# tk1363704/CAREL-VAE

Measured on AMD Instinct MI355X. Metric: clause-pairs/sec (training step), higher is better.
Workload: dtype bf16

## Files before the change

carel_vae_amd/csrc/carel_hip_internal.h:

```cpp
#pragma once
#include <hip/hip_runtime.h>
#include <stdarg.h>
#include <stdio.h>
#include "../../include/carel_hip.h"
#include "carel_common.h"

#ifdef CAREL_EXPERIMENTS
#define CAREL_TUNABLE(type, name, value) static type name = value
#else
#define CAREL_TUNABLE(type, name, value) static constexpr type name = value
#endif

namespace carel {

int set_error(int code, const char* fmt, ...);
int check_launch(const char* what);
int slab_reduce_multi(const void* slabs, void* out, int64_t n, const void* slabs2, void* out2, int64_t n2, int splits, const void* partials,
                      int nparts, void* dgamma, void* dbeta, void* dbias, hipStream_t stream);
#ifdef CAREL_EXPERIMENTS
int gemm_rowln_wanted(long rows);
int gemm_rowln_wanted_k(int K);
#else
inline int gemm_rowln_wanted(long) { return 0; }
inline int gemm_rowln_wanted_k(int) { return 0; }
#endif
void encoder_ln_resid_enable(int on);
void encoder_ln_slab_fusion_enable(int on);
void encoder_wgrad_group_enable(int on);
void adam_grid_cap(long cap);
void tail_overlap_enable(int on);
int gemm_pp_init_device(int device);
int gather_rows(const void* in_f32, const void* in_bf16, const void* idx, int n, void* out_f32, void* out_bf16, hipStream_t stream);
int scatter_rows(const void* in_f32, const void* in_bf16, const void* idx, int n, void* out_f32, void* out_bf16, hipStream_t stream);

int layernorm_bwd_rows(const void* dy, const void* h, const void* stats, const void* gamma, int64_t rows, uint32_t drop_seed, uint32_t drop_site,
                       uint32_t drop_idx_offset, float drop_p, const void* drop_row_map, void* dh_f32, void* dy_bf16, void* partials,
                       hipStream_t stream);
int layernorm_bwd_reduce(const void* partials, int64_t rows, void* dgamma, void* dbeta, void* dbias, hipStream_t stream);
int layernorm_bwd_blocks_max(int64_t rows);
int layernorm_bwd_rows_slabs(const void* slabs, int splits, const void* resid, const void* h, const void* stats, const void* gamma, int64_t rows,
                             uint32_t drop_seed, uint32_t drop_site, uint32_t drop_idx_offset, float drop_p, const void* drop_row_map, void* dh_f32,
                             void* dy_bf16, void* partials, hipStream_t stream);
int layernorm_fwd_slabs(const void* slabs, int splits, const void* bias, const void* resid, const void* resid_stats, const void* resid_gamma,
                        const void* resid_beta, uint32_t drop_seed, uint32_t drop_site, uint32_t drop_idx_offset, float drop_p, const void* drop_row_map,
                        void* h_out, const void* gamma, const void* beta, float eps, int64_t rows, void* x_f32, void* x_bf16, void* stats,
                        hipStream_t stream);

constexpr int GEMM_EX_FIXED_ROWS = 0x100;
constexpr int GEMM_EX_DEFER_EPILOGUE = 0x200;
int gemm_bf16_ex(const carel_gemm_args* a, int split_tile_factor, void* stream);
int gemm_bf16_split_plan(const carel_gemm_args* a, int split_tile_factor);
int gemm_wgrad_splits_max(int M, int N, long T);
int embed_ln_bwd_ex(const carel_embed_args* a, const void* dx0, void* dword, void* dpos, void* dtype_, void* dgamma, void* dbeta,
                    void* partials, void* row_scratch, hipStream_t stream, const void* sort_ws = nullptr);
int embed_sort_supported(const carel_embed_args* a);
size_t embed_sort_bytes();
int embed_ln_fwd_keys(const carel_embed_args* a, void* sort_ws, hipStream_t stream);
int embed_sort_rows(const carel_embed_args* a, void* sort_ws, hipStream_t stream);

struct WgradGroupProb { const void* dY; const void* X; void* dW; void* db; int M, N; };
struct WgradGroupLn { const void* partials; int nparts; void* dgamma; void* dbeta; void* dbias; };
size_t gemm_pp_wgrad_group_ws_bytes(const WgradGroupProb* pb, int n, long T);
int gemm_pp_wgrad_group_ok(const WgradGroupProb* pb, int n, long T);
int gemm_pp_wgrad_group(const WgradGroupProb* pb, int n, long T, void* ws, size_t ws_bytes, const WgradGroupLn* ln, int n_ln, hipStream_t stream);

inline Dropout make_dropout(uint32_t seed, uint32_t site, float p, uint32_t idx_offset) {
  Dropout d;
  d.key = mix32(seed + site * 0x9E3779B9u);
  d.idx_offset = idx_offset;
  if (p <= 0.f) { d.thresh = 0u; d.scale = 1.f; }
  else if (p >= 1.f) { d.thresh = 0xFFFFFFFFu; d.scale = 0.f; }
  else {
    d.thresh = (uint32_t)((double)p * 4294967296.0);
    d.scale = (float)(1.0 / (1.0 - (double)p));
    if (d.thresh == 0u) d.scale = 1.f;
  }
  return d;
}

struct AttnParams;
int attn_long_fwd(const AttnParams& q, hipStream_t stream);
int attn_long_bwd(const AttnParams& q, void* workspace, int64_t workspace_bytes, hipStream_t stream);

}
```

carel_vae_amd/csrc/encoder.hip:

```cpp
#include <cstdlib>
#include <mutex>
#include <vector>
#include "carel_hip_internal.h"

using namespace carel;

namespace {

constexpr int EH = 768, EI = 3072, ENH = 12;

size_t al(size_t x) { return (x + 255) & ~(size_t)255; }

struct LayerAct {
  char* xin_bf16; char* qkv; char* lse; char* ctx; char* h1; char* st1; char* x1_bf16; char* u; char* g; char* h2; char* st2;
};
struct ActLayout {
  size_t per_layer, total;
  size_t o_xin, o_qkv, o_lse, o_ctx, o_h1, o_st1, o_x1, o_u, o_g, o_h2, o_st2;
  size_t o_embst, o_xa, o_xb, o_cctx, o_cxres, o_layers;
};

ActLayout act_layout(long B, long S, int L, int inference) {
  const size_t T = (size_t)B * S;
  ActLayout a; size_t o = 0;
// ... 51 lines not shown
    const size_t n = (size_t)gemm_wgrad_splits_max(sh[0], sh[1], (long)T) * ((size_t)sh[0] * sh[1] + sh[0]) * 4;
    slab = n > slab ? n : slab;
  }
  {
    const WgradGroupProb pb[4] = {{nullptr, nullptr, nullptr, nullptr, EH, EI}, {nullptr, nullptr, nullptr, nullptr, EI, EH}, {nullptr, nullptr, nullptr, nullptr, 3 * EH, EH},
                                  {nullptr, nullptr, nullptr, nullptr, EH, EH}};
    const size_t n = gemm_pp_wgrad_group_ws_bytes(pb, 4, (long)T);
    slab = n > slab ? n : slab;
  }
  s.o_slabs = o; o += al(slab); s.slab_bytes = al(slab);
  s.o_ws = o; o += al(slab); s.ws_bytes = al(slab);
  size_t part = (size_t)layernorm_bwd_blocks_max((long)T) * 4 * EH * 4;
  const size_t cs = ((T + 255) / 256) * EI * 4;
  part = part > cs ? part : cs;
  for (int par = 0; par < 2; ++par) {
    s.o_part[par] = o; o += al(part);
    s.o_part3[par] = o; o += al(part);
  }
  s.o_part2 = o; o += al(part);
  s.o_sort = o; o += al(embed_sort_bytes());
  s.attn_bytes = (size_t)carel_attention_bwd_workspace_bytes((int32_t)B, (int32_t)S, 1);
  s.o_attn = o; o += al(s.attn_bytes);
  s.total = o;
  return s;
}

Scratch scratch_of(const ScratchLayout& l, char* b, int par = 0) {
  Scratch s; s.dy = b + l.o_dy; s.dyb = b + l.o_dyb[par]; s.dyb2 = b + l.o_dyb2[par]; s.du = b + l.o_du[par]; s.dctx = b + l.o_dctx; s.dqkv = b + l.o_dqkv[par];
  s.slabs = b + l.o_slabs; s.ws = b + l.o_ws; s.part = b + l.o_part[par]; s.part2 = b + l.o_part2; s.part3 = b + l.o_part3[par];
  return s;
}

long n_rows_of(const carel_encoder_args* a) {
  return (a->tok_row && a->n_tokens > 0) ? (long)a->n_tokens : (long)a->batch * a->seq_len;
}

int enc_check(const carel_encoder_args* a, const char* who) {
  if (!a) return set_error(CAREL_ERR_ARG, "%s: null args", who);
  if (a->hidden != EH || a->heads != ENH || a->intermediate != EI)
    return set_error(CAREL_ERR_SHAPE, "%s: only the BERT-base geometry (768/12/3072) is supported", who);
  if (a->batch < 1 || a->n_layers < 1) return set_error(CAREL_ERR_SHAPE, "%s: bad batch / n_layers", who);
  if (a->seq_len < 32 || a->seq_len > 512 || (a->seq_len & 31)) return set_error(CAREL_ERR_SHAPE, "%s: seq_len must be a multiple of 32 in [32, 512]", who);
  if (((long)a->batch * a->seq_len) % 128) return set_error(CAREL_ERR_SHAPE, "%s: batch*seq_len must be a multiple of 128 (pad the batch)", who);
  if (!a->input_ids || !a->layers || !a->act) return set_error(CAREL_ERR_ARG, "%s: null tensor", who);
  if (a->n_cls) {
    if (!a->cls_rows || !a->cls_orig_rows || a->n_cls % 128 || a->n_cls < a->batch || a->n_cls > ((a->batch + 127) / 128) * 128)
      return set_error(CAREL_ERR_ARG, "%s: n_cls must be batch rounded up to 128, with cls_rows and cls_orig_rows", who);
  }
  if (a->tok_row || a->cu_seqlens || a->n_tokens) {
    if (!a->tok_row || !a->cu_seqlens || a->n_tokens <= 0 || a->n_tokens % 128 || a->n_tokens > a->batch * a->seq_len)
      return set_error(CAREL_ERR_ARG, "%s: packing needs tok_row, cu_seqlens and n_tokens (multiple of 128, <= batch*seq_len)", who);
  }
  return CAREL_OK;
}

struct SideStream { static constexpr int NEV = 13; hipStream_t stream; hipStream_t aux; hipStream_t peer; hipEvent_t ev[NEV]; bool ok; };
SideStream* side_stream() {
  static SideStream per_dev[16];
  static bool made[16];
  int dev = 0;
  if (hipGetDevice(&dev) != hipSuccess || dev < 0 || dev >= 16) return nullptr;
  if (!made[dev]) {
    SideStream& s = per_dev[dev];
    int lo = 0, hi = 0;
    s.ok = hipDeviceGetStreamPriorityRange(&lo, &hi) == hipSuccess;
#ifdef CAREL_EXPERIMENTS
    if (const char* e = getenv("CAREL_SIDE_STREAM_PRIORITY")) { if (e[0] == 'n') lo = 0; else if (e[0] == 'h') lo = hi; }
#endif
    s.ok = s.ok &&
           hipStreamCreateWithPriority(&s.stream, hipStreamNonBlocking, lo) == hipSuccess &&
           hipStreamCreateWithPriority(&s.aux, hipStreamNonBlocking, lo) == hipSuccess &&
           hipStreamCreateWithFlags(&s.peer, hipStreamNonBlocking) == hipSuccess;
    for (int i = 0; i < SideStream::NEV && s.ok; ++i) s.ok = hipEventCreateWithFlags(&s.ev[i], hipEventDisableTiming) == hipSuccess;
    made[dev] = true;
  }
  return per_dev[dev].ok ? &per_dev[dev] : nullptr;
}

struct LnResid { const void* stats; const void* gamma; const void* beta; };
CAREL_TUNABLE(int, g_ln_slab_fusion, 1);
int ln_slab_fusion_enabled() { return g_ln_slab_fusion; }
CAREL_TUNABLE(int, g_wgrad_group, 1);
int wgrad_group_enabled() { return g_wgrad_group; }
CAREL_TUNABLE(int, g_ln_resid, 1);
int ln_resid_enabled() { return g_ln_resid; }
struct GemmCall { carel_gemm_args g; int flags; };
GemmCall gemm_fill(const void* A, const void* B, long lda, long ldb, int M, int N, int K, int form, int epi, int splits, void* out_bf16,
                   void* out2, void* out_f32, const void* bias, const void* resid, const void* aux, uint32_t seed, uint32_t site,
                   uint32_t off, float p, void* colsum_part = nullptr, const void* row_map = nullptr, void* ws = nullptr,
                   size_t ws_bytes = 0, int split_tile_factor = 1, const LnResid* lnres = nullptr) {
  GemmCall c;
  c.flags = split_tile_factor;
  carel_gemm_args& g = c.g;
  g.resid_ln_stats = lnres ? lnres->stats : nullptr; g.resid_ln_gamma = lnres ? lnres->gamma : nullptr; g.resid_ln_beta = lnres ? lnres->beta : nullptr;
  g.A = A; g.B = B; g.lda = lda; g.ldb = ldb; g.ldc = N; g.M = M; g.N = N; g.K = K; g.form = form; g.epilogue = epi; g.splits = splits;
  g.out_bf16 = out_bf16; g.out2_bf16 = out2; g.out_f32 = out_f32; g.bias = bias; g.resid_f32 = resid; g.aux_bf16 = aux;
  g.drop_seed = seed; g.drop_site = site; g.drop_idx_offset = off; g.drop_p = p; g.colsum_part = colsum_part; g.drop_row_map = row_map; g.colsum_a = nullptr;
  g.splitk_ws = ws; g.splitk_ws_bytes = (int64_t)ws_bytes;
  g.splitk_ws_zeroed = (ws != nullptr && (split_tile_factor & 0xff) == 1) ? 1 : 0;
  return c;
}
int gemm_run_ln(const GemmCall& c, bool fuse, void* stream, int* slabs) {
  *slabs = fuse ? gemm_bf16_split_plan(&c.g, c.flags) : 1;
  return gemm_bf16_ex(&c.g, c.flags | (*slabs > 1 ? GEMM_EX_DEFER_EPILOGUE : 0), stream);
}
int gemm_run(const GemmCall& c, void* stream) { return gemm_bf16_ex(&c.g, c.flags, stream); }

struct LnPartials { const void* partials; long rows; void* dgamma; void* dbeta; void* dbias; };
int wgrad_call(const void* dY, const void* X, long T, int M, int N, void* slabs, void* dW, void* stream, void* db = nullptr,
               const LnPartials* lnp = nullptr) {
  const int splits = wgrad_splits(T, M, N);
  carel_gemm_args g = gemm_fill(dY, X, M, N, M, N, (int)T, CAREL_GEMM_TN, CAREL_EPI_SLAB_F32, splits, nullptr, nullptr, slabs, nullptr, nullptr, nullptr, 0, 0, 0,
                                0.f).g;
  float* cs = db ? (float*)slabs + (size_t)splits * M * N : nullptr;
  g.colsum_a = cs;
  if (splits == 1) {
    g.out_f32 = dW;
    if (db) g.colsum_a = db;
    int rc = carel_gemm_bf16(&g, stream);
    if (!rc && lnp) rc = layernorm_bwd_reduce(lnp->partials, lnp->rows, lnp->dgamma, lnp->dbeta, lnp->dbias, (hipStream_t)stream);
    return rc;
  }
  int rc = carel_gemm_bf16(&g, stream);
  if (rc) return rc;
  return slab_reduce_multi(slabs, dW, (int64_t)M * N, cs, db, M, splits, lnp ? lnp->partials : nullptr,
                           lnp ? carel_layernorm_bwd_blocks(lnp->rows) : 0, lnp ? lnp->dgamma : nullptr, lnp ? lnp->dbeta : nullptr,
                           lnp ? lnp->dbias : nullptr, (hipStream_t)stream);
}

}

#ifdef CAREL_EXPERIMENTS
extern "C" int64_t carel_encoder_workspace_bytes(int32_t batch, int32_t seq_len, int32_t which) {
  const ScratchLayout sl = scratch_layout(batch, seq_len);
  return which == 0 ? (int64_t)sl.ws_bytes : which == 1 ? (int64_t)sl.slab_bytes : -1;
}
namespace carel { void encoder_ln_resid_enable(int on) { g_ln_resid = on ? 1 : 0; } void encoder_wgrad_group_enable(int on) { g_wgrad_group = on ? 1 : 0; }
                  void encoder_ln_slab_fusion_enable(int on) { g_ln_slab_fusion = on ? 1 : 0; } }
#endif

extern "C" void* carel_side_stream(int32_t which) {
  SideStream* sd = side_stream();
  if (!sd) { set_error(CAREL_ERR_HIP, "carel_side_stream: could not create the side streams"); return nullptr; }
  return which == 0 ? (void*)sd->stream : (void*)sd->aux;
}

extern "C" int64_t carel_encoder_act_bytes(int32_t batch, int32_t seq_len, int32_t n_layers, int32_t inference) {
  return (int64_t)act_layout(batch, seq_len, n_layers, inference).total;
}
extern "C" int64_t carel_encoder_scratch_bytes(int32_t batch, int32_t seq_len) {
  return (int64_t)scratch_layout(batch, seq_len).total;
}
extern "C" void* carel_encoder_x_last(const carel_encoder_args* a) {
  if (!a || !a->act) return nullptr;
  const ActLayout l = act_layout(a->batch, a->seq_len, a->n_layers, a->inference);
  return (char*)a->act + l.o_xa;
}

static carel_embed_args embed_args_of(const carel_encoder_args* a, const ActLayout& l, const LayerAct& first) {
  carel_embed_args e;
  e.input_ids = a->input_ids; e.token_type_ids = a->token_type_ids; e.word_emb = a->word_emb; e.pos_emb = a->pos_emb;
  e.type_emb = a->type_emb; e.ln_gamma = a->emb_ln_g; e.ln_beta = a->emb_ln_b; e.ln_eps = a->ln_eps;
  e.batch = a->batch; e.seq_len = a->seq_len; e.hidden = EH; e.vocab_size = a->vocab_size; e.max_pos = a->max_pos;
  e.type_vocab = a->type_vocab; e.roberta = a->roberta; e.pad_id = a->pad_id;
  e.drop_seed = a->drop_seed; e.drop_idx_offset = a->drop_row_offset * (uint32_t)(a->seq_len * EH); e.drop_p = a->hidden_dropout;
  e.x_f32 = (char*)a->act + l.o_xa; e.x_bf16 = first.xin_bf16; e.stats = (char*)a->act + l.o_embst;
  e.tok_row = a->tok_row; e.n_rows = a->tok_row ? a->n_tokens : 0;
  return e;
}

static int forward_layers(const carel_encoder_args* a, int l0, int l1, long b0, long nb, void* stream, char* ws, size_t ws_bytes, int chains = 1) {
  int rc;
  const long B = a->batch, S = a->seq_len;
  const bool whole = b0 == 0 && nb == B;
  const long T = whole ? n_rows_of(a) : nb * S;
  const long r0 = b0 * S;
  const ActLayout l = act_layout(B, S, a->n_layers, a->inference);
  char* base = (char*)a->act;
  char* xa = base + l.o_xa + (size_t)r0 * EH * 4;
  char* xb = base + l.o_xb + (size_t)r0 * EH * 4;
  const uint32_t hoff = (a->drop_row_offset + (uint32_t)b0) * (uint32_t)(S * EH), aoff = (a->drop_row_offset + (uint32_t)b0) * (uint32_t)(ENH * S * S);
  for (int i = l0; i < l1; ++i) {
    const carel_layer_params& w = a->layers[i];
    LayerAct la = layer_act(l, base, i, a->inference);
    la.xin_bf16 += (size_t)r0 * EH * 2; la.qkv += (size_t)r0 * 3 * EH * 2; la.lse += (size_t)b0 * ENH * S * 4; la.ctx += (size_t)r0 * EH * 2;
    la.h1 += (size_t)r0 * EH * 4; la.st1 += (size_t)r0 * 2 * 4; la.x1_bf16 += (size_t)r0 * EH * 2; la.u += (size_t)r0 * EI * 2;
    la.g += (size_t)r0 * EI * 2; la.h2 += (size_t)r0 * EH * 4; la.st2 += (size_t)r0 * 2 * 4;
    if ((rc = gemm_run(gemm_fill(la.xin_bf16, w.qkv_w, EH, EH, (int)T, 3 * EH, EH, CAREL_GEMM_NT, CAREL_EPI_BIAS_BF16, 1, la.qkv, nullptr, nullptr,
                                 w.qkv_b, nullptr, nullptr, 0, 0, 0, 0.f, nullptr, nullptr, ws, ws_bytes, chains), stream))) return rc;
    carel_attn_args at;
    at.qkv = la.qkv; at.attention_mask = a->attention_mask ? (const void*)((const long*)a->attention_mask + b0 * S) : nullptr;
    at.ctx = la.ctx; at.lse = la.lse; at.dctx = nullptr; at.dqkv = nullptr;
    at.batch = (int)nb; at.seq_len = (int)S; at.heads = ENH; at.head_dim = 64;
    at.drop_seed = a->drop_seed; at.drop_site = 1 + 3 * i; at.drop_idx_offset = aoff; at.drop_p = a->attn_dropout;
    at.cu_seqlens = whole ? a->cu_seqlens : nullptr;
    at.rel_bias_dist = a->rel_bias_dist; at.d_rel_bias_dist = nullptr;
    const bool cls_only = a->n_cls > 0 && i + 1 == a->n_layers;
    at.q_rows = cls_only ? 32 : 0;
    at.workspace = nullptr; at.workspace_bytes = 0;
    if ((rc = carel_attention_fwd(&at, stream))) return rc;
    if (cls_only && !whole) return set_error(CAREL_ERR_ARG, "carel_encoder_forward: internal: [CLS]-only layer on a partial batch");
    long R = T;
    const int fixed = cls_only ? GEMM_EX_FIXED_ROWS : 0;
    const void* Actx = la.ctx; const void* res1 = xa; const void* rmap = whole ? a->tok_row : nullptr;
    LnResid lr1, lr2;
    const LnResid* plr1 = nullptr;
    const bool lnres_on = ln_resid_enabled() && !gemm_rowln_wanted(T);
    if (lnres_on && i > 0 && !cls_only) {
      LayerAct lp = layer_act(l, base, i - 1, a->inference);
      lr1.stats = (const char*)lp.st2 + (size_t)r0 * 2 * 4; lr1.gamma = a->layers[i - 1].ln2_g; lr1.beta = a->layers[i - 1].ln2_b;
      res1 = (const char*)lp.h2 + (size_t)r0 * EH * 4; plr1 = &lr1;
    }
    if (cls_only) {
      R = a->n_cls;
      char* cctx = base + l.o_cctx; char* cxres = base + l.o_cxres;
      if ((rc = gather_rows(xa, la.ctx, a->cls_rows, (int)R, cxres, cctx, (hipStream_t)stream))) return rc;
      Actx = cctx; res1 = cxres; rmap = a->cls_orig_rows;
    }
    const bool lnres2 = lnres_on;
    lr2.stats = la.st1; lr2.gamma = w.ln1_g; lr2.beta = w.ln1_b;
// ... 126 lines not shown
    sd = side_stream();
    if (!sd) return set_error(CAREL_ERR_HIP, "carel_encoder_backward_layer: could not create the side stream / events");
  }
  void* wstream = sd ? (void*)sd->stream : stream;
  int nfork = 0;
  auto fork = [&]() -> int {
    if (!sd) return CAREL_OK;
    hipEvent_t ev = sd->ev[nfork++];
    if (hipEventRecord(ev, (hipStream_t)stream) != hipSuccess || hipStreamWaitEvent(sd->stream, ev, 0) != hipSuccess)
      return set_error(CAREL_ERR_HIP, "carel_encoder_backward_layer: event fork failed");
    return CAREL_OK;
  };
  auto group_done = [&](int i) -> int {
    if (!sd) return CAREL_OK;
    return hipEventRecord(sd->ev[4 + i], sd->stream) == hipSuccess ? CAREL_OK : set_error(CAREL_ERR_HIP, "carel_encoder_backward_layer: event record failed");
  };
  auto wait_group = [&](int i) -> int {
    if (!sd) return CAREL_OK;
    return hipStreamWaitEvent((hipStream_t)stream, sd->ev[4 + i], 0) == hipSuccess ? CAREL_OK : set_error(CAREL_ERR_HIP, "carel_encoder_backward_layer: event wait failed");
  };
  const bool cls_only = a->n_cls > 0 && layer + 1 == a->n_layers;
  const long R = cls_only ? (long)a->n_cls : T;
  const void* rmap = cls_only ? a->cls_orig_rows : a->tok_row;
  const void* ctx_rows = cls_only ? (const void*)((char*)a->act + l.o_cctx) : (const void*)la.ctx;
  carel_wgrad_group_args ga;
  ga.prob[0] = carel_wgrad_problem{s.dyb, la.g, g.ffn2_w, nullptr, EH, EI};
  ga.prob[1] = carel_wgrad_problem{s.du, la.x1_bf16, g.ffn1_w, g.ffn1_b, EI, EH};
  ga.prob[2] = carel_wgrad_problem{s.dqkv, la.xin_bf16, g.qkv_w, g.qkv_b, 3 * EH, EH};
  ga.prob[3] = carel_wgrad_problem{s.dyb2, la.ctx, g.out_w, nullptr, EH, EH};
  ga.n_prob = 4; ga.T = T; ga.workspace = s.slabs; ga.workspace_bytes = (int64_t)sl.slab_bytes;
  ga.ln[0] = carel_ln_partial_set{s.part, R, g.ln2_g, g.ln2_b, g.ffn2_b};
  ga.ln[1] = carel_ln_partial_set{s.part3, R, g.ln1_g, g.ln1_b, g.out_b};
  ga.n_ln = 2;
  bool grouped = false;
  if (wgrad_group_enabled() && !cls_only) {
    const int64_t need = carel_gemm_wgrad_group_ws_bytes(&ga);
    grouped = need >= 0 && need <= (int64_t)sl.slab_bytes;
  }
  GemmCall gqkv = gemm_fill(s.dqkv, w.qkv_w, 3 * EH, EH, (int)T, EH, 3 * EH, CAREL_GEMM_NN, CAREL_EPI_ADD_F32, 1, nullptr, nullptr, a->dx, nullptr, s.dy,
                            nullptr, 0, 0, 0, 0.f, nullptr, nullptr, s.ws, ws_bytes, 1);
  const int qkv_slabs = ln_slab_fusion_enabled() ? gemm_bf16_split_plan(&gqkv.g, gqkv.flags) : 1;
  const bool dx_in_slabs = qkv_slabs > 1 && layer + 1 < a->n_layers && !(a->n_cls > 0 && layer + 2 == a->n_layers);
  if ((rc = wait_group(0))) return rc;
  if (dx_in_slabs) {
    if ((rc = layernorm_bwd_rows_slabs(s.ws, qkv_slabs, s.dy, la.h2, la.st2, w.ln2_g, R, a->drop_seed, 3 + 3 * layer, hoff, a->hidden_dropout, rmap, s.dy,
                                       s.dyb, s.part, (hipStream_t)stream))) return rc;
  } else if ((rc = layernorm_bwd_rows(a->dx, la.h2, la.st2, w.ln2_g, R, a->drop_seed, 3 + 3 * layer, hoff, a->hidden_dropout, rmap, s.dy, s.dyb,
                               s.part, (hipStream_t)stream))) return rc;
  if (!grouped) {
    if ((rc = fork())) return rc;
    const LnPartials lp2{s.part, R, g.ln2_g, g.ln2_b, g.ffn2_b};
    if ((rc = wgrad_call(s.dyb, la.g, R, EH, EI, s.slabs, g.ffn2_w, wstream, nullptr, &lp2))) return rc;
    if ((rc = group_done(0))) return rc;
  }
  if ((rc = wait_group(1))) return rc;
  if ((rc = gemm_run(gemm_fill(s.dyb, w.ffn2_w, EH, EI, (int)R, EI, EH, CAREL_GEMM_NN, CAREL_EPI_MUL_BF16, 1, s.du, nullptr, nullptr, nullptr,
                               nullptr, la.u, 0, 0, 0, 0.f, nullptr), stream))) return rc;
  if (!grouped) {
    if ((rc = fork())) return rc;
    if ((rc = wgrad_call(s.du, la.x1_bf16, R, EI, EH, s.slabs, g.ffn1_w, wstream, g.ffn1_b))) return rc;
    if ((rc = group_done(1))) return rc;
  }
  int ffn1_slabs;
  if ((rc = gemm_run_ln(gemm_fill(s.du, w.ffn1_w, EI, EH, (int)R, EH, EI, CAREL_GEMM_NN, CAREL_EPI_ADD_F32, 1, nullptr, nullptr, a->dx, nullptr, s.dy, nullptr,
                                  0, 0, 0, 0.f, nullptr, nullptr, s.ws, ws_bytes, 1 | (cls_only ? GEMM_EX_FIXED_ROWS : 0)),
                        ln_slab_fusion_enabled() && !cls_only, stream, &ffn1_slabs))) return rc;
  if ((rc = wait_group(2))) return rc;
  if (ffn1_slabs > 1) {
    if ((rc = layernorm_bwd_rows_slabs(s.ws, ffn1_slabs, s.dy, la.h1, la.st1, w.ln1_g, R, a->drop_seed, 2 + 3 * layer, hoff, a->hidden_dropout, rmap, s.dy,
                                       s.dyb2, s.part3, (hipStream_t)stream))) return rc;
  } else if ((rc = layernorm_bwd_rows(a->dx, la.h1, la.st1, w.ln1_g, R, a->drop_seed, 2 + 3 * layer, hoff, a->hidden_dropout, rmap, s.dy, s.dyb2,
                               s.part3, (hipStream_t)stream))) return rc;
  void* dctx_rows = cls_only ? (void*)s.dqkv : (void*)s.dctx;
  if (!grouped) {
    if ((rc = fork())) return rc;
    const LnPartials lp1{s.part3, R, g.ln1_g, g.ln1_b, g.out_b};
    if ((rc = wgrad_call(s.dyb2, ctx_rows, R, EH, EH, s.slabs, g.out_w, wstream, nullptr, &lp1))) return rc;
    if ((rc = group_done(2))) return rc;
  }
  if (cls_only && (rc = wait_group(3))) return rc;
  if ((rc = gemm_run(gemm_fill(s.dyb2, w.out_w, EH, EH, (int)R, EH, EH, CAREL_GEMM_NN, CAREL_EPI_BIAS_BF16, 1, dctx_rows, nullptr, nullptr, nullptr,
                               nullptr, nullptr, 0, 0, 0, 0.f, nullptr, nullptr, s.ws, ws_bytes, 1 | (cls_only ? GEMM_EX_FIXED_ROWS : 0)), stream))) return rc;
  if (cls_only) {
    hipError_t he = hipMemsetAsync(s.dctx, 0, (size_t)T * EH * 2, (hipStream_t)stream);
    if (he == hipSuccess) he = hipMemsetAsync(a->dx, 0, (size_t)T * EH * 4, (hipStream_t)stream);
    if (he != hipSuccess) return set_error(CAREL_ERR_HIP, "carel_encoder_backward_layer: memset: %s", hipGetErrorString(he));
    if ((rc = scatter_rows(nullptr, s.dqkv, a->cls_rows, (int)R, nullptr, s.dctx, (hipStream_t)stream))) return rc;
    if ((rc = scatter_rows(s.dy, nullptr, a->cls_rows, (int)R, a->dx, nullptr, (hipStream_t)stream))) return rc;
  }
  const void* dh1_full = cls_only ? (const void*)a->dx : (const void*)s.dy;
  carel_attn_args at;
  at.qkv = la.qkv; at.attention_mask = a->attention_mask; at.ctx = la.ctx; at.lse = la.lse; at.dctx = s.dctx; at.dqkv = s.dqkv;
  at.batch = (int)B; at.seq_len = (int)S; at.heads = ENH; at.head_dim = 64;
  at.drop_seed = a->drop_seed; at.drop_site = 1 + 3 * layer; at.drop_idx_offset = aoff; at.drop_p = a->attn_dropout;
  at.cu_seqlens = a->cu_seqlens;
  at.rel_bias_dist = a->rel_bias_dist; at.d_rel_bias_dist = a->d_rel_bias_dist;
  at.q_rows = cls_only ? 32 : 0;
  at.workspace = (char*)a->scratch + sl.o_attn; at.workspace_bytes = (int64_t)sl.attn_bytes;
  if (a->tok_row && layer + 2 >= a->n_layers) {
    hipError_t he = hipMemsetAsync(s.dqkv + (size_t)(T - 128) * 3 * EH * 2, 0, (size_t)128 * 3 * EH * 2, (hipStream_t)stream);
    if (he != hipSuccess) return set_error(CAREL_ERR_HIP, "carel_encoder_backward_layer: memset: %s", hipGetErrorString(he));
  }
  if ((rc = wait_group(3))) return rc;
  if ((rc = carel_attention_bwd(&at, stream))) return rc;
  if ((rc = fork())) return rc;
  if (grouped) { if ((rc = carel_gemm_wgrad_group(&ga, wstream))) return rc; }
  else if ((rc = wgrad_call(s.dqkv, la.xin_bf16, T, 3 * EH, EH, s.slabs, g.qkv_w, wstream, g.qkv_b))) return rc;
  const bool defer_qkv = qkv_slabs > 1 && layer > 0 && !cls_only;
  gqkv.g.resid_f32 = dh1_full;
  if ((rc = gemm_bf16_ex(&gqkv.g, gqkv.flags | (defer_qkv ? GEMM_EX_DEFER_EPILOGUE : 0), stream))) return rc;
  if (!grouped && (rc = group_done(3))) return rc;
  if (sd) {
    if (hipEventRecord(sd->ev[10 + par], sd->stream) != hipSuccess || hipStreamWaitEvent((hipStream_t)stream, sd->ev[10 + (par ^ 1)], 0) != hipSuccess)
      return set_error(CAREL_ERR_HIP, "carel_encoder_backward_layer: event record / wait failed");
  }
  return CAREL_OK;
}

extern "C" int carel_encoder_backward_join(const carel_encoder_args* a, void* stream) {
  if (!a) return set_error(CAREL_ERR_ARG, "carel_encoder_backward_join: null args");
  if (!(a->overlap_wgrad & 1)) return CAREL_OK;
  SideStream* sd = side_stream();
  if (!sd) return set_error(CAREL_ERR_HIP, "carel_encoder_backward_join: no side stream");
  hipEvent_t ev = sd->ev[SideStream::NEV - 1];
  if (hipEventRecord(ev, sd->stream) != hipSuccess || hipStreamWaitEvent((hipStream_t)stream, ev, 0) != hipSuccess)
    return set_error(CAREL_ERR_HIP, "carel_encoder_backward_join: event join failed");
  return CAREL_OK;
}

extern "C" int carel_encoder_backward_embeddings(const carel_encoder_args* a, void* stream) {
  int rc = enc_check(a, "carel_encoder_backward_embeddings");
  if (rc) return rc;
  if ((rc = carel_encoder_backward_join(a, stream))) return rc;
  if (a->inference || !a->scratch || !a->dx || !a->d_word_emb || !a->d_pos_emb || !a->d_type_emb || !a->d_emb_ln_g || !a->d_emb_ln_b)
    return set_error(CAREL_ERR_ARG, "carel_encoder_backward_embeddings: null buffer or inference-mode forward");
  const long B = a->batch, S = a->seq_len;
  const ActLayout l = act_layout(B, S, a->n_layers, 0);
  const LayerAct la = layer_act(l, (char*)a->act, 0, 0);
  const Scratch s = scratch_of(scratch_layout(B, S), (char*)a->scratch);
  carel_embed_args e = embed_args_of(a, l, la);
  hipError_t he = hipMemsetAsync(a->d_word_emb, 0, (size_t)a->vocab_size * EH * 4, (hipStream_t)stream);
  if (he == hipSuccess) he = hipMemsetAsync(a->d_pos_emb, 0, (size_t)a->max_pos * EH * 4, (hipStream_t)stream);
  if (he != hipSuccess) return set_error(CAREL_ERR_HIP, "carel_encoder_backward_embeddings: memset: %s", hipGetErrorString(he));
  const ScratchLayout sl = scratch_layout(B, S);
  bool side = false;
  const bool keyed = embed_sort_supported(&e) && embed_keys_match(a, &e, &side);
  if (keyed && side && !(a->overlap_wgrad & 1)) {
    SideStream* sd = side_stream();
    if (!sd) return set_error(CAREL_ERR_HIP, "carel_encoder_backward_embeddings: no side stream");
    hipEvent_t ev = sd->ev[SideStream::NEV - 1];
    if (hipEventRecord(ev, sd->stream) != hipSuccess || hipStreamWaitEvent((hipStream_t)stream, ev, 0) != hipSuccess)
      return set_error(CAREL_ERR_HIP, "carel_encoder_backward_embeddings: event join failed");
  }
  const void* sort_ws = keyed ? (const char*)a->scratch + sl.o_sort : nullptr;
  return embed_ln_bwd_ex(&e, a->dx, a->d_word_emb, a->d_pos_emb, a->d_type_emb, a->d_emb_ln_g, a->d_emb_ln_b, s.part, s.dy, (hipStream_t)stream, sort_ws);
}

namespace {

__global__ __launch_bounds__(64) void attn_f32_kernel(const float* __restrict__ qkv, const long* __restrict__ mask, const float* __restrict__ rel,
                                                      float* __restrict__ ctx, int S) {
  const int lane = threadIdx.x;
  const int q = blockIdx.x % S, h = (blockIdx.x / S) % ENH, b = blockIdx.x / (S * ENH);
  __shared__ float qs[64], ps[128];
  const float* base = qkv + (long)b * S * (3 * EH);
  qs[lane] = base[(long)q * (3 * EH) + h * 64 + lane];
  __syncthreads();
  float sc[2], mx = -INFINITY;
#pragma unroll
  for (int i = 0; i < 2; ++i) {
    const int k = lane + i * 64;
// ... 91 lines not shown
```

carel_vae_amd/csrc/gemm.hip:

```cpp
#include "gemm_epilogue.h"
#include "reduce_device.h"

namespace carel {

template <int EPI>
__global__ __launch_bounds__(256) void slab_epilogue_kernel(GemmParams p, const float* __restrict__ slabs, int splits) {
  const long chunk = (long)blockIdx.x * 256 + threadIdx.x;
  const int cpr = p.N >> 3;
  if (chunk >= (long)p.M * cpr) return;
  const long row = chunk / cpr, col = (chunk - row * cpr) * 8;
  const long off = row * p.N + col, plane = (long)p.M * p.N;
  float v[8];
  {
    const float4 a = *(const float4*)(slabs + off), b = *(const float4*)(slabs + off + 4);
    v[0] = a.x; v[1] = a.y; v[2] = a.z; v[3] = a.w; v[4] = b.x; v[5] = b.y; v[6] = b.z; v[7] = b.w;
  }
  for (int z = 1; z < splits; ++z) {
    const float4 a = *(const float4*)(slabs + z * plane + off), b = *(const float4*)(slabs + z * plane + off + 4);
    v[0] += a.x; v[1] += a.y; v[2] += a.z; v[3] += a.w; v[4] += b.x; v[5] += b.y; v[6] += b.z; v[7] += b.w;
  }
  epi_store8<EPI>(p, v, row, col);
}

template <bool AT, bool BT, int EPI, int DBG = 0>
// ... 675 lines not shown
      if (hipEventSynchronize(g_prof.cal2[i + 1]) == hipSuccess && hipEventElapsedTime(&t, g_prof.cal2[i], g_prof.cal2[i + 1]) == hipSuccess) c2.push_back(t);
    }
    if (!c2.empty()) { std::sort(c2.begin(), c2.end()); g_prof.last_pair_us = c2[c2.size() / 2] * 1e3; }
  }
  for (size_t i = 0; i + 1 < g_prof.used; i += 2) {
    if (hipEventSynchronize(g_prof.ev[i + 1]) != hipSuccess) return set_error(CAREL_ERR_HIP, "carel_profile_gemm_read: event sync failed");
    float t = 0.f;
    if (hipEventElapsedTime(&t, g_prof.ev[i], g_prof.ev[i + 1]) != hipSuccess) return set_error(CAREL_ERR_HIP, "carel_profile_gemm_read: elapsed failed");
    ms += (t > overhead ? t - overhead : 0.0); fl += g_prof.flops[i / 2];
  }
  *total_ms = ms; *total_flops = fl; *launches = (int64_t)(g_prof.used / 2);
  g_prof.used = 0; g_prof.flops.clear();
  return CAREL_OK;
}

extern "C" int carel_profile_gemm_overheads(double* empty_kernel_bracket_us, double* event_pair_us) {
  if (!empty_kernel_bracket_us || !event_pair_us) return set_error(CAREL_ERR_ARG, "carel_profile_gemm_overheads: null output");
  *empty_kernel_bracket_us = g_prof.last_empty_us; *event_pair_us = g_prof.last_pair_us;
  return CAREL_OK;
}

static int gemm_shape_ok(int M, int N, int K, int splits, int form) {
  if (M <= 0 || N <= 0 || K <= 0 || splits <= 0) return 0;
  if (form == CAREL_GEMM_TN) {
    if (M % 256 == 0 && N % 96 == 0 && K % 64 == 0 && (K >> 6) / splits >= 4) return 1;
  }
  const bool pp = form != CAREL_GEMM_TN && N % 96 == 0 && K >= 256;
  if (!((M % 128 == 0 && N % 128 == 0) || (M % 256 == 0 && N % 192 == 0) || pp)) return 0;
  if (K % (64 * splits)) return 0;
  return 1;
}

#ifdef CAREL_EXPERIMENTS
CAREL_TUNABLE(int, g_rowln_mode, 0);
CAREL_TUNABLE(long, g_rowln_min_rows, 6144);
namespace carel {
int gemm_rowln_wanted(long rows) { return g_rowln_mode != 0 && rows >= g_rowln_min_rows; }
int gemm_rowln_wanted_k(int K) { return g_rowln_mode == 1 || K <= 768; }
}
extern "C" int carel_gemm_rowln(const carel_gemm_rowln_args* a, void* stream_) {
  hipStream_t stream = (hipStream_t)stream_;
  if (!a) return set_error(CAREL_ERR_ARG, "carel_gemm_rowln: null args");
  if (a->M < 1 || a->K < 128 || (a->K & 127)) return set_error(CAREL_ERR_SHAPE, "carel_gemm_rowln: M >= 1 and K a multiple of 128 (M=%d K=%d)", a->M, a->K);
  if (!a->A || !a->W || !a->resid_f32 || !a->gamma || !a->beta) return set_error(CAREL_ERR_ARG, "carel_gemm_rowln: null operand");
  if ((((uintptr_t)a->A | (uintptr_t)a->W | (uintptr_t)a->resid_f32 | (uintptr_t)a->gamma | (uintptr_t)a->beta | (uintptr_t)a->bias | (uintptr_t)a->h_f32 |
        (uintptr_t)a->x_f32 | (uintptr_t)a->x_bf16) & 15) || (a->lda & 7) || a->lda < a->K || (!a->w_packed && ((a->ldb & 7) || a->ldb < a->K)))
    return set_error(CAREL_ERR_ARG, "carel_gemm_rowln: operands must be 16-byte aligned, leading dimensions multiples of 8 and >= K");
  RowLnParams p;
  p.A = (const bf16_t*)a->A; p.lda = a->lda; p.W = (const bf16_t*)a->W; p.ldb = a->ldb; p.bias = (const float*)a->bias; p.resid = (const float*)a->resid_f32;
  p.gamma = (const float*)a->gamma; p.beta = (const float*)a->beta; p.eps = a->eps;
  p.h_out = (float*)a->h_f32; p.x_f32 = (float*)a->x_f32; p.x_bf16 = (bf16_t*)a->x_bf16; p.stats = (float*)a->stats; p.M = a->M; p.K = a->K;
  p.drop = make_dropout(a->drop_seed, a->drop_site, a->drop_p, a->drop_idx_offset); p.drop_row_map = (const int*)a->drop_row_map;
  ProfScope prof_scope(stream, 2.0 * (double)a->M * 768.0 * (double)a->K);
  return gemm_rowln_launch(p, a->w_packed != 0, stream);
}
extern "C" int carel_gemm_rowln_pack(const void* W, int64_t ldb, int32_t K, void* out, void* stream) {
  if (!W || !out || K < 128 || (K & 127) || ldb < K || (ldb & 7) || (((uintptr_t)W | (uintptr_t)out) & 15))
    return set_error(CAREL_ERR_ARG, "carel_gemm_rowln_pack: bad arguments (K multiple of 128, ldb >= K multiple of 8, 16-byte aligned pointers)");
  return gemm_rowln_pack(W, (long)ldb, K, out, (hipStream_t)stream);
}

extern "C" int carel_gemm_set_variant(int32_t v) {
  if (v >= 20 && v <= 23) { g_xcd_n = 1 << (v - 20); return CAREL_OK; }
  if (v == 24) { g_xcd_n = 0; return CAREL_OK; }
  if (v == 30 || v == 31) { g_big_auto = v - 30; return CAREL_OK; }
  if (v >= 50 && v <= 59) { g_pp_min_tiles = (v - 50) * 32; return CAREL_OK; }
  if (v >= 340 && v <= 342) { g_sm_mode = v - 340; return CAREL_OK; }
  if (v >= 330 && v <= 333) { g_resid_split = v - 330; return CAREL_OK; }
  if (v >= 40 && v <= 49) { g_pp_min_tiles_k768 = (v - 40) * 32; return CAREL_OK; }
  if (v >= 70 && v <= 73) { gemm_pp_force_npn(v - 70); return CAREL_OK; }
  if (v >= 100 && v <= 116) { gemm_pp_wgrad_force(v - 100); return CAREL_OK; }
  if (v == 130 || v == 131) { g_auto_split_min_k = v == 130 ? 1536 : 768; return CAREL_OK; }
  if (v == 140 || v == 141) { g_pp_split = v - 140; return CAREL_OK; }
  if (v == 160 || v == 161) { gemm_pp_gelu_lut(v - 160); return CAREL_OK; }
  if (v >= 190 && v <= 192) { g_rowln_mode = v - 190; return CAREL_OK; }
  if (v >= 193 && v <= 195) { gemm_rowln_dbg(v - 193); return CAREL_OK; }
  if (v == 270 || v == 271) { encoder_ln_slab_fusion_enable(v - 270); return CAREL_OK; }
  if (v >= 250 && v <= 252) { gemm_pp_group_mode(v - 250); return CAREL_OK; }
  if (v == 240 || v == 241) { encoder_wgrad_group_enable(v - 240); return CAREL_OK; }
  if (v == 230 || v == 231) { encoder_ln_resid_enable(v - 230); return CAREL_OK; }
  if (v >= 220 && v <= 225) { gemm_tri_enable(v - 220); return CAREL_OK; }
  if (v >= 280 && v <= 292) { adam_grid_cap(32L << (v - 280)); return CAREL_OK; }
  if (v == 210 || v == 211) { tail_overlap_enable(v - 210); return CAREL_OK; }
  if (v == 200 || v == 201) { gemm_pp_pair_enable(v - 200); return CAREL_OK; }
  if (v == 170 || v == 171) { gemm_pp_epi_prefetch(v - 170); return CAREL_OK; }
  if (v == 120 || v == 121) { gemm_pp_xcd_rect(v - 120); return CAREL_OK; }
  if (v == 90 || v == 91) { gemm_pp_wide_variant(v - 90); return CAREL_OK; }
  g_gemm_variant = v;
  return CAREL_OK;
}
#endif

static int gemm_prepare(const carel_gemm_args* a, int split_tile_factor, PlannedGemm* out) {
  if (!a) return set_error(CAREL_ERR_ARG, "carel_gemm_bf16: null args");
  const int splits = a->splits > 0 ? a->splits : 1;
  if (!gemm_shape_ok(a->M, a->N, a->K, splits, a->form))
    return set_error(CAREL_ERR_SHAPE, "carel_gemm_bf16: (M,N) must be multiples of (128,128) or (256,192) and K of 64*splits (M=%d N=%d K=%d splits=%d)",
                     a->M, a->N, a->K, splits);
  if (!a->A || !a->B) return set_error(CAREL_ERR_ARG, "carel_gemm_bf16: null operand");
  if (((uintptr_t)a->A | (uintptr_t)a->B) & 15 || (a->lda & 7) || (a->ldb & 7) || (a->ldc & 3))
    return set_error(CAREL_ERR_ARG, "carel_gemm_bf16: operands must be 16-byte aligned, ld multiples of 8");
  GemmParams p = {};
  p.A = (const bf16_t*)a->A; p.B = (const bf16_t*)a->B; p.lda = a->lda; p.ldb = a->ldb;
  p.M = a->M; p.N = a->N; p.K = a->K / splits;
  p.out0 = (bf16_t*)a->out_bf16; p.out1 = (bf16_t*)a->out2_bf16; p.outf = (float*)a->out_f32; p.ldc = a->ldc;
  p.bias = (const float*)a->bias; p.resid = (const float*)a->resid_f32; p.aux = (const bf16_t*)a->aux_bf16;
  p.resid_stats = (const float*)a->resid_ln_stats; p.resid_gamma = (const float*)a->resid_ln_gamma; p.resid_beta = (const float*)a->resid_ln_beta;
  if (p.resid_stats || p.resid_gamma || p.resid_beta) {
    if (a->epilogue != EPI_BIAS_DROP_RESID || !p.resid_stats || !p.resid_gamma || !p.resid_beta)
      return set_error(CAREL_ERR_ARG, "carel_gemm_bf16: resid_ln_stats / _gamma / _beta go together and with CAREL_EPI_BIAS_DROP_RESID only");
    if ((((uintptr_t)p.resid_stats) & 7) || (((uintptr_t)p.resid_gamma | (uintptr_t)p.resid_beta) & 15))
      return set_error(CAREL_ERR_ARG, "carel_gemm_bf16: resid_ln_* pointers must be 8 / 16-byte aligned");
  }
  p.drop = make_dropout(a->drop_seed, a->drop_site, a->drop_p, a->drop_idx_offset);
  p.tiles_m = a->M / 128; p.tiles_n = a->N / 128;
  p.split_tile_factor = split_tile_factor;
  p.xcd_n = (a->form == CAREL_GEMM_TN && g_xcd_n <= 1) ? 8 : g_xcd_n;
  p.splitk_ws = (float*)a->splitk_ws; p.splitk_ws_bytes = a->splitk_ws ? (size_t)a->splitk_ws_bytes : 0;
  p.pair_flags = nullptr; p.pair_seq = 0;
  if (a->splitk_ws && a->splitk_ws_zeroed && (size_t)a->splitk_ws_bytes > (size_t)(64 << 20) && ((uintptr_t)a->splitk_ws & 15) == 0 && (a->splitk_ws_bytes & 15) == 0) {
    p.splitk_ws_bytes -= PP_PAIR_FLAG_BYTES;
    p.pair_flags = (unsigned*)((char*)a->splitk_ws + p.splitk_ws_bytes);
  }
  if (a->ldc != a->N) p.splitk_ws = nullptr;
  if (a->colsum_part) p.splitk_ws = nullptr;
  p.colsum_part = (float*)a->colsum_part; p.drop_row_map = (const int*)a->drop_row_map; p.colsum_a = (float*)a->colsum_a;
  if (p.colsum_a && a->form != CAREL_GEMM_TN) return set_error(CAREL_ERR_ARG, "carel_gemm_bf16: colsum_a is a TN-form (wgrad) option");
  const int form = a->form, epi = a->epilogue;
  if (splits != 1 && epi != EPI_SLAB_F32) return set_error(CAREL_ERR_ARG, "carel_gemm_bf16: split-K only with the slab epilogue");
#define NEED(ptr, what) if (!(ptr)) return set_error(CAREL_ERR_ARG, "carel_gemm_bf16: epilogue needs " what)
  switch (epi) {
    case EPI_BIAS_BF16: NEED(p.out0, "out_bf16"); break;
    case EPI_BIAS_GELU: NEED(p.out1, "out2_bf16"); break;
    case EPI_BIAS_GELU_DG: NEED(p.out0, "out_bf16"); NEED(p.out1, "out2_bf16"); break;
    case EPI_BIAS_DROP_RESID: NEED(p.outf, "out_f32"); NEED(p.resid, "resid_f32"); break;
    case EPI_DGELU_BF16: case EPI_MUL_BF16: NEED(p.out0, "out_bf16"); NEED(p.aux, "aux_bf16"); break;
    case EPI_ADD_F32: NEED(p.outf, "out_f32"); break;
    case EPI_SLAB_F32: NEED(p.outf, "out_f32"); break;
    default: return set_error(CAREL_ERR_ARG, "carel_gemm_bf16: unknown epilogue %d", epi);
  }
#undef NEED
  const auto fn = launch_instance(form, epi);
  if (!fn) return set_error(CAREL_ERR_ARG, "carel_gemm_bf16: unsupported form/epilogue combination (%d,%d)", form, epi);
  *out = PlannedGemm{p, splits, gemm_plan(p, form, epi, splits, a->K), fn};
  if (form == CAREL_GEMM_TN && out->plan.family == PLAN_PP) out->p.K = a->K;
  if (out->plan.family == PLAN_NONE)
    return set_error(CAREL_ERR_SHAPE, "carel_gemm_bf16: no kernel of this form takes the shape (M=%d N=%d K=%d splits=%d)", a->M, a->N, a->K, splits);
  return CAREL_OK;
}

extern "C" int carel_gemm_bf16(const carel_gemm_args* a, void* stream_) { return carel::gemm_bf16_ex(a, 1, stream_); }

int carel::gemm_bf16_split_plan(const carel_gemm_args* a, int split_tile_factor) {
  PlannedGemm g;
  return gemm_prepare(a, split_tile_factor, &g) ? 1 : g.plan.slabs;
}

#ifdef CAREL_EXPERIMENTS
extern "C" int carel_gemm_split_plan(const carel_gemm_args* a, int32_t flags, int32_t* plan) {
  if (!plan) return set_error(CAREL_ERR_ARG, "carel_gemm_split_plan: null plan");
  if (flags & ~(0xff | GEMM_EX_FIXED_ROWS)) return set_error(CAREL_ERR_ARG, "carel_gemm_split_plan: flags are a chain count | CAREL_PLAN_FIXED_ROWS");
  PlannedGemm g;
  if (const int rc = gemm_prepare(a, flags ? flags : 1, &g)) return rc;
  plan[0] = g.plan.slabs; plan[1] = g.plan.family; plan[2] = g.plan.npn;
  return CAREL_OK;
}
// ... 92 lines not shown
```

carel_vae_amd/csrc/ln.hip:

```cpp
#include "carel_hip_internal.h"
#include "ln_device.h"
#include "reduce_device.h"

namespace carel {

__global__ __launch_bounds__(256) void ln_fwd_kernel(const float* __restrict__ h, const float* __restrict__ gamma,
                                                     const float* __restrict__ beta, float eps, long rows,
                                                     float* __restrict__ x_f32, bf16_t* __restrict__ x_bf16,
                                                     float* __restrict__ stats) {
  const int lane = threadIdx.x & 63;
  const long row = (long)blockIdx.x * 4 + (threadIdx.x >> 6);
  if (row >= rows) return;
  Row X = load_row(h + row * H, lane);
  const Row G = load_row(gamma, lane), Bt = load_row(beta, lane);
  float mean, rstd;
  ln_normalise(X, G, Bt, eps, mean, rstd);
  if (x_f32) store_row(x_f32 + row * H, lane, X);
  if (x_bf16) store_row_bf16(x_bf16 + row * H, lane, X);
  if (stats && lane == 0) { stats[row * 2] = mean; stats[row * 2 + 1] = rstd; }
}

struct LnFwdSlabs {
  const float* slabs; int splits; long plane;
  const float* bias; const float* resid; const float* resid_stats; const float* resid_gamma; const float* resid_beta;
// ... 364 lines not shown
  if (threadIdx.x < PR_COLS && c < n) out[c] = accumulate ? out[c] + t : t;
}

__global__ __launch_bounds__(256) void partial_reduce_seg_kernel(const float* __restrict__ partials, SegOuts outs, int seg,
                                                                 int n, int nparts) {
  __shared__ float lds[256];
  int c;
  const float t = partial_colsum16(partials, n, nparts, lds, c, (int)blockIdx.x);
  if (threadIdx.x < PR_COLS && c < n) {
    float* o = outs.p[c / seg];
    if (o) o[c % seg] = t;
  }
}

__global__ __launch_bounds__(256) void colsum_bf16_kernel(const bf16_t* __restrict__ x, long ld, long rows, int n,
                                                          float* __restrict__ partials) {
  __shared__ float lds[8][256 + 8];
  const int cg = threadIdx.x & 31, rl = threadIdx.x >> 5;
  const int col = blockIdx.x * 256 + cg * 8;
  const long r0 = (long)blockIdx.y * 256;
  float acc[8] = {0.f, 0.f, 0.f, 0.f, 0.f, 0.f, 0.f, 0.f};
  if (col < n) {
    for (long r = r0 + rl; r < r0 + 256 && r < rows; r += 8) {
      const uint4 v = *(const uint4*)(x + r * ld + col);
      acc[0] += bf2f((bf16_t)(v.x & 0xffff)); acc[1] += bf2f((bf16_t)(v.x >> 16));
      acc[2] += bf2f((bf16_t)(v.y & 0xffff)); acc[3] += bf2f((bf16_t)(v.y >> 16));
      acc[4] += bf2f((bf16_t)(v.z & 0xffff)); acc[5] += bf2f((bf16_t)(v.z >> 16));
      acc[6] += bf2f((bf16_t)(v.w & 0xffff)); acc[7] += bf2f((bf16_t)(v.w >> 16));
    }
  }
#pragma unroll
  for (int e = 0; e < 8; ++e) lds[rl][cg * 8 + e] = acc[e];
  __syncthreads();
  const int c = threadIdx.x;
  if (blockIdx.x * 256 + c < n) {
    float s = 0.f;
#pragma unroll
    for (int r = 0; r < 8; ++r) s += lds[r][c];
    partials[(long)blockIdx.y * n + blockIdx.x * 256 + c] = s;
  }
}

__global__ __launch_bounds__(256) void gather_rows_kernel(const float* __restrict__ in_f, const bf16_t* __restrict__ in_b,
                                                          const int* __restrict__ idx, int n, float* __restrict__ out_f,
                                                          bf16_t* __restrict__ out_b) {
  const int lane = threadIdx.x & 63;
  const int i = blockIdx.x * 4 + (threadIdx.x >> 6);
  if (i >= n) return;
  const long r = idx[i];
  if (in_f) {
    Row X;
    if (r >= 0) X = load_row(in_f + r * H, lane);
    else for (int v = 0; v < NV; ++v) X.v[v] = float4{0.f, 0.f, 0.f, 0.f};
    store_row(out_f + (long)i * H, lane, X);
  }
  if (in_b) {
#pragma unroll
    for (int v = 0; v < NV; ++v) {
      const int c = (v * 64 + lane) * 4;
      uint2 x = {0u, 0u};
      if (r >= 0) x = *(const uint2*)(in_b + r * H + c);
      *(uint2*)(out_b + (long)i * H + c) = x;
    }
  }
}
__global__ __launch_bounds__(256) void scatter_rows_kernel(const float* __restrict__ in_f, const bf16_t* __restrict__ in_b,
                                                           const int* __restrict__ idx, int n, float* __restrict__ out_f,
                                                           bf16_t* __restrict__ out_b) {
  const int lane = threadIdx.x & 63;
  const int i = blockIdx.x * 4 + (threadIdx.x >> 6);
  if (i >= n) return;
  const long r = idx[i];
  if (r < 0) return;
  if (in_f) store_row(out_f + r * H, lane, load_row(in_f + (long)i * H, lane));
  if (in_b) {
#pragma unroll
    for (int v = 0; v < NV; ++v) {
      const int c = (v * 64 + lane) * 4;
      *(uint2*)(out_b + r * H + c) = *(const uint2*)(in_b + (long)i * H + c);
    }
  }
}

int gather_rows(const void* in_f32, const void* in_bf16, const void* idx, int n, void* out_f32, void* out_bf16, hipStream_t stream) {
  hipLaunchKernelGGL(gather_rows_kernel, dim3((n + 3) / 4), dim3(256), 0, stream, (const float*)in_f32, (const bf16_t*)in_bf16,
                     (const int*)idx, n, (float*)out_f32, (bf16_t*)out_bf16);
  return check_launch("gather_rows_kernel");
}
int scatter_rows(const void* in_f32, const void* in_bf16, const void* idx, int n, void* out_f32, void* out_bf16, hipStream_t stream) {
  hipLaunchKernelGGL(scatter_rows_kernel, dim3((n + 3) / 4), dim3(256), 0, stream, (const float*)in_f32, (const bf16_t*)in_bf16,
                     (const int*)idx, n, (float*)out_f32, (bf16_t*)out_bf16);
  return check_launch("scatter_rows_kernel");
}

}

using namespace carel;

static EmbedArgs make_embed(const carel_embed_args* a) {
  EmbedArgs e;
  e.ids = (const long*)a->input_ids; e.tt = (const long*)a->token_type_ids;
  e.word = (const float*)a->word_emb; e.pos = (const float*)a->pos_emb; e.type = (const float*)a->type_emb;
  e.gamma = (const float*)a->ln_gamma; e.beta = (const float*)a->ln_beta;
  e.eps = a->ln_eps; e.S = a->seq_len; e.roberta = a->roberta; e.pad_id = a->pad_id;
  e.tok_row = (const int*)a->tok_row;
  e.rows = (a->tok_row && a->n_rows > 0) ? (long)a->n_rows : (long)a->batch * a->seq_len;
  e.vocab = a->vocab_size; e.max_pos = a->max_pos; e.type_vocab = a->type_vocab;
  e.drop = make_dropout(a->drop_seed, 0u, a->drop_p, a->drop_idx_offset);
  return e;
}

static int embed_check(const carel_embed_args* a, const char* who) {
  if (!a) return set_error(CAREL_ERR_ARG, "%s: null args", who);
  if (a->hidden != H) return set_error(CAREL_ERR_SHAPE, "%s: hidden must be %d (got %d)", who, H, a->hidden);
  if (!a->input_ids || !a->word_emb || !a->pos_emb || !a->type_emb || !a->ln_gamma || !a->ln_beta)
    return set_error(CAREL_ERR_ARG, "%s: null tensor", who);
  if (a->batch <= 0 || a->seq_len <= 0 || a->type_vocab < 1 || a->type_vocab > 2)
    return set_error(CAREL_ERR_SHAPE, "%s: bad batch/seq_len/type_vocab", who);
  const long pos_limit = a->roberta ? (long)a->max_pos - a->pad_id - 1 : (long)a->max_pos;
  if (a->seq_len > pos_limit)
    return set_error(CAREL_ERR_SHAPE, "%s: seq_len %d runs past the position table (max_pos %d%s: at most %ld positions)", who, a->seq_len,
                     a->max_pos, a->roberta ? ", ids from pad_id + 1" : "", pos_limit);
  return CAREL_OK;
}

extern "C" int carel_embed_ln_fwd(const carel_embed_args* a, void* stream_) {
  hipStream_t stream = (hipStream_t)stream_;
  int rc = embed_check(a, "carel_embed_ln_fwd");
  if (rc) return rc;
  if (!a->x_f32 || !a->x_bf16 || !a->stats) return set_error(CAREL_ERR_ARG, "carel_embed_ln_fwd: null output");
  EmbedArgs e = make_embed(a);
  hipLaunchKernelGGL(embed_fwd_kernel, dim3((unsigned)((e.rows + 3) / 4)), dim3(256), 0, stream, e, (float*)a->x_f32,
                     (bf16_t*)a->x_bf16, (float*)a->stats, (int2*)nullptr);
  return check_launch("embed_fwd_kernel");
}

namespace carel {
int embed_sort_supported(const carel_embed_args* a) {
  const long rows = (a->tok_row && a->n_rows > 0) ? (long)a->n_rows : (long)a->batch * a->seq_len;
  return rows >= 1 && rows <= EMB_SORT_MAX && a->vocab_size < (1 << (32 - EMB_ROW_BITS)) && a->max_pos < (1 << (32 - EMB_ROW_BITS));
}
size_t embed_sort_bytes() { return (size_t)EMB_SORT_MAX * 8 + 2 * (size_t)EMB_SORT_MAX * 4; }
int embed_ln_fwd_keys(const carel_embed_args* a, void* sort_ws, hipStream_t stream) {
  int rc = embed_check(a, "carel_embed_ln_fwd");
  if (rc) return rc;
  if (!a->x_f32 || !a->x_bf16 || !a->stats || !sort_ws) return set_error(CAREL_ERR_ARG, "carel_embed_ln_fwd: null output");
  EmbedArgs e = make_embed(a);
  hipLaunchKernelGGL(embed_fwd_kernel, dim3((unsigned)((e.rows + 3) / 4)), dim3(256), 0, stream, e, (float*)a->x_f32,
                     (bf16_t*)a->x_bf16, (float*)a->stats, (int2*)sort_ws);
  return check_launch("embed_fwd_kernel");
}
int embed_sort_rows(const carel_embed_args* a, void* sort_ws, hipStream_t stream) {
  const long rows = (a->tok_row && a->n_rows > 0) ? (long)a->n_rows : (long)a->batch * a->seq_len;
  hipLaunchKernelGGL(embed_sort_kernel, dim3(2), dim3(1024), 0, stream, (const int2*)sort_ws, (int)rows, (uint32_t*)((char*)sort_ws + (size_t)EMB_SORT_MAX * 8));
  return check_launch("embed_sort_kernel");
}
}

extern "C" int carel_embed_ln_bwd_blocks(int64_t rows) { return (int)((rows + LNB_ROWS - 1) / LNB_ROWS); }

namespace carel {
int embed_ln_bwd_ex(const carel_embed_args* a, const void* dx0, void* dword, void* dpos, void* dtype_, void* dgamma, void* dbeta,
                    void* partials, void* row_scratch, hipStream_t stream, const void* sort_ws) {
  int rc = embed_check(a, "carel_embed_ln_bwd");
  if (rc) return rc;
  if (!dx0 || !dword || !dpos || !dtype_ || !dgamma || !dbeta || !partials || !a->stats)
// ... 151 lines not shown
```

carel_vae_amd/csrc/rowvec_device.h:

```cpp
#pragma once
#include "carel_hip_internal.h"

namespace carel {

constexpr int TH = 768;
constexpr int TNV = TH / 256;

struct PtrSet4 { const float* w[4]; const float* b[4]; };

template <int ACT>
__global__ __launch_bounds__(256) void rowvec_linear_kernel(const float* __restrict__ in, long in_stride, const int* __restrict__ row_idx,
                                                            int B, int N, int seg, PtrSet4 ps, float* __restrict__ out, long out_stride) {
  const int lane = threadIdx.x & 63;
  const int n = blockIdx.x * 4 + (threadIdx.x >> 6);
  if (n >= N) return;
  const int bg = (B + gridDim.y - 1) / gridDim.y, b0 = blockIdx.y * bg, b1 = min(B, b0 + bg);
  const float* w = ps.w[n / seg] + (long)(n % seg) * TH;
  const float bias = ps.b[n / seg] ? ps.b[n / seg][n % seg] : 0.f;
  float4 wv[TNV];
#pragma unroll
  for (int i = 0; i < TNV; ++i) wv[i] = *(const float4*)(w + (i * 64 + lane) * 4);
  for (int b = b0; b < b1; b += 4) {
    float s[4];
#pragma unroll
    for (int u = 0; u < 4; ++u) {
      const int bb = min(b + u, b1 - 1);
      const float* x = row_idx ? in + (long)row_idx[bb] * TH : in + (long)bb * in_stride;
      float t = 0.f;
#pragma unroll
      for (int i = 0; i < TNV; ++i) {
        const float4 xv = *(const float4*)(x + (i * 64 + lane) * 4);
        t += (xv.x * wv[i].x + xv.y * wv[i].y) + (xv.z * wv[i].z + xv.w * wv[i].w);
      }
      s[u] = t;
    }
#pragma unroll
    for (int off = 32; off > 0; off >>= 1) {
#pragma unroll
      for (int u = 0; u < 4; ++u) s[u] += __shfl_xor(s[u], off, 64);
    }
#pragma unroll
    for (int u = 0; u < 4; ++u) {
      float v = s[u] + bias;
      if (ACT == 1) v = tanhf(v);
      if (lane == 0 && b + u < b1) out[(long)(b + u) * out_stride + n] = v;
    }
  }
}

struct OutSet4 { float* w[4]; float* b[4]; };
static __global__ __launch_bounds__(256) void rowvec_wgrad_kernel(const float* __restrict__ dY, long dy_stride, const float* __restrict__ X,
                                                           long x_stride, const int* __restrict__ row_idx, int B, int N, int seg, OutSet4 os) {
  const int lane = threadIdx.x & 63;
  const int n = blockIdx.x * 4 + (threadIdx.x >> 6);
  if (n >= N) return;
  float4 acc[TNV];
#pragma unroll
  for (int i = 0; i < TNV; ++i) acc[i] = float4{0.f, 0.f, 0.f, 0.f};
  float sb = 0.f;
  constexpr int U = 8;
  for (int b = 0; b < B; b += U) {
    float g[U]; float4 xv[U][TNV];
#pragma unroll
    for (int u = 0; u < U; ++u) {
      const int bb = min(b + u, B - 1);
      g[u] = (b + u < B) ? dY[(long)bb * dy_stride + n] : 0.f;
      const float* x = row_idx ? X + (long)row_idx[bb] * TH : X + (long)bb * x_stride;
#pragma unroll
      for (int i = 0; i < TNV; ++i) xv[u][i] = *(const float4*)(x + (i * 64 + lane) * 4);
    }
#pragma unroll
    for (int u = 0; u < U; ++u) {
      sb += g[u];
#pragma unroll
      for (int i = 0; i < TNV; ++i) {
        acc[i].x = fmaf(g[u], xv[u][i].x, acc[i].x); acc[i].y = fmaf(g[u], xv[u][i].y, acc[i].y);
        acc[i].z = fmaf(g[u], xv[u][i].z, acc[i].z); acc[i].w = fmaf(g[u], xv[u][i].w, acc[i].w);
      }
    }
  }
  float* w = os.w[n / seg] + (long)(n % seg) * TH;
#pragma unroll
  for (int i = 0; i < TNV; ++i) *(float4*)(w + (i * 64 + lane) * 4) = acc[i];
  if (lane == 0 && os.b[n / seg]) os.b[n / seg][n % seg] = sb;
}

constexpr int DG_CHUNK = 32;
template <int MODE>
__global__ __launch_bounds__(256) void rowvec_dgrad_kernel(const float* __restrict__ dY, long dy_stride, int B, int N, int seg,
                                                           PtrSet4 ps, const float* __restrict__ y, float* __restrict__ dpre,
                                                           float* __restrict__ part) {
  const int lane = threadIdx.x & 63;
  const int b = blockIdx.x * 4 + (threadIdx.x >> 6);
  if (b >= B) return;
  float4 acc[TNV];
#pragma unroll
  for (int i = 0; i < TNV; ++i) acc[i] = float4{0.f, 0.f, 0.f, 0.f};
  const int n0 = blockIdx.y * DG_CHUNK, n1 = min(N, n0 + DG_CHUNK);
  constexpr int U = 8;
  for (int nb = n0; nb < n1; nb += U) {
    float g[U]; float4 wv[U][TNV];
#pragma unroll
    for (int u = 0; u < U; ++u) {
      const int n = min(nb + u, n1 - 1);
      float gg = (nb + u < n1) ? dY[(long)b * dy_stride + n] : 0.f;
      if (MODE == 1) {
        const float yy = y[(long)b * N + n];
        gg *= (1.0f - yy * yy);
        if (lane == 0 && nb + u < n1) dpre[(long)b * N + n] = gg;
      }
      g[u] = gg;
      const float* w = ps.w[n / seg] + (long)(n % seg) * TH;
#pragma unroll
      for (int i = 0; i < TNV; ++i) wv[u][i] = *(const float4*)(w + (i * 64 + lane) * 4);
    }
#pragma unroll
    for (int u = 0; u < U; ++u) {
#pragma unroll
      for (int i = 0; i < TNV; ++i) {
        acc[i].x = fmaf(g[u], wv[u][i].x, acc[i].x); acc[i].y = fmaf(g[u], wv[u][i].y, acc[i].y);
        acc[i].z = fmaf(g[u], wv[u][i].z, acc[i].z); acc[i].w = fmaf(g[u], wv[u][i].w, acc[i].w);
      }
    }
  }
  float* o = part + ((long)blockIdx.y * B + b) * TH;
#pragma unroll
  for (int i = 0; i < TNV; ++i) *(float4*)(o + (i * 64 + lane) * 4) = acc[i];
}

static __global__ __launch_bounds__(256) void sum_parts_kernel(const float* __restrict__ part, float* __restrict__ out, long n, int nparts) {
  const long i = ((long)blockIdx.x * 256 + threadIdx.x) * 4;
  if (i >= n) return;
  float4 a = *(const float4*)(part + i);
  for (int p = 1; p < nparts; ++p) {
    const float4 b = *(const float4*)(part + (long)p * n + i);
    a.x += b.x; a.y += b.y; a.z += b.z; a.w += b.w;
  }
  *(float4*)(out + i) = a;
}

static __global__ void scale_inplace_kernel(float* __restrict__ x, long n, const float* __restrict__ scale) {
  const float s = scale[0];
  long i = (long)blockIdx.x * blockDim.x + threadIdx.x;
  const long stride = (long)gridDim.x * blockDim.x;
  for (; i < n; i += stride) x[i] *= s;
}
static __global__ __launch_bounds__(256) void scatter_cls_kernel(const float* __restrict__ dcls, int B, int S, const int* __restrict__ row_idx,
                                                          float* __restrict__ dx) {
  const int b = blockIdx.x;
  const long row = row_idx ? (long)row_idx[b] : (long)b * S;
  for (int k = threadIdx.x; k < TH; k += 256) dx[row * TH + k] = dcls[(long)b * TH + k];
}


}
```

carel_vae_amd/csrc/tail.hip:

```cpp
#include "carel_hip_internal.h"
#include "mmd_device.h"
#include "hsic_device.h"
#include "rowvec_device.h"

namespace carel {

struct TailCore {
  int B, D, EC;
  const float* lat;
  const float* eps_e; const float* eps_c;
  const float* emo_w; const float* emo_b;
  const float* cau_w; const float* cau_b;
  const float* pair_w; const float* pair_b;
  const long* emo_labels; const float* cau_labels; const float* pair_labels;
  float w_mmd, w_emo, w_cau, w_pair, kl_w, ls;
  int dis_mode;
  int emo_bce;
  Dropout d_emo, d_cau, d_pair;
  float alpha, mmd_eps;
  const float* label_sum_override; float n_override;
  int label_sum_ranks;
  const float* z_global; int n_global, row_offset; float mmd_grad_scale;
  int rank_stride;
  const float* mmd_part; int mmd_nblk; const float* dz_mmd;
// ... 9 lines not shown

struct MmdGlobalArgs {
  const float* zg; int n, B, D, rank_stride, row_offset;
  float alpha, eps, gscale;
  float* part;
  float* dz;
};
template <int CD>
__global__ __launch_bounds__(256) void mmd_global_kernel(MmdGlobalArgs a) {
  constexpr int CH = 256, ZS = CD + 1;
  __shared__ float zc[CH * ZS];
  __shared__ float nc[CH];
  __shared__ float red[64];
  const int t = threadIdx.x, grp = t & 7;
  const int n = a.n, n2 = 2 * n, D = a.D, D2 = 2 * D;
  auto zrow = [&](int r) -> const float* {
    const int side = r >= n, s = r - side * n;
    return a.zg + (long)(s / a.B) * a.rank_stride + (long)(s % a.B) * D2 + side * D;
  };
  const int i = blockIdx.x * 32 + (t >> 3);
  const bool live = i < n2;
  float zi[CD], g[CD];
  float ni = 0.f;
  {
    const float* zp = zrow(live ? i : 0);
#pragma unroll
    for (int k = 0; k < CD; ++k) { zi[k] = (k < D) ? zp[k] : 0.f; g[k] = 0.f; ni = fmaf(zi[k], zi[k], ni); }
  }
  const bool i1 = i < n;
  const int si = i - (i1 ? 0 : n);
  const bool local = live && si >= a.row_offset && si < a.row_offset + a.B;
  const float a00 = (float)(1.0 / ((double)n * (n - 1))), a01 = (float)(-1.0 / ((double)n * n));
  float s11 = 0.f, s22 = 0.f, s12 = 0.f;
  for (int c0 = 0; c0 < n2; c0 += CH) {
    const int cn = min(CH, n2 - c0);
    __syncthreads();
    for (int e = t; e < cn * CD; e += 256) {
      const int r = e / CD, k = e - r * CD;
      zc[r * ZS + k] = (k < D) ? zrow(c0 + r)[k] : 0.f;
    }
    __syncthreads();
    for (int r = t; r < cn; r += 256) {
      float s = 0.f;
#pragma unroll
      for (int k = 0; k < CD; ++k) s = fmaf(zc[r * ZS + k], zc[r * ZS + k], s);
      nc[r] = s;
    }
    __syncthreads();
    if (live) {
      for (int jj = grp; jj < cn; jj += 8) {
        const int j = c0 + jj;
        if (j == i) continue;
        float zj[CD], dot = 0.f;
#pragma unroll
        for (int k = 0; k < CD; ++k) { zj[k] = zc[jj * ZS + k]; dot = fmaf(zi[k], zj[k], dot); }
        const float d2 = ni + nc[jj] - 2.0f * dot;
        const float e = expf(-a.alpha * (a.eps + fabsf(d2)));
        const bool j1 = j < n;
        if (i1 && j1) s11 += e; else if (!i1 && !j1) s22 += e; else if (i1 && !j1) s12 += e;
        if (local) {
          const float dcs = (d2 > 0.f) ? a.alpha * e : ((d2 < 0.f) ? -a.alpha * e : 0.f);
          const float coef = -4.0f * ((i1 == j1) ? a00 : a01) * dcs * a.gscale;
#pragma unroll
          for (int k = 0; k < CD; ++k) g[k] = fmaf(coef, zi[k] - zj[k], g[k]);
        }
      }
    }
  }
#pragma unroll
  for (int k = 0; k < CD; ++k) {
    float v = g[k];
    v += __shfl_xor(v, 1, 64); v += __shfl_xor(v, 2, 64); v += __shfl_xor(v, 4, 64);
    if (local && grp == 0 && k < D) a.dz[(long)(si - a.row_offset) * D2 + (i1 ? 0 : D) + k] = v;
  }
  __syncthreads();
  s11 = block_sum(s11, red);
  s22 = block_sum(s22, red + 16);
  s12 = block_sum(s12, red + 32);
  if (t == 0) { a.part[blockIdx.x * 4] = s11; a.part[blockIdx.x * 4 + 1] = s22; a.part[blockIdx.x * 4 + 2] = s12; }
}

static long long* g_tail_prof = nullptr;
CAREL_TUNABLE(int, g_tail_overlap, 1);
#ifdef CAREL_EXPERIMENTS
void tail_overlap_enable(int on) { g_tail_overlap = on ? 1 : 0; }
#endif
struct TailEvents { hipEvent_t fork, join; bool ok; };
static TailEvents* tail_events() {
  static TailEvents per_dev[16];
  static bool made[16];
  int dev = 0;
  if (hipGetDevice(&dev) != hipSuccess || dev < 0 || dev >= 16) return nullptr;
  if (!made[dev]) {
    TailEvents& t = per_dev[dev];
    t.ok = hipEventCreateWithFlags(&t.fork, hipEventDisableTiming) == hipSuccess && hipEventCreateWithFlags(&t.join, hipEventDisableTiming) == hipSuccess;
    made[dev] = true;
  }
  return per_dev[dev].ok ? &per_dev[dev] : nullptr;
}

__global__ __launch_bounds__(1024) void tail_core_kernel(TailCore a) {
  extern __shared__ __attribute__((aligned(16))) char smem_raw[];
  float* red = (float*)smem_raw;
  float* sc = red + 64;
  const int B = a.B, D = a.D, D2 = 2 * a.D, D4 = 4 * a.D;
  float* zl = sc + 64;
  float* dzl = zl + B * D2;
  float* elog = dzl + B * D2;
  float* gx = elog + B * 8;
  float* mlt = gx + B * 2;
  float* lg = mlt + B * D4;
  float* hw = lg + B * 16;
  const int n_emo = a.EC * D;
  const int o_eb = n_emo, o_cw = o_eb + a.EC, o_cb = o_cw + D, o_pw = o_cb + 1, o_pb = o_pw + D2, n_hw = o_pb + 1;
  const int nm = a.z_global ? a.n_global : B;
  float* nrm = hw + ((n_hw + 3) & ~3);
  float* Z = nrm + ((2 * nm + 3) & ~3);
  const int zs = D | 1;
  const int t = threadIdx.x;
  TAIL_STAMP(0);

  for (int e = t; e < B * D2; e += blockDim.x) {
    const int b = e / D2, k = e - b * D2;
    const float* row = a.lat + (long)b * 4 * D;
    const float z = (k < D) ? row[k] + a.eps_e[k] * expf(row[D + k]) : row[2 * D + (k - D)] + a.eps_c[k - D] * expf(row[3 * D + (k - D)]);
    zl[e] = z; dzl[e] = 0.f;
    if (a.z) a.z[e] = z;
  }
  for (int e = t; e < B * D4; e += blockDim.x) {
    const int b = e / D4, k = e - b * D4;
    mlt[e] = k < D ? dropout_mult(a.d_emo, b * D + k) : (k < D2 ? dropout_mult(a.d_cau, b * D + (k - D)) : dropout_mult(a.d_pair, b * D2 + (k - D2)));
  }
  for (int e = t; e < n_hw; e += blockDim.x)
    hw[e] = e < o_eb ? a.emo_w[e] : e < o_cw ? a.emo_b[e - o_eb] : e < o_cb ? a.cau_w[e - o_cw] : e < o_pw ? a.cau_b[0]
          : e < o_pb ? a.pair_w[e - o_pw] : a.pair_b[0];
  __syncthreads();
  for (int e = t; e < (a.mmd_part ? 0 : 2 * nm * D); e += blockDim.x) {
    const int i = e / D, k = e - i * D;
    const int s = i < nm ? i : i - nm, off = i < nm ? 0 : D;
    Z[i * zs + k] = a.z_global ? a.z_global[(long)(s / B) * a.rank_stride + (long)(s % B) * D2 + off + k] : zl[s * D2 + off + k];
  }
  __syncthreads();
  TAIL_STAMP(1);
  float mmd = 0.f;
  float dis_term = 0.f;
  if (a.dis_mode == 0 && a.mmd_part) {
    if (t == 0) {
      double s11 = 0.0, s22 = 0.0, s12 = 0.0;
      for (int q = 0; q < a.mmd_nblk; ++q) { s11 += a.mmd_part[q * 4]; s22 += a.mmd_part[q * 4 + 1]; s12 += a.mmd_part[q * 4 + 2]; }
      const double b00 = 1.0 / ((double)nm * (nm - 1)), b01 = -1.0 / ((double)nm * nm);
      sc[0] = (float)(2.0 * b01 * s12 + b00 * s11 + b00 * s22);
    }
    __syncthreads();
    mmd = sc[0];
    dis_term = -a.w_mmd * mmd;
    for (int e = t; e < B * D2; e += blockDim.x) dzl[e] += a.dz_mmd[e];
    TAIL_STAMP(2);
  } else if (a.dis_mode == 0) {
    MmdCfg mc; mc.n1 = nm; mc.n2 = nm; mc.d = D; mc.zs = zs; mc.n_alphas = 1; mc.alphas[0] = a.alpha; mc.eps = a.mmd_eps;
    if (!a.z_global && D == 24) {
      mmd = mmd_forward_backward_block<24>(mc, Z, nrm, red, -a.w_mmd * a.mmd_grad_scale, dzl, D2);
      dis_term = -a.w_mmd * mmd;
      TAIL_STAMP(2);
    } else {
      mmd = mmd_forward_block(mc, Z, nrm, red, nullptr);
      dis_term = -a.w_mmd * mmd;
      TAIL_STAMP(2);
      const int rows = 2 * B;
// ... 96 lines not shown
    const float sg = 1.0f / (1.0f + expf(-xb));
    gx[b * 2 + 1] = dead ? 0.f : ((1.f - tb) - lw * (1.f - sg)) * (a.w_pair / B);
  }
  __syncthreads();
  TAIL_STAMP(4);
  float kle = 0.f, klc = 0.f;
  for (int e = t; e < B * D; e += blockDim.x) {
    const int b = e / D, k = e - b * D;
    const float* row = a.lat + (long)b * 4 * D;
    const float mue = row[k], lve = row[D + k], muc = row[2 * D + k], lvc = row[3 * D + k];
    kle += -0.5f * (1.f + lve - expf(lve) - mue * mue);
    klc += -0.5f * (1.f + lvc - expf(lvc) - muc * muc);
    float* dl = a.dlat_direct + (long)b * 4 * D;
    dl[k] = a.kl_w * mue / B; dl[D + k] = a.kl_w * (-0.5f) * (1.f - expf(lve)) / B;
    dl[2 * D + k] = a.kl_w * muc / B; dl[3 * D + k] = a.kl_w * (-0.5f) * (1.f - expf(lvc)) / B;
  }
  kle = block_sum(kle, red) / B * a.kl_w;
  klc = block_sum(klc, red) / B * a.kl_w;
  TAIL_STAMP(5);
  for (int e = t; e < B * D2; e += blockDim.x) {
    const int b = e / D2, k = e - b * D2;
    float g = hw[o_pw + k] * gx[b * 2 + 1] * mlt[b * D4 + D2 + k];
    if (k < D) {
      float s = 0.f;
      for (int c = 0; c < a.EC; ++c) s = fmaf(hw[c * D + k], elog[b * 8 + c], s);
      g += s * mlt[b * D4 + k];
    } else {
      g += hw[o_cw + (k - D)] * gx[b * 2] * mlt[b * D4 + k];
    }
    dzl[e] += g;
  }
  TAIL_STAMP(6);
  for (int e = t; e < n_hw; e += blockDim.x) {
    float s = 0.f;
    if (e < o_eb) {
      const int c = e / D, k = e - c * D;
      for (int b = 0; b < B; ++b) s = fmaf(elog[b * 8 + c], zl[b * D2 + k] * mlt[b * D4 + k], s);
      a.d_emo_w[e] = s;
    } else if (e < o_cw) {
      const int c = e - o_eb;
      for (int b = 0; b < B; ++b) s += elog[b * 8 + c];
      a.d_emo_b[c] = s;
    } else if (e < o_cb) {
      const int k = e - o_cw;
      for (int b = 0; b < B; ++b) s = fmaf(gx[b * 2], zl[b * D2 + D + k] * mlt[b * D4 + D + k], s);
      a.d_cau_w[k] = s;
    } else if (e == o_cb) {
      for (int b = 0; b < B; ++b) s += gx[b * 2];
      a.d_cau_b[0] = s;
    } else if (e < o_pb) {
      const int k = e - o_pw;
      for (int b = 0; b < B; ++b) s = fmaf(gx[b * 2 + 1], zl[b * D2 + k] * mlt[b * D4 + D2 + k], s);
      a.d_pair_w[k] = s;
    } else {
      for (int b = 0; b < B; ++b) s += gx[b * 2 + 1];
      a.d_pair_b[0] = s;
    }
  }
  __syncthreads();
  TAIL_STAMP(7);
  for (int e = t; e < B * D2; e += blockDim.x) a.dz[e] = dzl[e];
  if (t == 0) {
    a.terms[1] = mmd; a.terms[2] = l_emo; a.terms[3] = l_cau; a.terms[4] = l_pair; a.terms[5] = kle; a.terms[6] = klc;
    a.terms[0] = dis_term + a.w_emo * l_emo + a.w_cau * l_cau + a.w_pair * l_pair + kle + klc;
    a.pair_dead[0] = dead ? 1.f : 0.f;
  }
}

constexpr int DEC_J = 128;
constexpr int DEC_MAXD2 = 64;
constexpr int DEC_MAXG = 4;

struct DecArgs {
  int B, D2, V;
  const float* z;
  const float* w; const float* b;
  const float* bow;
  float ls;
  float* part;
  float* rowstat;
  float* dz_part;
  float* dw; float* db;
  float gscale;
};

template <int CD2>
__device__ __forceinline__ float dec_logit(const float* wr, const float* zrow, int D2rt, float bias) {
  const int D2 = CD2 ? CD2 : D2rt;
  float s = bias;
  if (CD2 && (CD2 & 3) == 0) {
#pragma unroll
    for (int k = 0; k < D2; k += 4) {
      const float4 zv = *(const float4*)(zrow + k);
      s = fmaf(wr[k], zv.x, s); s = fmaf(wr[k + 1], zv.y, s); s = fmaf(wr[k + 2], zv.z, s); s = fmaf(wr[k + 3], zv.w, s);
    }
  } else {
#pragma unroll
    for (int k = 0; k < D2; ++k) s = fmaf(wr[k], zrow[k], s);
  }
  return s;
}

template <int PASS, int CD2>
__global__ __launch_bounds__(DEC_J * DEC_MAXG) void decoder_kernel(DecArgs a) {
  const int D2 = CD2 ? CD2 : a.D2;
  const int ws = D2 + 1;
  extern __shared__ __attribute__((aligned(16))) char smem_raw[];
  float* zl = (float*)smem_raw;
  float* red = zl + a.B * D2;
  float* wl = red + 16;
  float* tile = wl + DEC_J * ws;
  float* tile2 = tile + a.B * DEC_J;
  const int t = threadIdx.x, nthr = blockDim.x, G = nthr / DEC_J;
  const int tj = t & (DEC_J - 1), g = t / DEC_J;
  const int j0 = blockIdx.x * DEC_J, j = j0 + tj;
  const bool live = j < a.V;
  const int Bg = (a.B + G - 1) / G, b0 = g * Bg, b1 = min(a.B, b0 + Bg);
  for (int e = t; e < a.B * D2; e += nthr) zl[e] = a.z[e];
  {
    const int nrow = min(DEC_J, a.V - j0);
    for (int e = t; e < nrow * D2; e += nthr) { const int r = e / D2, k = e - r * D2; wl[r * ws + k] = a.w[(long)j0 * D2 + e]; }
  }
  __syncthreads();
  float wr[CD2 ? CD2 : DEC_MAXD2];
  _Pragma("unroll") for (int k = 0; k < D2; ++k) wr[k] = live ? wl[tj * ws + k] : 0.f;
  const float bias = live ? a.b[j] : 0.f;
  const int lane = t & 63, wv = t >> 6, nwv = nthr >> 6;
  if (PASS == 1) {
    for (int b = b0; b < b1; ++b) tile[b * DEC_J + tj] = live ? dec_logit<CD2>(wr, zl + b * D2, D2, bias) : -INFINITY;
    __syncthreads();
    for (int b = wv; b < a.B; b += nwv) {
      const float x0 = tile[b * DEC_J + lane], x1 = tile[b * DEC_J + 64 + lane];
      const float m = wave_max(fmaxf(x0, x1));
      const float s2 = wave_sum(expf(x0 - m) + expf(x1 - m));
      if (lane == 0) { a.part[((long)blockIdx.x * a.B + b) * 2] = m; a.part[((long)blockIdx.x * a.B + b) * 2 + 1] = s2; }
    }
  } else if (PASS == 2) {
    for (int bb = b0; bb < b1; bb += 4) {
      float bw[4];
      _Pragma("unroll") for (int u = 0; u < 4; ++u) bw[u] = (live && bb + u < b1) ? a.bow[(long)(bb + u) * a.V + j] : 0.f;
      _Pragma("unroll") for (int u = 0; u < 4; ++u) {
        const int b = bb + u;
        if (b < b1) {
          float le = 0.f, dt = 0.f;
          if (live) {
            const float lp = dec_logit<CD2>(wr, zl + b * D2, D2, bias) - a.rowstat[b * 4] - a.rowstat[b * 4 + 1];
            const float p = expf(lp);
            const float tg = bw[u] * (1.f - a.ls) + a.ls / a.V;
            le = -(tg * fmaxf(lp, -100.f) + (1.f - tg) * fmaxf(log1pf(-p), -100.f));
            dt = p * ((p - tg) / fmaxf((1.f - p) * p, 1e-12f));
          }
          tile[b * DEC_J + tj] = le; tile2[b * DEC_J + tj] = dt;
        }
      }
    }
    __syncthreads();
    for (int b = wv; b < a.B; b += nwv) {
      const float le = wave_sum(tile[b * DEC_J + lane] + tile[b * DEC_J + 64 + lane]);
      const float dt = wave_sum(tile2[b * DEC_J + lane] + tile2[b * DEC_J + 64 + lane]);
      if (lane == 0) { a.part[((long)blockIdx.x * a.B + b) * 2] = le; a.part[((long)blockIdx.x * a.B + b) * 2 + 1] = dt; }
    }
  } else {
    float dwr[CD2 ? CD2 : DEC_MAXD2];
    _Pragma("unroll") for (int k = 0; k < D2; ++k) dwr[k] = 0.f;
    float dbj = 0.f;
    for (int bb = b0; bb < b1; bb += 4) {
      float bw[4];
      _Pragma("unroll") for (int u = 0; u < 4; ++u) bw[u] = (live && bb + u < b1) ? a.bow[(long)(bb + u) * a.V + j] : 0.f;
      _Pragma("unroll") for (int u = 0; u < 4; ++u) {
        const int b = bb + u;
        if (b < b1) {
          float gg = 0.f;
          if (live) {
            const float lp = dec_logit<CD2>(wr, zl + b * D2, D2, bias) - a.rowstat[b * 4] - a.rowstat[b * 4 + 1];
            const float p = expf(lp);
            const float tg = bw[u] * (1.f - a.ls) + a.ls / a.V;
            const float gp = (p - tg) / fmaxf((1.f - p) * p, 1e-12f);
            gg = p * (gp - a.rowstat[b * 4 + 2]) * a.gscale;
            _Pragma("unroll") for (int k = 0; k < D2; ++k) dwr[k] = fmaf(gg, zl[b * D2 + k], dwr[k]);
            dbj += gg;
          }
          tile[b * DEC_J + tj] = gg;
        }
      }
    }
    float* dwp = tile2;
    float* dbp = dwp + (G - 1) * DEC_J * ws;
    if (g > 0) {
      _Pragma("unroll") for (int k = 0; k < D2; ++k) dwp[((g - 1) * DEC_J + tj) * ws + k] = dwr[k];
      dbp[(g - 1) * DEC_J + tj] = dbj;
    }
    __syncthreads();
    if (g == 0 && live) {
      for (int q = 0; q < G - 1; ++q) {
        _Pragma("unroll") for (int k = 0; k < D2; ++k) dwr[k] += dwp[(q * DEC_J + tj) * ws + k];
        dbj += dbp[q * DEC_J + tj];
      }
      _Pragma("unroll") for (int k = 0; k < D2; ++k) a.dw[(long)j * D2 + k] = dwr[k];
      a.db[j] = dbj;
    }
    for (int e = t; e < a.B * D2; e += nthr) {
      const int b = e / D2, k = e - b * D2;
      const int nrow = min(DEC_J, a.V - j0);
      float s = 0.f;
      for (int jj = 0; jj < nrow; ++jj) s = fmaf(tile[b * DEC_J + jj], wl[jj * ws + k], s);
      a.dz_part[(long)blockIdx.x * a.B * D2 + e] = s;
    }
  }
}

__global__ __launch_bounds__(256) void decoder_combine_kernel(const float* __restrict__ part, int chunks, int B, int pass,
                                                              float* __restrict__ rowstat) {
  const int lane = threadIdx.x & 63;
  const int b = blockIdx.x * 4 + (threadIdx.x >> 6);
  if (b >= B) return;
  if (pass == 1) {
    float m = -INFINITY;
    for (int c = lane; c < chunks; c += 64) m = fmaxf(m, part[((long)c * B + b) * 2]);
    m = wave_max(m);
    float s = 0.f;
    for (int c = lane; c < chunks; c += 64) s += part[((long)c * B + b) * 2 + 1] * expf(part[((long)c * B + b) * 2] - m);
    s = wave_sum(s);
    if (lane == 0) { rowstat[b * 4] = m; rowstat[b * 4 + 1] = logf(s); }
  } else {
    float le = 0.f, dt = 0.f;
    for (int c = lane; c < chunks; c += 64) { le += part[((long)c * B + b) * 2]; dt += part[((long)c * B + b) * 2 + 1]; }
    le = wave_sum(le); dt = wave_sum(dt);
    if (lane == 0) { rowstat[b * 4 + 2] = dt; rowstat[b * 4 + 3] = le; }
  }
}
__global__ __launch_bounds__(256) void decoder_total_kernel(const float* __restrict__ rowstat, int B, float inv_bv, float* __restrict__ terms) {
  __shared__ float red[16];
  float tot = 0.f;
  for (int b = threadIdx.x; b < B; b += 256) tot += rowstat[b * 4 + 3];
  tot = block_sum(tot, red);
  if (threadIdx.x == 0) { terms[7] = tot * inv_bv; terms[8] = terms[0] + tot * inv_bv; }
}

__global__ __launch_bounds__(256) void reduce_parts16_kernel(const float* __restrict__ parts, float* __restrict__ out, int n, int nparts) {
  __shared__ float lds[256];
  const int cl = threadIdx.x & 15, rl = threadIdx.x >> 4;
  const int c = blockIdx.x * 16 + cl;
  float s = 0.f;
  if (c < n) for (int p = rl; p < nparts; p += 16) s += parts[(long)p * n + c];
  lds[threadIdx.x] = s;
  __syncthreads();
  if (rl == 0 && c < n) {
    float t = 0.f;
#pragma unroll
    for (int r = 0; r < 16; ++r) t += lds[r * 16 + cl];
    out[c] = t;
  }
}

__global__ __launch_bounds__(256) void tail_dlat_kernel(const float* __restrict__ dz_core, const float* __restrict__ dz_part, int chunks,
                                                        const float* __restrict__ dlat_direct, const float* __restrict__ lat,
                                                        const float* __restrict__ eps_e, const float* __restrict__ eps_c, int B, int D,
                                                        float gout, float* __restrict__ dlat) {
  const int e = blockIdx.x * 256 + threadIdx.x;
  if (e >= B * 2 * D) return;
  const int b = e / (2 * D), k = e - b * 2 * D;
  float g = dz_core[e];
  for (int c = 0; c < chunks; ++c) g += dz_part[(long)c * B * 2 * D + e];
  const int side = k >= D, kk = k - side * D;
  const float* row = lat + (long)b * 4 * D;
  const float ep = side ? eps_c[kk] : eps_e[kk];
  const float lv = row[(2 * side + 1) * D + kk];
  dlat[(long)b * 4 * D + 2 * side * D + kk] = (dlat_direct[(long)b * 4 * D + 2 * side * D + kk] + g) * gout;
  dlat[(long)b * 4 * D + (2 * side + 1) * D + kk] = (dlat_direct[(long)b * 4 * D + (2 * side + 1) * D + kk] + g * ep * expf(lv)) * gout;
}

__global__ __launch_bounds__(256) void sample_z_kernel(const float* __restrict__ lat, const float* __restrict__ eps_e,
                                                       const float* __restrict__ eps_c, int B, int D, float* __restrict__ z) {
  const int e = blockIdx.x * 256 + threadIdx.x;
  if (e >= B * 2 * D) return;
  const int b = e / (2 * D), k = e - b * 2 * D;
  const float* row = lat + (long)b * 4 * D;
  z[e] = (k < D) ? row[k] + eps_e[k] * expf(row[D + k]) : row[2 * D + (k - D)] + eps_c[k - D] * expf(row[3 * D + (k - D)]);
}

__global__ __launch_bounds__(256) void pair_prob_kernel(const float* __restrict__ lat, const float* __restrict__ eps_e,
                                                        const float* __restrict__ eps_c, const float* __restrict__ w,
                                                        const float* __restrict__ bias, int B, int D, float* __restrict__ prob) {
  const int b = blockIdx.x * 256 + threadIdx.x;
  if (b >= B) return;
  const float* row = lat + (long)b * 4 * D;
  float s = bias[0];
  for (int k = 0; k < D; ++k) {
    s = fmaf(w[k], row[k] + eps_e[k] * expf(row[D + k]), s);
    s = fmaf(w[D + k], row[2 * D + k] + eps_c[k] * expf(row[3 * D + k]), s);
  }
  prob[b] = 1.0f / (1.0f + expf(-s));
}

constexpr int TT_R = 64;
constexpr int TT_THREADS = 256;
constexpr int TT_MAX_B = 1024;
constexpr int TT_MAX_SLABS = TT_MAX_B / TT_R;
constexpr int TT_MAX_NHW = 8 * 32 + 8 + 32 + 1 + 64 + 1;

struct TailTiled {
  TailCore c;
  float* lg;
  float* spart;
  float* hpart;
};

template <int PHASE>
__global__ __launch_bounds__(TT_THREADS) void tail_heads_kernel(TailTiled q) {
  const TailCore& a = q.c;
  extern __shared__ __attribute__((aligned(16))) char smem_raw[];
  float* red = (float*)smem_raw;
  const int B = a.B, D = a.D, D2 = 2 * a.D, D4 = 4 * a.D;
  float* zl = red + 64;
  float* mlt = zl + TT_R * D2;
  float* lg = mlt + TT_R * D4;
  float* elog = lg + TT_R * 16;
  float* gx = elog + TT_R * 8;
  float* hw = gx + TT_R * 2;
  const int n_emo = a.EC * D;
  const int o_eb = n_emo, o_cw = o_eb + a.EC, o_cb = o_cw + D, o_pw = o_cb + 1, o_pb = o_pw + D2, n_hw = o_pb + 1;
  const int t = threadIdx.x;
  const int r0 = blockIdx.x * TT_R, nr = min(TT_R, B - r0);
  const int nslab = gridDim.x;

  for (int e = t; e < nr * D2; e += TT_THREADS) zl[e] = a.z[(long)r0 * D2 + e];
  for (int e = t; e < nr * D4; e += TT_THREADS) {
    const int b = r0 + e / D4, k = e % D4;
    mlt[e] = k < D ? dropout_mult(a.d_emo, b * D + k) : (k < D2 ? dropout_mult(a.d_cau, b * D + (k - D)) : dropout_mult(a.d_pair, b * D2 + (k - D2)));
  }
  for (int e = t; e < n_hw; e += TT_THREADS)
    hw[e] = e < o_eb ? a.emo_w[e] : e < o_cw ? a.emo_b[e - o_eb] : e < o_cb ? a.cau_w[e - o_cw] : e < o_pw ? a.cau_b[0]
          : e < o_pb ? a.pair_w[e - o_pw] : a.pair_b[0];
  if (PHASE == 2) for (int e = t; e < nr * 16; e += TT_THREADS) lg[e] = q.lg[(long)r0 * 16 + e];
  __syncthreads();
  if (PHASE == 1) {
    for (int e = t; e < nr * 16; e += TT_THREADS) {
      const int b = e >> 4, h = e & 15;
      float s = 0.f;
      if (h < a.EC) {
        s = hw[o_eb + h];
        for (int k = 0; k < D; ++k) s = fmaf(hw[h * D + k], zl[b * D2 + k] * mlt[b * D4 + k], s);
      } else if (h == a.EC) {
        s = hw[o_cb];
        for (int k = 0; k < D; ++k) s = fmaf(hw[o_cw + k], zl[b * D2 + D + k] * mlt[b * D4 + D + k], s);
      } else if (h == a.EC + 1) {
        s = hw[o_pb];
        for (int k = 0; k < D2; ++k) s = fmaf(hw[o_pw + k], zl[b * D2 + k] * mlt[b * D4 + D2 + k], s);
      }
      lg[e] = s;
      q.lg[(long)r0 * 16 + e] = s;
    }
  }
  float ysum = 0.f;
  for (int b = t; b < B; b += TT_THREADS) ysum += a.pair_labels[b];
  ysum = block_sum(ysum, red);
  const float ntot = a.label_sum_override ? a.n_override : (float)B;
  float ytot = ysum;
  if (a.label_sum_override) {
    ytot = a.label_sum_override[0];
    for (int r = 1; r < a.label_sum_ranks; ++r) ytot += a.label_sum_override[(long)r * a.rank_stride];
// ... 196 lines not shown
              le = -(tg * fmaxf(lp, -100.f) + (1.f - tg) * fmaxf(log1pf(-p), -100.f));
              dt = p * ((p - tg) / fmaxf((1.f - p) * p, 1e-12f));
            }
            tile[lb * DEC_J + tj] = le; tile2[lb * DEC_J + tj] = dt;
          }
        }
      }
      __syncthreads();
      for (int lb = wv; lb < nb; lb += nwv) {
        const float le = wave_sum(tile[lb * DEC_J + lane] + tile[lb * DEC_J + 64 + lane]);
        const float dt = wave_sum(tile2[lb * DEC_J + lane] + tile2[lb * DEC_J + 64 + lane]);
        if (lane == 0) { a.part[((long)blockIdx.x * a.B + t0 + lb) * 2] = le; a.part[((long)blockIdx.x * a.B + t0 + lb) * 2 + 1] = dt; }
      }
    }
  } else {
    float dwr[CD2 ? CD2 : DEC_MAXD2];
    _Pragma("unroll") for (int k = 0; k < D2; ++k) dwr[k] = 0.f;
    float dbj = 0.f;
    for (int t0 = 0; t0 < a.B; t0 += TB) {
      const int nb = min(TB, a.B - t0);
      const int lb1 = min(nb, lb0 + Rg);
      __syncthreads();
      for (int e = t; e < nb * D2; e += NTHR) zl[e] = a.z[(long)t0 * D2 + e];
      __syncthreads();
      for (int bb = lb0; bb < lb1; bb += 4) {
        float bw[4];
        _Pragma("unroll") for (int u = 0; u < 4; ++u) bw[u] = (live && bb + u < lb1) ? a.bow[(long)(t0 + bb + u) * a.V + j] : 0.f;
        _Pragma("unroll") for (int u = 0; u < 4; ++u) {
          const int lb = bb + u;
          if (lb < lb1) {
            float gg = 0.f;
            if (live) {
              const float lp = dec_logit<CD2>(wr, zl + lb * D2, D2, bias) - a.rowstat[(t0 + lb) * 4] - a.rowstat[(t0 + lb) * 4 + 1];
              const float p = expf(lp);
              const float tg = bw[u] * (1.f - a.ls) + a.ls / a.V;
              const float gp = (p - tg) / fmaxf((1.f - p) * p, 1e-12f);
              gg = p * (gp - a.rowstat[(t0 + lb) * 4 + 2]) * a.gscale;
              _Pragma("unroll") for (int k = 0; k < D2; ++k) dwr[k] = fmaf(gg, zl[lb * D2 + k], dwr[k]);
              dbj += gg;
            }
            tile[lb * DEC_J + tj] = gg;
          }
        }
      }
      __syncthreads();
      for (int e = t; e < nb * D2; e += NTHR) {
        const int lb = e / D2, k = e - lb * D2;
        float s = 0.f;
        for (int jj = 0; jj < nrow; ++jj) s = fmaf(tile[lb * DEC_J + jj], wl[jj * ws + k], s);
        a.dz_part[((long)blockIdx.x * a.B + t0) * D2 + e] = s;
      }
    }
    for (int p = 1; p < G; ++p) {
      __syncthreads();
      if (g == p) {
        _Pragma("unroll") for (int k = 0; k < D2; ++k) wl[tj * ws + k] = dwr[k];
        tile[tj] = dbj;
      }
      __syncthreads();
      if (g == 0) {
        _Pragma("unroll") for (int k = 0; k < D2; ++k) dwr[k] += wl[tj * ws + k];
        dbj += tile[tj];
      }
    }
    if (g == 0 && live) {
      _Pragma("unroll") for (int k = 0; k < D2; ++k) a.dw[(long)j * D2 + k] = dwr[k];
      a.db[j] = dbj;
    }
  }
}

}

using namespace carel;

static size_t align_up(size_t x) { return (x + 63) & ~(size_t)63; }
constexpr int MMD_MAX_BLOCKS = 1024;
constexpr size_t TAIL_LDS_MAX = 160 * 1024;

struct TailWork {
  float* dz_core; float* dlat_direct; float* dlat; float* dpooled; float* dpre; float* part; float* rowstat; float* dz_part;
  float* dcls; float* dgpart; float* pair_dead; float* mmd_part; float* dz_mmd;
  float* tt_lg; float* tt_spart; float* tt_hpart;
  size_t total;
};
static TailWork carve(float* base, int B, int D, int V) {
  TailWork w; size_t o = 0;
  const int chunks = (V + DEC_J - 1) / DEC_J;
  auto take = [&](size_t n) { float* p = base ? base + o : nullptr; o += align_up(n); return p; };
  w.dz_core = take((size_t)B * 2 * D); w.dlat_direct = take((size_t)B * 4 * D); w.dlat = take((size_t)B * 4 * D);
  w.dpooled = take((size_t)B * TH); w.dpre = take((size_t)B * TH); w.part = take((size_t)chunks * B * 2);
  w.rowstat = take((size_t)B * 4); w.dz_part = take((size_t)chunks * B * 2 * D); w.dcls = take((size_t)B * TH);
  w.dgpart = take((size_t)((TH + DG_CHUNK - 1) / DG_CHUNK) * B * TH);
  w.pair_dead = take(16);
  w.mmd_part = take(4 * MMD_MAX_BLOCKS); w.dz_mmd = take((size_t)B * 2 * D);
  w.tt_lg = take((size_t)B * 16); w.tt_spart = take((size_t)TT_MAX_SLABS * 8); w.tt_hpart = take((size_t)TT_MAX_SLABS * TT_MAX_NHW);
  w.total = o;
  return w;
}

extern "C" int64_t carel_tail_workspace_floats(int32_t batch, int32_t ec_dim, int32_t bow_dim) {
  return (int64_t)carve(nullptr, batch, ec_dim, bow_dim).total;
}

static int tail_check(const carel_tail_args* a, const char* who) {
  if (!a) return set_error(CAREL_ERR_ARG, "%s: null args", who);
  if (a->hidden != TH) return set_error(CAREL_ERR_SHAPE, "%s: hidden must be %d", who, TH);
  if (a->batch < 1 || a->seq_len < 1) return set_error(CAREL_ERR_SHAPE, "%s: bad batch/seq_len", who);
  if (a->ec_dim < 1 || a->ec_dim > 32 || a->e_classes < 1 || a->e_classes > 8)
    return set_error(CAREL_ERR_SHAPE, "%s: ec_dim must be <= 32 and e_num_class <= 8", who);
  if (!a->x_last_f32 || !a->pooler_w || !a->pooler_b || !a->pooled || !a->lat)
    return set_error(CAREL_ERR_ARG, "%s: null tensor", who);
  for (int i = 0; i < 4; ++i) if (!a->head_w[i] || !a->head_b[i]) return set_error(CAREL_ERR_ARG, "%s: null latent head", who);
  return CAREL_OK;
}

extern "C" int carel_tail_latents(const carel_tail_args* a, void* stream_) {
  hipStream_t stream = (hipStream_t)stream_;
  int rc = tail_check(a, "carel_tail_latents");
  if (rc) return rc;
  auto sample_groups = [&](int ncols) { int g = (4096 + ncols - 1) / ncols;       const int mx = (a->batch + 3) / 4; g = g > mx ? mx : g; return g < 1 ? 1 : g; };
  const int N = 4 * a->ec_dim;
  if (a->head_in_f32) {
    const int N2 = 2 * a->ec_dim;
    for (int side = 0; side < 2; ++side) {
      PtrSet4 hp; for (int i = 0; i < 4; ++i) { hp.w[i] = nullptr; hp.b[i] = nullptr; }
      for (int i = 0; i < 2; ++i) { hp.w[i] = (const float*)a->head_w[2 * side + i]; hp.b[i] = (const float*)a->head_b[2 * side + i]; }
      hipLaunchKernelGGL(rowvec_linear_kernel<0>, dim3((N2 + 3) / 4, sample_groups(N2)), dim3(256), 0, stream,
                         (const float*)a->head_in_f32 + (long)side * a->batch * TH, (long)TH, (const int*)nullptr, a->batch, N2, a->ec_dim, hp,
                         (float*)a->lat + side * N2, (long)N);
    }
  } else {
    PtrSet4 pp; for (int i = 0; i < 4; ++i) { pp.w[i] = nullptr; pp.b[i] = nullptr; }
    pp.w[0] = (const float*)a->pooler_w; pp.b[0] = (const float*)a->pooler_b;
    hipLaunchKernelGGL(rowvec_linear_kernel<1>, dim3(TH / 4, sample_groups(TH)), dim3(256), 0, stream, (const float*)a->x_last_f32,
                       (long)a->seq_len * TH, (const int*)a->cls_rows, a->batch, TH, TH, pp, (float*)a->pooled, (long)TH);
    PtrSet4 hp; for (int i = 0; i < 4; ++i) { hp.w[i] = (const float*)a->head_w[i]; hp.b[i] = (const float*)a->head_b[i]; }
    hipLaunchKernelGGL(rowvec_linear_kernel<0>, dim3((N + 3) / 4, sample_groups(N)), dim3(256), 0, stream, (const float*)a->pooled, (long)TH,
                       (const int*)nullptr, a->batch, N, a->ec_dim, hp, (float*)a->lat, (long)N);
  }
  if (a->eps_e && a->eps_c && a->z)
    hipLaunchKernelGGL(sample_z_kernel, dim3((a->batch * 2 * a->ec_dim + 255) / 256), dim3(256), 0, stream, (const float*)a->lat,
                       (const float*)a->eps_e, (const float*)a->eps_c, a->batch, a->ec_dim, (float*)a->z);
  return check_launch("tail latents");
}

extern "C" int carel_pair_probs(const void* lat, const void* eps_e, const void* eps_c, const void* pair_w, const void* pair_b,
                                int32_t batch, int32_t ec_dim, void* prob, void* stream_) {
  hipStream_t stream = (hipStream_t)stream_;
  if (!lat || !eps_e || !eps_c || !pair_w || !pair_b || !prob || batch < 1) return set_error(CAREL_ERR_ARG, "carel_pair_probs: bad arguments");
  hipLaunchKernelGGL(pair_prob_kernel, dim3((batch + 255) / 256), dim3(256), 0, stream, (const float*)lat, (const float*)eps_e,
                     (const float*)eps_c, (const float*)pair_w, (const float*)pair_b, batch, ec_dim, (float*)prob);
  return check_launch("pair_prob_kernel");
}

static size_t tail_core_lds_bytes(int B, int D, int EC, int nm) {
  const int n_hw = EC * D + EC + D + 1 + 2 * D + 1;
  return sizeof(float) * (64 + 64 + (size_t)2 * B * 2 * D + (size_t)B * 8 + (size_t)B * 2 + (size_t)B * 4 * D + (size_t)B * 16 +
                          ((n_hw + 3) & ~3) + ((2 * nm + 3) & ~3) + (size_t)2 * nm * (D | 1) + 2 * (size_t)B);
}
struct DecPlan { int G; size_t lds1, lds2, lds3, ldsmax; };
static DecPlan tail_decoder_plan(int B, int D) {
  DecPlan p;
  const size_t lds0 = sizeof(float) * ((size_t)B * 2 * D + 16 + (size_t)DEC_J * (2 * D + 1) + (size_t)B * DEC_J);
  int G = DEC_MAXG;
  auto lds3_of = [&](int g) { return lds0 + sizeof(float) * (size_t)(g - 1) * DEC_J * (2 * D + 2); };
  while (G > 1 && (lds3_of(G) > TAIL_LDS_MAX || (B + G - 1) / G < 4)) G >>= 1;
  p.G = G; p.lds1 = lds0; p.lds2 = lds0 + sizeof(float) * (size_t)B * DEC_J; p.lds3 = lds3_of(G);
  p.ldsmax = p.lds2 > p.lds3 ? p.lds2 : p.lds3;
  return p;
}

extern "C" int32_t carel_tail_batch_limit(int32_t ec_dim, int32_t e_classes) {
  if (ec_dim < 1 || ec_dim > 32 || e_classes < 1 || e_classes > 8 || 2 * ec_dim > DEC_MAXD2) return 0;
  int B = 1;
  while (tail_core_lds_bytes(B + 1, ec_dim, e_classes, B + 1) <= TAIL_LDS_MAX && tail_decoder_plan(B + 1, ec_dim).ldsmax <= TAIL_LDS_MAX) ++B;
  return B >= 2 ? B : 0;
}

static int tail_losses_prepare(const carel_tail_args* a, const char* who, TailCore& c, TailWork& w) {
  int rc = tail_check(a, who);
  if (rc) return rc;
  const int B = a->batch, D = a->ec_dim, V = a->bow_dim;
  if (V < 1) return set_error(CAREL_ERR_SHAPE, "%s: bow_dim must be positive", who);
  if (2 * D > DEC_MAXD2) return set_error(CAREL_ERR_SHAPE, "%s: 2*ec_dim must be <= %d", who, DEC_MAXD2);
  if (B < 2 && !a->z_global) return set_error(CAREL_ERR_SHAPE, "%s: batch must be >= 2 (MMD divides by n(n-1))", who);
  if (!a->emo_w || !a->emo_b || !a->cau_w || !a->cau_b || !a->pair_w || !a->pair_b || !a->dec_w || !a->dec_b ||
      !a->emo_labels || !a->cau_labels || !a->pair_labels || !a->bow || !a->eps_e || !a->eps_c || !a->z || !a->terms ||
      !a->work || !a->d_emo_w || !a->d_emo_b || !a->d_cau_w || !a->d_cau_b || !a->d_pair_w || !a->d_pair_b || !a->d_dec_w ||
      !a->d_dec_b)
    return set_error(CAREL_ERR_ARG, "%s: null tensor", who);
  w = carve((float*)a->work, B, D, V);
  c.B = B; c.D = D; c.EC = a->e_classes; c.lat = (const float*)a->lat; c.eps_e = (const float*)a->eps_e; c.eps_c = (const float*)a->eps_c;
  c.emo_w = (const float*)a->emo_w; c.emo_b = (const float*)a->emo_b; c.cau_w = (const float*)a->cau_w; c.cau_b = (const float*)a->cau_b;
  c.pair_w = (const float*)a->pair_w; c.pair_b = (const float*)a->pair_b;
  c.emo_labels = (const long*)a->emo_labels; c.cau_labels = (const float*)a->cau_labels; c.pair_labels = (const float*)a->pair_labels;
  c.w_mmd = a->w_mmd; c.w_emo = a->w_emo; c.w_cau = a->w_cau; c.w_pair = a->w_pair; c.kl_w = a->kl_weight; c.ls = a->label_smoothing;
  c.dis_mode = a->dis_mode; c.emo_bce = a->emo_bce;
  if (c.dis_mode < 0 || c.dis_mode > 2) return set_error(CAREL_ERR_ARG, "%s: dis_mode must be 0 (MMD), 1 (HSIC) or 2 (none)", who);
  if (c.emo_bce && a->e_classes != 1) return set_error(CAREL_ERR_ARG, "%s: the BCE emotion head has exactly one logit", who);
  if (c.dis_mode == 1 && a->z_global) return set_error(CAREL_ERR_ARG, "%s: HSIC has no global-batch mode", who);
  c.d_emo = make_dropout(a->drop_seed, 100u, a->drop_p, a->drop_row_offset * (uint32_t)D);
  c.d_cau = make_dropout(a->drop_seed, 101u, a->drop_p, a->drop_row_offset * (uint32_t)D);
  c.d_pair = make_dropout(a->drop_seed, 102u, a->drop_p, a->drop_row_offset * (uint32_t)(2 * D));
  c.alpha = a->mmd_alpha; c.mmd_eps = a->mmd_eps;
  c.label_sum_override = (const float*)a->global_label_sum; c.n_override = (float)a->global_n;
  c.label_sum_ranks = a->global_label_ranks > 1 ? a->global_label_ranks : 1;
  if (c.label_sum_ranks > 1 && a->global_rank_stride <= 0)
    return set_error(CAREL_ERR_ARG, "%s: global_label_ranks > 1 needs global_rank_stride", who);
  c.z_global = (const float*)a->z_global; c.n_global = a->global_n; c.row_offset = a->global_row_offset;
  c.rank_stride = a->global_rank_stride > 0 ? a->global_rank_stride : B * 2 * D;
  if (c.z_global && a->global_rank_stride > 0 && (a->global_rank_stride < B * 2 * D || c.n_global % B))
    return set_error(CAREL_ERR_ARG, "%s: global_rank_stride needs global_n to be a multiple of batch and stride >= batch*2*ec_dim", who);
  c.mmd_grad_scale = a->mmd_grad_scale > 0.f ? a->mmd_grad_scale : 1.f;
  if (c.z_global && (c.n_global < 2 || c.row_offset < 0 || c.row_offset + B > c.n_global))
    return set_error(CAREL_ERR_ARG, "%s: inconsistent global batch description", who);
  c.z = (float*)a->z; c.terms = (float*)a->terms; c.dz = w.dz_core; c.dlat_direct = w.dlat_direct;
  c.d_emo_w = (float*)a->d_emo_w; c.d_emo_b = (float*)a->d_emo_b; c.d_cau_w = (float*)a->d_cau_w; c.d_cau_b = (float*)a->d_cau_b;
  c.d_pair_w = (float*)a->d_pair_w; c.d_pair_b = (float*)a->d_pair_b; c.pair_dead = w.pair_dead;
  c.mmd_part = nullptr; c.mmd_nblk = 0; c.dz_mmd = nullptr; c.prof = nullptr;
  return CAREL_OK;
}

extern "C" int carel_tail_losses(const carel_tail_args* a, void* stream_) {
  hipStream_t stream = (hipStream_t)stream_;
  TailCore c; TailWork w;
  int rc = tail_losses_prepare(a, "carel_tail_losses", c, w);
  if (rc) return rc;
  const int B = a->batch, D = a->ec_dim, V = a->bow_dim;
  const int nm = (c.z_global && c.dis_mode != 0) ? c.n_global : B;
  const size_t lds = tail_core_lds_bytes(B, D, a->e_classes, nm);
  if (lds > TAIL_LDS_MAX) return set_error(CAREL_ERR_SHAPE, "carel_tail_losses: batch too large for the single-workgroup tail (%zu B LDS)", lds);
  if (lds > 64 * 1024) {
    hipError_t e = hipFuncSetAttribute((const void*)tail_core_kernel, hipFuncAttributeMaxDynamicSharedMemorySize, (int)lds);
    if (e != hipSuccess) return set_error(CAREL_ERR_HIP, "carel_tail_losses: hipFuncSetAttribute: %s", hipGetErrorString(e));
  }
  const int chunks = (V + DEC_J - 1) / DEC_J;
  const DecPlan dp = tail_decoder_plan(B, D);
  const int G = dp.G;
  const size_t lds1 = dp.lds1, lds2 = dp.lds2, lds3 = dp.lds3, ldsmax = dp.ldsmax;
  if (ldsmax > TAIL_LDS_MAX) return set_error(CAREL_ERR_SHAPE, "carel_tail_losses: batch too large for the decoder kernel (%zu B LDS)", ldsmax);
  if (ldsmax > 64 * 1024) {
    hipError_t e = hipSuccess;
    const void* fns[6] = {(const void*)decoder_kernel<1, 48>, (const void*)decoder_kernel<2, 48>, (const void*)decoder_kernel<3, 48>,
                          (const void*)decoder_kernel<1, 0>, (const void*)decoder_kernel<2, 0>, (const void*)decoder_kernel<3, 0>};
    for (int i = 0; i < 6 && e == hipSuccess; ++i) e = hipFuncSetAttribute(fns[i], hipFuncAttributeMaxDynamicSharedMemorySize, (int)ldsmax);
    if (e != hipSuccess) return set_error(CAREL_ERR_HIP, "carel_tail_losses: hipFuncSetAttribute: %s", hipGetErrorString(e));
  }
  c.mmd_part = nullptr; c.mmd_nblk = 0; c.dz_mmd = nullptr;
  if (c.z_global && c.dis_mode == 0 && (2 * c.n_global + 31) / 32 > MMD_MAX_BLOCKS)
    return set_error(CAREL_ERR_SHAPE, "carel_tail_losses: global batch too large for the MMD partial buffer");
  hipStream_t core_stream = stream;
  TailEvents* tev = nullptr;
  auto join_on_error = [&](int code) -> int {
    if (tev && core_stream != stream) {
      (void)hipEventRecord(tev->join, core_stream);
      (void)hipStreamWaitEvent(stream, tev->join, 0);
    }
    return code;
  };
  if (g_tail_overlap && !a->serial && !g_tail_prof) {
    hipStream_t side = (hipStream_t)carel_side_stream(0);
    tev = side ? tail_events() : nullptr;
    if (tev) {
      hipLaunchKernelGGL(sample_z_kernel, dim3((B * 2 * D + 255) / 256), dim3(256), 0, stream, c.lat, c.eps_e, c.eps_c, B, D, c.z);
      if (hipEventRecord(tev->fork, stream) != hipSuccess || hipStreamWaitEvent(side, tev->fork, 0) != hipSuccess)
        return set_error(CAREL_ERR_HIP, "carel_tail_losses: event fork failed");
      core_stream = side;
      c.z = nullptr;
    }
  }
  if (c.z_global && c.dis_mode == 0) {
    MmdGlobalArgs g;
    g.zg = c.z_global; g.n = c.n_global; g.B = B; g.D = D; g.rank_stride = c.rank_stride; g.row_offset = c.row_offset;
    g.alpha = c.alpha; g.eps = c.mmd_eps; g.gscale = -c.w_mmd * c.mmd_grad_scale; g.part = w.mmd_part; g.dz = w.dz_mmd;
    const int nblk = (2 * c.n_global + 31) / 32;
    if (D == 24) hipLaunchKernelGGL(mmd_global_kernel<24>, dim3(nblk), dim3(256), 0, core_stream, g);
    else hipLaunchKernelGGL(mmd_global_kernel<32>, dim3(nblk), dim3(256), 0, core_stream, g);
    if ((rc = check_launch("mmd_global_kernel"))) return join_on_error(rc);
    c.mmd_part = w.mmd_part; c.mmd_nblk = nblk; c.dz_mmd = w.dz_mmd;
  }
  c.prof = g_tail_prof;
  hipLaunchKernelGGL(tail_core_kernel, dim3(1), dim3(1024), lds, core_stream, c);
  if ((rc = check_launch("tail_core_kernel"))) return join_on_error(rc);
  if (tev && hipEventRecord(tev->join, core_stream) != hipSuccess) return join_on_error(set_error(CAREL_ERR_HIP, "carel_tail_losses: event record failed"));

  DecArgs d;
  d.B = B; d.D2 = 2 * D; d.V = V; d.z = (const float*)a->z; d.w = (const float*)a->dec_w; d.b = (const float*)a->dec_b;
  d.bow = (const float*)a->bow; d.ls = a->label_smoothing; d.part = w.part; d.rowstat = w.rowstat; d.dz_part = w.dz_part;
  d.dw = (float*)a->d_dec_w; d.db = (float*)a->d_dec_b; d.gscale = 1.0f / ((float)B * (float)V);
#define DEC_LAUNCH(PASS, LDS)                                                                              \
  do {                                                                                                  \
    if (2 * D == 48) hipLaunchKernelGGL((decoder_kernel<PASS, 48>), dim3(chunks), dim3(DEC_J * G), LDS, stream, d); \
    else hipLaunchKernelGGL((decoder_kernel<PASS, 0>), dim3(chunks), dim3(DEC_J * G), LDS, stream, d);      \
  } while (0)
  DEC_LAUNCH(1, lds1);
  hipLaunchKernelGGL(decoder_combine_kernel, dim3((B + 3) / 4), dim3(256), 0, stream, (const float*)w.part, chunks, B, 1, w.rowstat);
  DEC_LAUNCH(2, lds2);
  hipLaunchKernelGGL(decoder_combine_kernel, dim3((B + 3) / 4), dim3(256), 0, stream, (const float*)w.part, chunks, B, 2, w.rowstat);
  DEC_LAUNCH(3, lds3);
#undef DEC_LAUNCH
  if ((rc = check_launch("decoder kernels"))) return join_on_error(rc);
  hipLaunchKernelGGL(reduce_parts16_kernel, dim3((B * 2 * D + 15) / 16), dim3(256), 0, stream, (const float*)w.dz_part, w.dz_part, B * 2 * D, chunks);
  if (tev && hipStreamWaitEvent(stream, tev->join, 0) != hipSuccess) return join_on_error(set_error(CAREL_ERR_HIP, "carel_tail_losses: event join failed"));
  hipLaunchKernelGGL(decoder_total_kernel, dim3(1), dim3(256), 0, stream, (const float*)w.rowstat, B, d.gscale, (float*)a->terms);
  hipLaunchKernelGGL(tail_dlat_kernel, dim3((B * 2 * D + 255) / 256), dim3(256), 0, stream, (const float*)w.dz_core, (const float*)w.dz_part,
                     1, (const float*)w.dlat_direct, (const float*)a->lat, (const float*)a->eps_e, (const float*)a->eps_c, B, D, 1.0f, w.dlat);
  return check_launch("tail_dlat_kernel");
}

extern "C" int carel_tail_losses_tiled(const carel_tail_args* a, void* stream_) {
  hipStream_t stream = (hipStream_t)stream_;
  const char* who = "carel_tail_losses_tiled";
  if (!a) return set_error(CAREL_ERR_ARG, "%s: null args", who);
  if (a->batch > TT_MAX_B) return set_error(CAREL_ERR_SHAPE, "%s: batch must be <= %d; got %d", who, TT_MAX_B, a->batch);
  TailTiled q; TailWork w;
  TailCore& c = q.c;
  int rc = tail_losses_prepare(a, who, c, w);
  if (rc) return rc;
  const int B = a->batch, D = a->ec_dim, V = a->bow_dim;
  if (c.dis_mode == 1)
    return set_error(CAREL_ERR_SHAPE, "%s: HSIC (dis_mode 1) keeps the single-workgroup limit of carel_tail_losses: batch <= %d at ec_dim %d, "
                     "e_classes %d; got %d", who, (int)carel_tail_batch_limit(D, a->e_classes), D, a->e_classes, B);
  const int nm = c.z_global ? c.n_global : B;
  const int nblk = (2 * nm + 31) / 32;
  if (c.dis_mode == 0 && nblk > MMD_MAX_BLOCKS) return set_error(CAREL_ERR_SHAPE, "%s: global batch too large for the MMD partial buffer", who);
  const int nslab = (B + TT_R - 1) / TT_R;
  const int n_hw = a->e_classes * D + a->e_classes + D + 1 + 2 * D + 1;
  const size_t lds_h = sizeof(float) * (64 + (size_t)TT_R * (2 * D + 4 * D + 16 + 8 + 2) + ((n_hw + 3) & ~3));
  const int D2 = 2 * D, chunks = (V + DEC_J - 1) / DEC_J;
  auto dec_lds = [&](int tb, int tiles) { return sizeof(float) * ((size_t)tb * D2 + ((DEC_J * (D2 + 1) + 3) & ~3) + (size_t)tiles * tb * DEC_J); };
  const int TB = dec_lds(32, 2) <= 64 * 1024 ? 32 : 16;
  if (lds_h > 64 * 1024 || dec_lds(TB, 2) > 64 * 1024 || nslab > TT_MAX_SLABS || n_hw > TT_MAX_NHW)
    return set_error(CAREL_ERR_SHAPE, "%s: internal tile plan does not fit (ec_dim %d, e_classes %d)", who, D, a->e_classes);
  const int ntile = (B + TB - 1) / TB;
  q.lg = w.tt_lg; q.spart = w.tt_spart; q.hpart = w.tt_hpart;

  hipLaunchKernelGGL(sample_z_kernel, dim3((B * 2 * D + 255) / 256), dim3(256), 0, stream, c.lat, c.eps_e, c.eps_c, B, D, c.z);
  if (c.dis_mode == 0) {
    MmdGlobalArgs g;
    g.zg = c.z_global ? c.z_global : (const float*)c.z; g.n = nm; g.B = B; g.D = D;
    g.rank_stride = c.z_global ? c.rank_stride : B * 2 * D; g.row_offset = c.z_global ? c.row_offset : 0;
    g.alpha = c.alpha; g.eps = c.mmd_eps; g.gscale = -c.w_mmd * c.mmd_grad_scale; g.part = w.mmd_part; g.dz = w.dz_mmd;
    if (D == 24) hipLaunchKernelGGL(mmd_global_kernel<24>, dim3(nblk), dim3(256), 0, stream, g);
    else hipLaunchKernelGGL(mmd_global_kernel<32>, dim3(nblk), dim3(256), 0, stream, g);
    if ((rc = check_launch("mmd_global_kernel"))) return rc;
    c.mmd_part = w.mmd_part; c.mmd_nblk = nblk; c.dz_mmd = w.dz_mmd;
  }
  hipLaunchKernelGGL(tail_heads_kernel<1>, dim3(nslab), dim3(TT_THREADS), lds_h, stream, q);
  hipLaunchKernelGGL(tail_heads_kernel<2>, dim3(nslab), dim3(TT_THREADS), lds_h, stream, q);
  hipLaunchKernelGGL(tail_head_grads_kernel, dim3(1), dim3(TT_THREADS), 0, stream, q, nslab);
  if ((rc = check_launch("tail_heads_kernel"))) return rc;

  DecArgs d;
  d.B = B; d.D2 = D2; d.V = V; d.z = (const float*)a->z; d.w = (const float*)a->dec_w; d.b = (const float*)a->dec_b;
  d.bow = (const float*)a->bow; d.ls = a->label_smoothing; d.part = w.part; d.rowstat = w.rowstat; d.dz_part = w.dz_part;
  d.dw = (float*)a->d_dec_w; d.db = (float*)a->d_dec_b; d.gscale = 1.0f / ((float)B * (float)V);
#define DEC_TILED_LAUNCH(PASS, GRID, LDS)                                                                                         \
  do {                                                                                                                         \
    if (D2 == 48) hipLaunchKernelGGL((decoder_tiled_kernel<PASS, 48>), GRID, dim3(DEC_J * DEC_MAXG), LDS, stream, d, TB);          \
    else hipLaunchKernelGGL((decoder_tiled_kernel<PASS, 0>), GRID, dim3(DEC_J * DEC_MAXG), LDS, stream, d, TB);                    \
  } while (0)
  DEC_TILED_LAUNCH(1, dim3(chunks, ntile), dec_lds(TB, 1));
  hipLaunchKernelGGL(decoder_combine_kernel, dim3((B + 3) / 4), dim3(256), 0, stream, (const float*)w.part, chunks, B, 1, w.rowstat);
  DEC_TILED_LAUNCH(2, dim3(chunks, ntile), dec_lds(TB, 2));
  hipLaunchKernelGGL(decoder_combine_kernel, dim3((B + 3) / 4), dim3(256), 0, stream, (const float*)w.part, chunks, B, 2, w.rowstat);
  DEC_TILED_LAUNCH(3, dim3(chunks), dec_lds(TB, 1));
#undef DEC_TILED_LAUNCH
  if ((rc = check_launch("decoder kernels (tiled)"))) return rc;
  hipLaunchKernelGGL(reduce_parts16_kernel, dim3((B * 2 * D + 15) / 16), dim3(256), 0, stream, (const float*)w.dz_part, w.dz_part, B * 2 * D, chunks);
  hipLaunchKernelGGL(decoder_total_kernel, dim3(1), dim3(256), 0, stream, (const float*)w.rowstat, B, d.gscale, (float*)a->terms);
  hipLaunchKernelGGL(tail_dlat_kernel, dim3((B * 2 * D + 255) / 256), dim3(256), 0, stream, (const float*)w.dz_core, (const float*)w.dz_part,
                     1, (const float*)w.dlat_direct, (const float*)a->lat, (const float*)a->eps_e, (const float*)a->eps_c, B, D, 1.0f, w.dlat);
  return check_launch("tail_dlat_kernel");
}

extern "C" int carel_scale_f32(void* x, int64_t n, const void* scale_dev, void* stream_) {
  hipStream_t stream = (hipStream_t)stream_;
  if (!x || !scale_dev || n <= 0) return set_error(CAREL_ERR_ARG, "carel_scale_f32: bad arguments");
  long blocks = (n + 255) / 256; if (blocks > 2048) blocks = 2048;
  hipLaunchKernelGGL(scale_inplace_kernel, dim3((unsigned)blocks), dim3(256), 0, stream, (float*)x, (long)n, (const float*)scale_dev);
  return check_launch("scale_inplace_kernel");
}

__global__ void bow_scatter_kernel(const int* __restrict__ rows, const int* __restrict__ cols, const float* __restrict__ vals, int nnz,
                                   float* __restrict__ out, int B, int V) {
  const int i = blockIdx.x * blockDim.x + threadIdx.x;
  if (i >= nnz) return;
  const int r = rows[i], c = cols[i];
  if (r >= 0 && r < B && c >= 0 && c < V) out[(long)r * V + c] = vals[i];
}
extern "C" int carel_bow_expand(const void* trip, int32_t nnz, void* out, int32_t B, int32_t V, void* stream_) {
  hipStream_t stream = (hipStream_t)stream_;
  if (!out || B < 1 || V < 1 || nnz < 0 || (nnz > 0 && !trip)) return set_error(CAREL_ERR_ARG, "carel_bow_expand: bad arguments");
  hipError_t e = hipMemsetAsync(out, 0, (size_t)B * V * 4, stream);
  if (e != hipSuccess) return set_error(CAREL_ERR_HIP, "carel_bow_expand: memset: %s", hipGetErrorString(e));
  if (nnz == 0) return CAREL_OK;
  const int* rows = (const int*)trip;
  hipLaunchKernelGGL(bow_scatter_kernel, dim3((nnz + 255) / 256), dim3(256), 0, stream, rows, rows + nnz, (const float*)(rows + 2 * (long)nnz), nnz,
                     (float*)out, B, V);
  return check_launch("bow_scatter_kernel");
}

extern "C" int64_t carel_tail_pair_dead_offset(int32_t batch, int32_t ec_dim, int32_t bow_dim) {
  TailWork w = carve((float*)nullptr + 1, batch, ec_dim, bow_dim);
  return (int64_t)(w.pair_dead - ((float*)nullptr + 1));
}

extern "C" int carel_tail_profile(void* dev_i64_x16) { g_tail_prof = (long long*)dev_i64_x16; return CAREL_OK; }

extern "C" int carel_tail_backward(const carel_tail_args* a, const void* grad_out_dev, void* stream_) {
  return carel_tail_backward_dz(a, grad_out_dev, nullptr, stream_);
}

__global__ __launch_bounds__(256) void tail_add_dz_kernel(const float* __restrict__ dz, const float* __restrict__ lat,
                                                          const float* __restrict__ eps_e, const float* __restrict__ eps_c, int B, int D,
                                                          float* __restrict__ dlat) {
  const int e = blockIdx.x * 256 + threadIdx.x;
  if (e >= B * 2 * D) return;
  const int b = e / (2 * D), k = e - b * 2 * D, side = k >= D, kk = k - side * D;
  const float g = dz[e];
  const float ep = side ? eps_c[kk] : eps_e[kk];
  const float lv = lat[(long)b * 4 * D + (2 * side + 1) * D + kk];
  dlat[(long)b * 4 * D + 2 * side * D + kk] += g;
  dlat[(long)b * 4 * D + (2 * side + 1) * D + kk] += g * ep * expf(lv);
}

extern "C" int carel_tail_backward_dz(const carel_tail_args* a, const void* grad_out_dev, const void* dz_extra, void* stream_) {
  hipStream_t stream = (hipStream_t)stream_;
  int rc = tail_check(a, "carel_tail_backward");
  if (rc) return rc;
  if (!a->work || !a->dx_last_f32 || !a->d_pooler_w || !a->d_pooler_b) return set_error(CAREL_ERR_ARG, "carel_tail_backward: null tensor");
  const int B = a->batch, D = a->ec_dim, N = 4 * D;
  TailWork w = carve((float*)a->work, B, D, a->bow_dim);
  if (grad_out_dev) {
    hipLaunchKernelGGL(scale_inplace_kernel, dim3((B * N + 255) / 256), dim3(256), 0, stream, w.dlat, (long)B * N, (const float*)grad_out_dev);
  }
  if (dz_extra) {
    if (!a->lat || !a->eps_e || !a->eps_c) return set_error(CAREL_ERR_ARG, "carel_tail_backward_dz: lat / eps needed");
    hipLaunchKernelGGL(tail_add_dz_kernel, dim3((B * 2 * D + 255) / 256), dim3(256), 0, stream, (const float*)dz_extra, (const float*)a->lat,
                       (const float*)a->eps_e, (const float*)a->eps_c, B, D, w.dlat);
  }
  const int hc = (N + DG_CHUNK - 1) / DG_CHUNK, pc = (TH + DG_CHUNK - 1) / DG_CHUNK;
  const long bt = (long)B * TH;
  if (a->head_in_f32) {
    if (!a->d_head_in_f32) return set_error(CAREL_ERR_ARG, "carel_tail_backward: head_in_f32 needs d_head_in_f32");
    const int N2 = 2 * D, hc2 = (N2 + DG_CHUNK - 1) / DG_CHUNK;
    for (int side = 0; side < 2; ++side) {
      PtrSet4 hp; OutSet4 ho;
      for (int i = 0; i < 4; ++i) { hp.w[i] = nullptr; hp.b[i] = nullptr; ho.w[i] = nullptr; ho.b[i] = nullptr; }
      for (int i = 0; i < 2; ++i) { hp.w[i] = (const float*)a->head_w[2 * side + i]; ho.w[i] = (float*)a->d_head_w[2 * side + i]; ho.b[i] = (float*)a->d_head_b[2 * side + i]; }
      const float* hin = (const float*)a->head_in_f32 + side * bt;
      if (ho.w[0] && ho.w[1])
        hipLaunchKernelGGL(rowvec_wgrad_kernel, dim3((N2 + 3) / 4), dim3(256), 0, stream, (const float*)w.dlat + side * N2, (long)N, hin,
                           (long)TH, (const int*)nullptr, B, N2, D, ho);
      hipLaunchKernelGGL(rowvec_dgrad_kernel<0>, dim3((B + 3) / 4, hc2), dim3(256), 0, stream, (const float*)w.dlat + side * N2, (long)N, B, N2, D, hp,
                         (const float*)nullptr, (float*)nullptr, w.dgpart);
      hipLaunchKernelGGL(sum_parts_kernel, dim3((unsigned)((bt / 4 + 255) / 256)), dim3(256), 0, stream, (const float*)w.dgpart,
                         (float*)a->d_head_in_f32 + side * bt, bt, hc2);
    }
    (void)hipMemsetAsync(a->d_pooler_w, 0, (size_t)TH * TH * sizeof(float), stream);
    (void)hipMemsetAsync(a->d_pooler_b, 0, (size_t)TH * sizeof(float), stream);
    return check_launch("tail backward (adapter heads)");
  }
  PtrSet4 hp; OutSet4 ho;
  for (int i = 0; i < 4; ++i) { hp.w[i] = (const float*)a->head_w[i]; hp.b[i] = nullptr; ho.w[i] = (float*)a->d_head_w[i]; ho.b[i] = (float*)a->d_head_b[i]; }
  if (ho.w[0] && ho.w[1] && ho.w[2] && ho.w[3])
    hipLaunchKernelGGL(rowvec_wgrad_kernel, dim3((N + 3) / 4), dim3(256), 0, stream, (const float*)w.dlat, (long)N, (const float*)a->pooled,
                       (long)TH, (const int*)nullptr, B, N, D, ho);
  hipLaunchKernelGGL(rowvec_dgrad_kernel<0>, dim3((B + 3) / 4, hc), dim3(256), 0, stream, (const float*)w.dlat, (long)N, B, N, D, hp,
                     (const float*)nullptr, (float*)nullptr, w.dgpart);
  hipLaunchKernelGGL(sum_parts_kernel, dim3((unsigned)((bt / 4 + 255) / 256)), dim3(256), 0, stream, (const float*)w.dgpart, w.dpooled, bt, hc);
  PtrSet4 pp; OutSet4 po;
  for (int i = 0; i < 4; ++i) { pp.w[i] = nullptr; pp.b[i] = nullptr; po.w[i] = nullptr; po.b[i] = nullptr; }
  pp.w[0] = (const float*)a->pooler_w; po.w[0] = (float*)a->d_pooler_w; po.b[0] = (float*)a->d_pooler_b;
  hipLaunchKernelGGL(rowvec_dgrad_kernel<1>, dim3((B + 3) / 4, pc), dim3(256), 0, stream, (const float*)w.dpooled, (long)TH, B, TH, TH, pp,
                     (const float*)a->pooled, w.dpre, w.dgpart);
  hipLaunchKernelGGL(sum_parts_kernel, dim3((unsigned)((bt / 4 + 255) / 256)), dim3(256), 0, stream, (const float*)w.dgpart, w.dcls, bt, pc);
  hipLaunchKernelGGL(rowvec_wgrad_kernel, dim3(TH / 4), dim3(256), 0, stream, (const float*)w.dpre, (long)TH, (const float*)a->x_last_f32,
                     (long)a->seq_len * TH, (const int*)a->cls_rows, B, TH, TH, po);
  const size_t dx_rows = a->n_rows > 0 ? (size_t)a->n_rows : (size_t)B * a->seq_len;
  (void)hipMemsetAsync(a->dx_last_f32, 0, dx_rows * TH * sizeof(float), stream);
  hipLaunchKernelGGL(scatter_cls_kernel, dim3(B), dim3(256), 0, stream, (const float*)w.dcls, B, a->seq_len, (const int*)a->cls_rows,
                     (float*)a->dx_last_f32);
  return check_launch("tail backward");
}
```

carel_vae_amd/drl_classifier.py:

```python
import ctypes as C
import math
import os
from types import SimpleNamespace

import numpy as np
import torch
import torch.nn as nn

from . import _lib as L
from . import ops

H, I_FF, NH = 768, 3072, 12

DEFAULT_OPT = dict(language="zh", max_len=128, e_num_class=6, c_num_class=1, pair_num_class=1, ec_dim=24, bert_dim=768,
                   kl_ann_iterations=20000, epochs=20, batch_size=64, ec_kl_lambda=0.03, label_smoothing=0.1,
                   mmd_loss_weight=30.0, emo_mul_loss_weight=10.0, cau_mul_loss_weight=10.0, pair_mul_loss_weight=30.0,
                   dropout=0.5, epsilon=1e-8, vae_lr=1e-5, aprx_lr=0.003, pair_bow_dim=23771, self_iteration=50, self_epochs=10,
                   self_strategy="random", best_model_path="ECPE_model/best_cause_pair_model", model_id="carel")


def make_opt(**kw):
    d = dict(DEFAULT_OPT)
    d.update(kw)
    return SimpleNamespace(**d)
# ... 849 lines not shown

    def _grad_view(self, k):
        p = self._named[k]
        o = self._offs[k]
        return self._flat_grad[o:o + p.numel()].view(p.shape)

    def _adapter_weights(self):
        out = []
        for side in ("emotion", "cause"):
            m = getattr(self, side + "_adapter")
            if self.adapter == "raw":
                w, b = m.in_proj_weight.data, m.in_proj_bias.data
                out.append(dict(q_w=w[:H], q_b=b[:H], k_w=w[H:2 * H], v_w=w[2 * H:], v_b=b[2 * H:], o_w=m.out_proj.weight.data,
                                o_b=m.out_proj.bias.data))
            else:
                out.append(dict(q_w=m.q_proj.weight.data, q_b=m.q_proj.bias.data, k_w=m.k_proj.weight.data))
        return out

    def _adapter_grads(self):
        out = []
        for side in ("emotion", "cause"):
            g = lambda n: self._grad_view("%s_adapter.%s" % (side, n))
            if self.adapter == "raw":
                w, b = g("in_proj_weight"), g("in_proj_bias")
                out.append(dict(d_q_w=w[:H], d_q_b=b[:H], d_k_w=w[H:2 * H], d_k_b=b[H:2 * H], d_v_w=w[2 * H:], d_v_b=b[2 * H:],
                                d_o_w=g("out_proj.weight"), d_o_b=g("out_proj.bias")))
            else:
                out.append(dict(d_q_w=g("q_proj.weight"), d_q_b=g("q_proj.bias"), d_k_w=g("k_proj.weight"), d_k_b=g("k_proj.bias")))
        return out

    def _adapter_forward(self, c, x_last_ptr):
        dev = self._flat.device
        G = self.head_number if self.adapter == "raw" else 1
        key = ("adapter", c.B, c.S)
        buf = self._ws.get(key)
        if buf is None:
            buf = self._ws[key] = ops.AdapterBuffers(c.B, c.S, G, dev)
        qs = [getattr(self, n).to(dev, torch.float32).reshape(-1).contiguous() for n in ("emotion_q", "cause_q")]
        if qs[0].numel() != H or qs[1].numel() != H:
            raise L.CarelError("emotion_q / cause_q must hold 768 values")
        u = self._ws.get("adapter_u")
        if u is None:
            u = self._ws["adapter_u"] = torch.empty((2, G, H), device=dev, dtype=torch.float32)
        a = ops.adapter_args(self.adapter, G, qs, self._adapter_weights(), u, buf, c.Bp, x=SimpleNamespace(data_ptr=lambda: x_last_ptr))
        ops.adapter_build_u(a)
        ops.adapter_forward(a)
        return a, buf

    def _run_forward(self, c, training):
        if self._adam_hook is not None:
            self._adam_hook._join()
        self._refresh_shadow()
        train_drop = self.training
        lib = L.load()
        st = L.current_stream()
        if self.debug_fp32:
            if training:
                raise L.CarelError("debug_fp32 is a forward-only measurement mode: call forward_terms() / forward() under torch.no_grad()")
            train_drop = False
            c.pack, c.cls, ws = None, None, None
            ea, x_f32 = self._run_encoder_fp32(c)
            x_last_ptr = x_f32.data_ptr()
        else:
            ws = self._workspace(c.Bp, c.S, inference=not training)
            c.cls = self._cls_info(c.B, c.Bp, c.S, c.pack, self._flat.device)
            ea = self._encoder_args(c.ids, c.att, c.tt, ws, c.Bp, c.S, not training, train_drop, c.seed, c.row_offset, c.pack, c.cls)
            L.check(lib.carel_encoder_forward(C.byref(ea), st), "carel_encoder_forward")
            x_last_ptr = lib.carel_encoder_x_last(C.byref(ea))
        W, G = self._tail_weights()
        xl = SimpleNamespace(data_ptr=lambda: x_last_ptr)
        c.ad = None
        head_in = d_head_in = None
        if self.adapter != "false":
            c.ad, abuf = self._adapter_forward(c, x_last_ptr)
            head_in, d_head_in = abuf.out, abuf.d_out
        klw = ops.kl_anneal_weight(c.iteration, self.opt)
        drop = (self.opt.dropout if train_drop else 0.0, c.seed, c.row_offset)
        if c.cls is not None:
            cls_rows, n_rows = c.cls.compact, c.cls.n_cls
        else:
            cls_rows, n_rows = (None, c.Bp * c.S) if c.pack is None else (c.pack.cu, c.pack.n_tokens)
        ta = ops.tail_args(c.buf, xl, W, c.labels, c.eps_e, c.eps_c, self.opt, klw, grads=G, drop=drop, cls_rows=cls_rows, n_rows=n_rows,
                           head_in=head_in, d_head_in=d_head_in)
        ops.tail_latents(ta)
        if self._dp is not None:
            self._dp.fill_global(ta, c)
        ta.serial = 0 if self.overlap_wgrad else 1
        ops.tail_losses(ta)
        if self._gan:
            c.gan_terms = self._gan_disc(c, drop)
        c.ea, c.ta, c.ws = ea, ta, ws
        c.keep = (W, G, xl)

    def _gan_disc(self, c, drop):
        key = ("gan_terms", c.B, c.S)
        terms = self._ws.get(key)
        if terms is None:
            terms = self._ws[key] = torch.zeros(8, device=self._flat.device, dtype=torch.float32)

        def img(i, k):
            o = self._offs[k] - self._disc_lo
            return self._disc_img[i][o:o + self._named[k].numel()]
        w = [self._named[g + ".weight"].data for g in GAN_DISCS]
        b = [self._named[g + ".bias"].data for g in GAN_DISCS]
        ops.gan_disc(c.buf.z, c.labels["emo_f"], c.labels["cau"], w, b, self.opt, terms,
                     [img(0, g + ".weight") for g in GAN_DISCS], [img(0, g + ".bias") for g in GAN_DISCS],
                     [img(1, g + ".weight") for g in GAN_DISCS], [img(1, g + ".bias") for g in GAN_DISCS],
                     drop=drop, vae_loss_in=c.buf.terms[8:9])
        return terms

    def _group_has_grad(self, g):
        if g == "vae":
            return self._named["encoder.embeddings.word_embeddings.weight"].grad is not None
        return all(self._named[g + t].grad is not None for t in (".weight", ".bias"))

    def _run_backward_gan(self, c, grads):
        f32 = torch.float32
        if self._grad_views is None:
            self._grad_views = {k: self._grad_view(k) for k in self._order}

        def share(group, image, g_dev):
            lo, hi = self._group_ranges[group]
            ops.axpy_(self._flat_grad[lo:hi], self._disc_img[image][lo - self._disc_lo:hi - self._disc_lo], g_dev, self._group_has_grad(group))
            for t in (".weight", ".bias"):
                self._named[group + t].grad = self._grad_views[group + t]

        for i, group in enumerate(GAN_DISCS):
            if grads[i] is not None:
                share(group, 0, grads[i].to(f32).reshape(1).contiguous())
        if grads[2] is not None:
            go = grads[2].to(f32).reshape(1).contiguous()
            w = float(self.opt.ecce_adv_loss_weight)
            ge = go if w == 1.0 else go * w
            for group in GAN_DISCS:
                share(group, 1, ge)
            self._run_backward(c, go, None)

    def _run_backward(self, c, grad_out, grad_z=None):
        lib = L.load()
        st = L.current_stream()
        named = self._named
        first = named[self._order[0]]
        accumulate = first.grad is not None
        prev = self._flat_grad.clone() if accumulate else None
        if accumulate and self._gan:
            prev[self._disc_lo:self._disc_hi].zero_()
        go = grad_out.to(torch.float32).reshape(1).contiguous()
        ea = c.ea
        ea.dx = c.buf.dx_last.data_ptr()
        ops.tail_backward(c.ta, go, None if grad_z is None else grad_z.to(torch.float32).contiguous())
        if c.ad is not None:
            c.ad.dx_f32 = ea.dx
            ops.adapter_backward(c.ad)
            if self._adapter_train_names:
                ops.adapter_backward_weights(c.ad, ops.adapter_wgrad_args(self._ws[("adapter", c.B, c.S)], self._adapter_grads()))
        lo = self._offs["decoder.weight"]
        ops.scale_(self._flat_grad[lo:self._pair_hi], go)
        if self._dp is not None:
            self._dp.tail_done()
        self._backward_encoder(ea, accumulate)
        if c.ad is not None:
            e = "encoder.embeddings."
            self._grad_view(e + "word_embeddings.weight")[self.cfg.pad_id].zero_()
            if self.cfg.roberta:
                self._grad_view(e + "position_embeddings.weight")[self.cfg.pad_id].zero_()
        if self._dp is not None:
            self._dp.backward_done(None if accumulate else self._adam_hook)
# ... 282 lines not shown
```

Before: 8394.

## Merge tail decoder passes and backward kernels, replace memset+scatter with expand_rows

Fuses the decoder's z sampling and per-pass combine reductions into the decoder kernels. It also folds the final reduce, total and dlat steps into a single close kernel. In the tail backward, the grad scaling and partial-sum reductions are folded into the rowvec kernels, and the memset plus scatter of dx is replaced by a kernel that writes every row once. The encoder's CLS-only backward likewise swaps two memsets and two scatters for one expand_rows kernel. The aim is fewer launches and fewer full-buffer passes, at the cost of redundant per-block combine work and more complex kernels.

```diff
diff --git a/carel_vae_amd/csrc/carel_hip_internal.h b/carel_vae_amd/csrc/carel_hip_internal.h
--- a/carel_vae_amd/csrc/carel_hip_internal.h
+++ b/carel_vae_amd/csrc/carel_hip_internal.h
@@ -29,9 +29,12 @@
 void encoder_wgrad_group_enable(int on);
 void adam_grid_cap(long cap);
 void tail_overlap_enable(int on);
+void tail_merged_enable(int on);
+void encoder_cls_expand_enable(int on);
 int gemm_pp_init_device(int device);
 int gather_rows(const void* in_f32, const void* in_bf16, const void* idx, int n, void* out_f32, void* out_bf16, hipStream_t stream);
 int scatter_rows(const void* in_f32, const void* in_bf16, const void* idx, int n, void* out_f32, void* out_bf16, hipStream_t stream);
+int expand_rows(const void* in_f32, const void* in_bf16, const void* idx, int n, int64_t rows, void* out_f32, void* out_bf16, hipStream_t stream);
 
 int layernorm_bwd_rows(const void* dy, const void* h, const void* stats, const void* gamma, int64_t rows, uint32_t drop_seed, uint32_t drop_site,
                        uint32_t drop_idx_offset, float drop_p, const void* drop_row_map, void* dh_f32, void* dy_bf16, void* partials,
diff --git a/carel_vae_amd/csrc/encoder.hip b/carel_vae_amd/csrc/encoder.hip
--- a/carel_vae_amd/csrc/encoder.hip
+++ b/carel_vae_amd/csrc/encoder.hip
@@ -157,6 +157,7 @@
 int ln_slab_fusion_enabled() { return g_ln_slab_fusion; }
 CAREL_TUNABLE(int, g_wgrad_group, 1);
 int wgrad_group_enabled() { return g_wgrad_group; }
+CAREL_TUNABLE(int, g_cls_expand, 1);
 CAREL_TUNABLE(int, g_ln_resid, 1);
 int ln_resid_enabled() { return g_ln_resid; }
 struct GemmCall { carel_gemm_args g; int flags; };
@@ -210,7 +211,7 @@
   const ScratchLayout sl = scratch_layout(batch, seq_len);
   return which == 0 ? (int64_t)sl.ws_bytes : which == 1 ? (int64_t)sl.slab_bytes : -1;
 }
-namespace carel { void encoder_ln_resid_enable(int on) { g_ln_resid = on ? 1 : 0; } void encoder_wgrad_group_enable(int on) { g_wgrad_group = on ? 1 : 0; }
+namespace carel { void encoder_cls_expand_enable(int on) { g_cls_expand = on ? 1 : 0; } void encoder_ln_resid_enable(int on) { g_ln_resid = on ? 1 : 0; } void encoder_wgrad_group_enable(int on) { g_wgrad_group = on ? 1 : 0; }
                   void encoder_ln_slab_fusion_enable(int on) { g_ln_slab_fusion = on ? 1 : 0; } }
 #endif
 
@@ -503,11 +504,15 @@
   if ((rc = gemm_run(gemm_fill(s.dyb2, w.out_w, EH, EH, (int)R, EH, EH, CAREL_GEMM_NN, CAREL_EPI_BIAS_BF16, 1, dctx_rows, nullptr, nullptr, nullptr,
                                nullptr, nullptr, 0, 0, 0, 0.f, nullptr, nullptr, s.ws, ws_bytes, 1 | (cls_only ? GEMM_EX_FIXED_ROWS : 0)), stream))) return rc;
   if (cls_only) {
-    hipError_t he = hipMemsetAsync(s.dctx, 0, (size_t)T * EH * 2, (hipStream_t)stream);
-    if (he == hipSuccess) he = hipMemsetAsync(a->dx, 0, (size_t)T * EH * 4, (hipStream_t)stream);
-    if (he != hipSuccess) return set_error(CAREL_ERR_HIP, "carel_encoder_backward_layer: memset: %s", hipGetErrorString(he));
-    if ((rc = scatter_rows(nullptr, s.dqkv, a->cls_rows, (int)R, nullptr, s.dctx, (hipStream_t)stream))) return rc;
-    if ((rc = scatter_rows(s.dy, nullptr, a->cls_rows, (int)R, a->dx, nullptr, (hipStream_t)stream))) return rc;
+    if (g_cls_expand) {
+      if ((rc = expand_rows(s.dy, s.dqkv, a->cls_rows, (int)R, T, a->dx, s.dctx, (hipStream_t)stream))) return rc;
+    } else {
+      hipError_t he = hipMemsetAsync(s.dctx, 0, (size_t)T * EH * 2, (hipStream_t)stream);
+      if (he == hipSuccess) he = hipMemsetAsync(a->dx, 0, (size_t)T * EH * 4, (hipStream_t)stream);
+      if (he != hipSuccess) return set_error(CAREL_ERR_HIP, "carel_encoder_backward_layer: memset: %s", hipGetErrorString(he));
+      if ((rc = scatter_rows(nullptr, s.dqkv, a->cls_rows, (int)R, nullptr, s.dctx, (hipStream_t)stream))) return rc;
+      if ((rc = scatter_rows(s.dy, nullptr, a->cls_rows, (int)R, a->dx, nullptr, (hipStream_t)stream))) return rc;
+    }
   }
   const void* dh1_full = cls_only ? (const void*)a->dx : (const void*)s.dy;
   carel_attn_args at;
diff --git a/carel_vae_amd/csrc/gemm.hip b/carel_vae_amd/csrc/gemm.hip
--- a/carel_vae_amd/csrc/gemm.hip
+++ b/carel_vae_amd/csrc/gemm.hip
@@ -781,6 +781,7 @@
   if (v >= 220 && v <= 225) { gemm_tri_enable(v - 220); return CAREL_OK; }
   if (v >= 280 && v <= 292) { adam_grid_cap(32L << (v - 280)); return CAREL_OK; }
   if (v == 210 || v == 211) { tail_overlap_enable(v - 210); return CAREL_OK; }
+  if (v == 350 || v == 351) { tail_merged_enable(v - 350); encoder_cls_expand_enable(v - 350); return CAREL_OK; }
   if (v == 200 || v == 201) { gemm_pp_pair_enable(v - 200); return CAREL_OK; }
   if (v == 170 || v == 171) { gemm_pp_epi_prefetch(v - 170); return CAREL_OK; }
   if (v == 120 || v == 121) { gemm_pp_xcd_rect(v - 120); return CAREL_OK; }
diff --git a/carel_vae_amd/csrc/ln.hip b/carel_vae_amd/csrc/ln.hip
--- a/carel_vae_amd/csrc/ln.hip
+++ b/carel_vae_amd/csrc/ln.hip
@@ -470,6 +470,48 @@
   }
 }
 
+constexpr int XR_ROWS = 16;
+__global__ __launch_bounds__(256) void expand_rows_kernel(const float* __restrict__ in_f, const bf16_t* __restrict__ in_b,
+                                                          const int* __restrict__ idx, int n, long rows, float* __restrict__ out_f,
+                                                          bf16_t* __restrict__ out_b) {
+  __shared__ int owner[XR_ROWS];
+  const int lane = threadIdx.x & 63, wv = threadIdx.x >> 6;
+  const long r0 = (long)blockIdx.x * XR_ROWS;
+  if (threadIdx.x < XR_ROWS) owner[threadIdx.x] = -1;
+  __syncthreads();
+  for (int i = threadIdx.x; i < n; i += 256) {
+    const long r = idx[i];
+    if (r >= r0 && r < r0 + XR_ROWS) owner[r - r0] = i;
+  }
+  __syncthreads();
+  for (int q = wv; q < XR_ROWS; q += 4) {
+    const long r = r0 + q;
+    if (r >= rows) break;
+    const int i = owner[q];
+    if (out_f) {
+      Row X;
+      if (i >= 0) X = load_row(in_f + (long)i * H, lane);
+      else for (int v = 0; v < NV; ++v) X.v[v] = float4{0.f, 0.f, 0.f, 0.f};
+      store_row(out_f + r * H, lane, X);
+    }
+    if (out_b) {
+#pragma unroll
+      for (int v = 0; v < NV; ++v) {
+        const int c = (v * 64 + lane) * 4;
+        uint2 x = {0u, 0u};
+        if (i >= 0) x = *(const uint2*)(in_b + (long)i * H + c);
+        *(uint2*)(out_b + r * H + c) = x;
+      }
+    }
+  }
+}
+int expand_rows(const void* in_f32, const void* in_bf16, const void* idx, int n, int64_t rows, void* out_f32, void* out_bf16, hipStream_t stream) {
+  if (rows < 1) return CAREL_OK;
+  hipLaunchKernelGGL(expand_rows_kernel, dim3((unsigned)((rows + XR_ROWS - 1) / XR_ROWS)), dim3(256), 0, stream, (const float*)in_f32,
+                     (const bf16_t*)in_bf16, (const int*)idx, n, (long)rows, in_f32 ? (float*)out_f32 : nullptr, in_bf16 ? (bf16_t*)out_bf16 : nullptr);
+  return check_launch("expand_rows_kernel");
+}
+
 int gather_rows(const void* in_f32, const void* in_bf16, const void* idx, int n, void* out_f32, void* out_bf16, hipStream_t stream) {
   hipLaunchKernelGGL(gather_rows_kernel, dim3((n + 3) / 4), dim3(256), 0, stream, (const float*)in_f32, (const bf16_t*)in_bf16,
                      (const int*)idx, n, (float*)out_f32, (bf16_t*)out_bf16);
diff --git a/carel_vae_amd/csrc/rowvec_device.h b/carel_vae_amd/csrc/rowvec_device.h
--- a/carel_vae_amd/csrc/rowvec_device.h
+++ b/carel_vae_amd/csrc/rowvec_device.h
@@ -50,7 +50,8 @@
 
 struct OutSet4 { float* w[4]; float* b[4]; };
 static __global__ __launch_bounds__(256) void rowvec_wgrad_kernel(const float* __restrict__ dY, long dy_stride, const float* __restrict__ X,
-                                                           long x_stride, const int* __restrict__ row_idx, int B, int N, int seg, OutSet4 os) {
+                                                           long x_stride, const int* __restrict__ row_idx, int B, int N, int seg, OutSet4 os,
+                                                           const float* __restrict__ dy_scale = nullptr) {
   const int lane = threadIdx.x & 63;
   const int n = blockIdx.x * 4 + (threadIdx.x >> 6);
   if (n >= N) return;
@@ -58,6 +59,7 @@
 #pragma unroll
   for (int i = 0; i < TNV; ++i) acc[i] = float4{0.f, 0.f, 0.f, 0.f};
   float sb = 0.f;
+  const float dys = dy_scale ? dy_scale[0] : 1.f;
   constexpr int U = 8;
   for (int b = 0; b < B; b += U) {
     float g[U]; float4 xv[U][TNV];
@@ -65,6 +67,7 @@
     for (int u = 0; u < U; ++u) {
       const int bb = min(b + u, B - 1);
       g[u] = (b + u < B) ? dY[(long)bb * dy_stride + n] : 0.f;
+      if (dy_scale) g[u] = __fmul_rn(g[u], dys);
       const float* x = row_idx ? X + (long)row_idx[bb] * TH : X + (long)bb * x_stride;
 #pragma unroll
       for (int i = 0; i < TNV; ++i) xv[u][i] = *(const float4*)(x + (i * 64 + lane) * 4);
@@ -89,7 +92,8 @@
 template <int MODE>
 __global__ __launch_bounds__(256) void rowvec_dgrad_kernel(const float* __restrict__ dY, long dy_stride, int B, int N, int seg,
                                                            PtrSet4 ps, const float* __restrict__ y, float* __restrict__ dpre,
-                                                           float* __restrict__ part) {
+                                                           float* __restrict__ part, int dy_parts = 1, long dy_part_stride = 0,
+                                                           const float* __restrict__ dy_scale = nullptr) {
   const int lane = threadIdx.x & 63;
   const int b = blockIdx.x * 4 + (threadIdx.x >> 6);
   if (b >= B) return;
@@ -97,19 +101,27 @@
 #pragma unroll
   for (int i = 0; i < TNV; ++i) acc[i] = float4{0.f, 0.f, 0.f, 0.f};
   const int n0 = blockIdx.y * DG_CHUNK, n1 = min(N, n0 + DG_CHUNK);
+  const float dys = dy_scale ? dy_scale[0] : 1.f;
+  float gl = 0.f;
+  if (n0 + lane < n1) {
+    const int n = n0 + lane;
+    gl = dY[(long)b * dy_stride + n];
+    for (int p = 1; p < dy_parts; ++p) gl += dY[p * dy_part_stride + (long)b * dy_stride + n];
+    if (dy_scale) gl = __fmul_rn(gl, dys);
+    if (MODE == 1) {
+      const float yy = y[(long)b * N + n];
+      gl *= (1.0f - yy * yy);
+      dpre[(long)b * N + n] = gl;
+    }
+  }
   constexpr int U = 8;
   for (int nb = n0; nb < n1; nb += U) {
     float g[U]; float4 wv[U][TNV];
 #pragma unroll
     for (int u = 0; u < U; ++u) {
       const int n = min(nb + u, n1 - 1);
-      float gg = (nb + u < n1) ? dY[(long)b * dy_stride + n] : 0.f;
-      if (MODE == 1) {
-        const float yy = y[(long)b * N + n];
-        gg *= (1.0f - yy * yy);
-        if (lane == 0 && nb + u < n1) dpre[(long)b * N + n] = gg;
-      }
-      g[u] = gg;
+      const float gs = __shfl(gl, n - n0, 64);
+      g[u] = (nb + u < n1) ? gs : 0.f;
       const float* w = ps.w[n / seg] + (long)(n % seg) * TH;
 #pragma unroll
       for (int i = 0; i < TNV; ++i) wv[u][i] = *(const float4*)(w + (i * 64 + lane) * 4);
@@ -152,5 +164,37 @@
   for (int k = threadIdx.x; k < TH; k += 256) dx[row * TH + k] = dcls[(long)b * TH + k];
 }
 
-
-}
+static __global__ __launch_bounds__(256) void tail_dx_kernel(const float* __restrict__ part, long n, int nparts, int B, int S,
+                                                             const int* __restrict__ row_idx, long rows, float* __restrict__ dx) {
+  __shared__ int owner;
+  const long r = blockIdx.x;
+  if (threadIdx.x == 0) owner = -1;
+  __syncthreads();
+  for (int b = threadIdx.x; b < B; b += 256) {
+    const long row = row_idx ? (long)row_idx[b] : (long)b * S;
+    if (row == r) owner = b;
+  }
+  __syncthreads();
+  const int b = owner;
+  if (threadIdx.x >= TH / 4) return;
+  float4 a = float4{0.f, 0.f, 0.f, 0.f};
+  if (b >= 0) {
+    const float* src = part + (long)b * TH + threadIdx.x * 4;
+    a = *(const float4*)src;
+    int p = 1;
+    for (; p + 8 <= nparts; p += 8) {
+      float4 c[8];
+#pragma unroll
+      for (int u = 0; u < 8; ++u) c[u] = *(const float4*)(src + (long)(p + u) * n);
+#pragma unroll
+      for (int u = 0; u < 8; ++u) { a.x += c[u].x; a.y += c[u].y; a.z += c[u].z; a.w += c[u].w; }
+    }
+    for (; p < nparts; ++p) {
+      const float4 c = *(const float4*)(src + (long)p * n);
+      a.x += c.x; a.y += c.y; a.z += c.z; a.w += c.w;
+    }
+  }
+  *(float4*)(dx + r * TH + threadIdx.x * 4) = a;
+}
+
+}
diff --git a/carel_vae_amd/csrc/tail.hip b/carel_vae_amd/csrc/tail.hip
--- a/carel_vae_amd/csrc/tail.hip
+++ b/carel_vae_amd/csrc/tail.hip
@@ -115,8 +115,10 @@
 
 static long long* g_tail_prof = nullptr;
 CAREL_TUNABLE(int, g_tail_overlap, 1);
+CAREL_TUNABLE(int, g_tail_merged, 1);
 #ifdef CAREL_EXPERIMENTS
 void tail_overlap_enable(int on) { g_tail_overlap = on ? 1 : 0; }
+void tail_merged_enable(int on) { g_tail_merged = on ? 1 : 0; }
 #endif
 struct TailEvents { hipEvent_t fork, join; bool ok; };
 static TailEvents* tail_events() {
@@ -379,7 +381,67 @@
   float* dz_part;
   float* dw; float* db;
   float gscale;
+  const float* lat; const float* eps_e; const float* eps_c;
+  float* z_out;
+  float* part2;
+  int chunks;
 };
+
+__device__ __forceinline__ float tail_sample_z(const float* __restrict__ lat, const float* __restrict__ eps_e, const float* __restrict__ eps_c,
+                                               int D, int b, int k) {
+  const float* row = lat + (long)b * 4 * D;
+  return (k < D) ? row[k] + eps_e[k] * expf(row[D + k]) : row[2 * D + (k - D)] + eps_c[k - D] * expf(row[3 * D + (k - D)]);
+}
+
+template <int WHICH>
+__device__ __forceinline__ void dec_combine_rows(const float* __restrict__ part, int chunks, int B, float* rs, int rss, float* __restrict__ out) {
+  constexpr int R = 8;
+  const int lane = threadIdx.x & 63, wv = threadIdx.x >> 6, nwv = blockDim.x >> 6;
+  const float2* __restrict__ p2 = (const float2*)part;
+  for (int r0 = wv * R; r0 < B; r0 += nwv * R) {
+    float x[R], y[R];
+    if (WHICH == 1) {
+      _Pragma("unroll") for (int u = 0; u < R; ++u) x[u] = -INFINITY;
+      for (int c = lane; c < chunks; c += 64) {
+        _Pragma("unroll") for (int u = 0; u < R; ++u) { const int b = min(r0 + u, B - 1); x[u] = fmaxf(x[u], p2[(long)b * chunks + c].x); }
+      }
+      _Pragma("unroll") for (int u = 0; u < R; ++u) { x[u] = wave_max(x[u]); y[u] = 0.f; }
+      for (int c = lane; c < chunks; c += 64) {
+        float2 v[R];
+        _Pragma("unroll") for (int u = 0; u < R; ++u) { const int b = min(r0 + u, B - 1); v[u] = p2[(long)b * chunks + c]; }
+        _Pragma("unroll") for (int u = 0; u < R; ++u) y[u] += v[u].y * expf(v[u].x - x[u]);
+      }
+      _Pragma("unroll") for (int u = 0; u < R; ++u) y[u] = wave_sum(y[u]);
+      if (lane == 0) {
+        _Pragma("unroll") for (int u = 0; u < R; ++u) {
+          const int b = r0 + u;
+          if (b < B) {
+            const float ll = logf(y[u]);
+            rs[b * rss] = x[u]; rs[b * rss + 1] = ll;
+            if (out) { out[b * 4] = x[u]; out[b * 4 + 1] = ll; }
+          }
+        }
+      }
+    } else {
+      _Pragma("unroll") for (int u = 0; u < R; ++u) { x[u] = 0.f; y[u] = 0.f; }
+      for (int c = lane; c < chunks; c += 64) {
+        float2 v[R];
+        _Pragma("unroll") for (int u = 0; u < R; ++u) { const int b = min(r0 + u, B - 1); v[u] = p2[(long)b * chunks + c]; }
+        _Pragma("unroll") for (int u = 0; u < R; ++u) { x[u] += v[u].x; y[u] += v[u].y; }
+      }
+      _Pragma("unroll") for (int u = 0; u < R; ++u) { x[u] = wave_sum(x[u]); y[u] = wave_sum(y[u]); }
+      if (lane == 0) {
+        _Pragma("unroll") for (int u = 0; u < R; ++u) {
+          const int b = r0 + u;
+          if (b < B) {
+            rs[b * rss + 2] = y[u]; rs[b * rss + 3] = x[u];
+            if (out) { out[b * 4 + 2] = y[u]; out[b * 4 + 3] = x[u]; }
+          }
+        }
+      }
+    }
+  }
+}
 
 template <int CD2>
 __device__ __forceinline__ float dec_logit(const float* wr, const float* zrow, int D2rt, float bias) {
@@ -398,7 +460,7 @@
   return s;
 }
 
-template <int PASS, int CD2>
+template <int PASS, int CD2, bool MG>
 __global__ __launch_bounds__(DEC_J * DEC_MAXG) void decoder_kernel(DecArgs a) {
   const int D2 = CD2 ? CD2 : a.D2;
   const int ws = D2 + 1;
@@ -413,7 +475,17 @@
   const int j0 = blockIdx.x * DEC_J, j = j0 + tj;
   const bool live = j < a.V;
   const int Bg = (a.B + G - 1) / G, b0 = g * Bg, b1 = min(a.B, b0 + Bg);
-  for (int e = t; e < a.B * D2; e += nthr) zl[e] = a.z[e];
+  if (MG) {
+    const int D = D2 >> 1;
+    for (int e = t; e < a.B * D2; e += nthr) {
+      const int b = e / D2, k = e - b * D2;
+      const float zv = tail_sample_z(a.lat, a.eps_e, a.eps_c, D, b, k);
+      zl[e] = zv;
+      if (PASS == 1 && a.z_out && blockIdx.x == 0) a.z_out[e] = zv;
+    }
+  } else {
+    for (int e = t; e < a.B * D2; e += nthr) zl[e] = a.z[e];
+  }
   {
     const int nrow = min(DEC_J, a.V - j0);
     for (int e = t; e < nrow * D2; e += nthr) { const int r = e / D2, k = e - r * D2; wl[r * ws + k] = a.w[(long)j0 * D2 + e]; }
@@ -423,6 +495,20 @@
   _Pragma("unroll") for (int k = 0; k < D2; ++k) wr[k] = live ? wl[tj * ws + k] : 0.f;
   const float bias = live ? a.b[j] : 0.f;
   const int lane = t & 63, wv = t >> 6, nwv = nthr >> 6;
+  const float* rs = a.rowstat;
+  int rss = 4;
+  if (MG && PASS == 2) {
+    __syncthreads();
+    dec_combine_rows<1>(a.part, a.chunks, a.B, wl, 2, blockIdx.x == 0 ? a.rowstat : nullptr);
+    rs = wl; rss = 2;
+    __syncthreads();
+  } else if (MG && PASS == 3) {
+    for (int b = t; b < a.B; b += nthr) { tile2[b * 4] = a.rowstat[b * 4]; tile2[b * 4 + 1] = a.rowstat[b * 4 + 1]; }
+    dec_combine_rows<2>(a.part2, a.chunks, a.B, tile2, 4, blockIdx.x == 0 ? a.rowstat : nullptr);
+    rs = tile2;
+    __syncthreads();
+  }
+  float* const part_out = (MG && PASS == 2) ? a.part2 : a.part;
   if (PASS == 1) {
     for (int b = b0; b < b1; ++b) tile[b * DEC_J + tj] = live ? dec_logit<CD2>(wr, zl + b * D2, D2, bias) : -INFINITY;
     __syncthreads();
@@ -430,7 +516,8 @@
       const float x0 = tile[b * DEC_J + lane], x1 = tile[b * DEC_J + 64 + lane];
       const float m = wave_max(fmaxf(x0, x1));
       const float s2 = wave_sum(expf(x0 - m) + expf(x1 - m));
-      if (lane == 0) { a.part[((long)blockIdx.x * a.B + b) * 2] = m; a.part[((long)blockIdx.x * a.B + b) * 2 + 1] = s2; }
+      const long pi = MG ? ((long)b * a.chunks + blockIdx.x) * 2 : ((long)blockIdx.x * a.B + b) * 2;
+      if (lane == 0) { a.part[pi] = m; a.part[pi + 1] = s2; }
     }
   } else if (PASS == 2) {
     for (int bb = b0; bb < b1; bb += 4) {
@@ -441,7 +528,7 @@
         if (b < b1) {
           float le = 0.f, dt = 0.f;
           if (live) {
-            const float lp = dec_logit<CD2>(wr, zl + b * D2, D2, bias) - a.rowstat[b * 4] - a.rowstat[b * 4 + 1];
+            const float lp = dec_logit<CD2>(wr, zl + b * D2, D2, bias) - rs[b * rss] - rs[b * rss + 1];
             const float p = expf(lp);
             const float tg = bw[u] * (1.f - a.ls) + a.ls / a.V;
             le = -(tg * fmaxf(lp, -100.f) + (1.f - tg) * fmaxf(log1pf(-p), -100.f));
@@ -455,7 +542,8 @@
     for (int b = wv; b < a.B; b += nwv) {
       const float le = wave_sum(tile[b * DEC_J + lane] + tile[b * DEC_J + 64 + lane]);
       const float dt = wave_sum(tile2[b * DEC_J + lane] + tile2[b * DEC_J + 64 + lane]);
-      if (lane == 0) { a.part[((long)blockIdx.x * a.B + b) * 2] = le; a.part[((long)blockIdx.x * a.B + b) * 2 + 1] = dt; }
+      const long pi = MG ? ((long)b * a.chunks + blockIdx.x) * 2 : ((long)blockIdx.x * a.B + b) * 2;
+      if (lane == 0) { part_out[pi] = le; part_out[pi + 1] = dt; }
     }
   } else {
     float dwr[CD2 ? CD2 : DEC_MAXD2];
@@ -469,11 +557,11 @@
         if (b < b1) {
           float gg = 0.f;
           if (live) {
-            const float lp = dec_logit<CD2>(wr, zl + b * D2, D2, bias) - a.rowstat[b * 4] - a.rowstat[b * 4 + 1];
+            const float lp = dec_logit<CD2>(wr, zl + b * D2, D2, bias) - rs[b * rss] - rs[b * rss + 1];
             const float p = expf(lp);
             const float tg = bw[u] * (1.f - a.ls) + a.ls / a.V;
             const float gp = (p - tg) / fmaxf((1.f - p) * p, 1e-12f);
-            gg = p * (gp - a.rowstat[b * 4 + 2]) * a.gscale;
+            gg = p * (gp - rs[b * rss + 2]) * a.gscale;
             _Pragma("unroll") for (int k = 0; k < D2; ++k) dwr[k] = fmaf(gg, zl[b * D2 + k], dwr[k]);
             dbj += gg;
           }
@@ -483,6 +571,7 @@
     }
     float* dwp = tile2;
     float* dbp = dwp + (G - 1) * DEC_J * ws;
+    if (MG) __syncthreads();
     if (g > 0) {
       _Pragma("unroll") for (int k = 0; k < D2; ++k) dwp[((g - 1) * DEC_J + tj) * ws + k] = dwr[k];
       dbp[(g - 1) * DEC_J + tj] = dbj;
@@ -500,7 +589,15 @@
       const int b = e / D2, k = e - b * D2;
       const int nrow = min(DEC_J, a.V - j0);
       float s = 0.f;
-      for (int jj = 0; jj < nrow; ++jj) s = fmaf(tile[b * DEC_J + jj], wl[jj * ws + k], s);
+      int jj = 0;
+      if (MG) {
+        for (; jj + 8 <= nrow; jj += 8) {
+          float tv[8], wv8[8];
+          _Pragma("unroll") for (int u = 0; u < 8; ++u) { tv[u] = tile[b * DEC_J + jj + u]; wv8[u] = wl[(jj + u) * ws + k]; }
+          _Pragma("unroll") for (int u = 0; u < 8; ++u) s = fmaf(tv[u], wv8[u], s);
+        }
+      }
+      for (; jj < nrow; ++jj) s = fmaf(tile[b * DEC_J + jj], wl[jj * ws + k], s);
       a.dz_part[(long)blockIdx.x * a.B * D2 + e] = s;
     }
   }
@@ -526,45 +623,74 @@
     if (lane == 0) { rowstat[b * 4 + 2] = dt; rowstat[b * 4 + 3] = le; }
   }
 }
-__global__ __launch_bounds__(256) void decoder_total_kernel(const float* __restrict__ rowstat, int B, float inv_bv, float* __restrict__ terms) {
-  __shared__ float red[16];
+__device__ __forceinline__ void decoder_total_store(const float* __restrict__ rowstat, int B, float inv_bv, float* __restrict__ terms, float* red) {
   float tot = 0.f;
   for (int b = threadIdx.x; b < B; b += 256) tot += rowstat[b * 4 + 3];
   tot = block_sum(tot, red);
   if (threadIdx.x == 0) { terms[7] = tot * inv_bv; terms[8] = terms[0] + tot * inv_bv; }
 }
-
-__global__ __launch_bounds__(256) void reduce_parts16_kernel(const float* __restrict__ parts, float* __restrict__ out, int n, int nparts) {
-  __shared__ float lds[256];
+__global__ __launch_bounds__(256) void decoder_total_kernel(const float* __restrict__ rowstat, int B, float inv_bv, float* __restrict__ terms) {
+  __shared__ float red[16];
+  decoder_total_store(rowstat, B, inv_bv, terms, red);
+}
+
+__device__ __forceinline__ bool parts16_sum(const float* __restrict__ parts, int n, int nparts, float* lds, int blk, int& c, float& t) {
   const int cl = threadIdx.x & 15, rl = threadIdx.x >> 4;
-  const int c = blockIdx.x * 16 + cl;
+  c = blk * 16 + cl;
   float s = 0.f;
   if (c < n) for (int p = rl; p < nparts; p += 16) s += parts[(long)p * n + c];
   lds[threadIdx.x] = s;
   __syncthreads();
+  t = 0.f;
   if (rl == 0 && c < n) {
-    float t = 0.f;
 #pragma unroll
     for (int r = 0; r < 16; ++r) t += lds[r * 16 + cl];
-    out[c] = t;
-  }
-}
-
+    return true;
+  }
+  return false;
+}
+__global__ __launch_bounds__(256) void reduce_parts16_kernel(const float* __restrict__ parts, float* __restrict__ out, int n, int nparts) {
+  __shared__ float lds[256];
+  int c; float t;
+  if (parts16_sum(parts, n, nparts, lds, blockIdx.x, c, t)) out[c] = t;
+}
+
+__device__ __forceinline__ void tail_dlat_store(int e, float g, const float* __restrict__ dlat_direct, const float* __restrict__ lat,
+                                                const float* __restrict__ eps_e, const float* __restrict__ eps_c, int D, float gout,
+                                                float* __restrict__ dlat) {
+  const int b = e / (2 * D), k = e - b * 2 * D;
+  const int side = k >= D, kk = k - side * D;
+  const float* row = lat + (long)b * 4 * D;
+  const float ep = side ? eps_c[kk] : eps_e[kk];
+  const float lv = row[(2 * side + 1) * D + kk];
+  dlat[(long)b * 4 * D + 2 * side * D + kk] = (dlat_direct[(long)b * 4 * D + 2 * side * D + kk] + g) * gout;
+  dlat[(long)b * 4 * D + (2 * side + 1) * D + kk] = (dlat_direct[(long)b * 4 * D + (2 * side + 1) * D + kk] + g * ep * expf(lv)) * gout;
+}
 __global__ __launch_bounds__(256) void tail_dlat_kernel(const float* __restrict__ dz_core, const float* __restrict__ dz_part, int chunks,
                                                         const float* __restrict__ dlat_direct, const float* __restrict__ lat,
                                                         const float* __restrict__ eps_e, const float* __restrict__ eps_c, int B, int D,
                                                         float gout, float* __restrict__ dlat) {
   const int e = blockIdx.x * 256 + threadIdx.x;
   if (e >= B * 2 * D) return;
-  const int b = e / (2 * D), k = e - b * 2 * D;
   float g = dz_core[e];
   for (int c = 0; c < chunks; ++c) g += dz_part[(long)c * B * 2 * D + e];
-  const int side = k >= D, kk = k - side * D;
-  const float* row = lat + (long)b * 4 * D;
-  const float ep = side ? eps_c[kk] : eps_e[kk];
-  const float lv = row[(2 * side + 1) * D + kk];
-  dlat[(long)b * 4 * D + 2 * side * D + kk] = (dlat_direct[(long)b * 4 * D + 2 * side * D + kk] + g) * gout;
-  dlat[(long)b * 4 * D + (2 * side + 1) * D + kk] = (dlat_direct[(long)b * 4 * D + (2 * side + 1) * D + kk] + g * ep * expf(lv)) * gout;
+  tail_dlat_store(e, g, dlat_direct, lat, eps_e, eps_c, D, gout, dlat);
+}
+
+__global__ __launch_bounds__(256) void tail_close_kernel(const float* __restrict__ dz_core, const float* __restrict__ dz_part, int chunks,
+                                                         const float* __restrict__ dlat_direct, const float* __restrict__ lat,
+                                                         const float* __restrict__ eps_e, const float* __restrict__ eps_c, int B, int D,
+                                                         float gout, float* __restrict__ dlat, const float* __restrict__ rowstat,
+                                                         float inv_bv, float* __restrict__ terms) {
+  __shared__ float lds[256];
+  __shared__ float red[16];
+  int c; float t;
+  if (parts16_sum(dz_part, B * 2 * D, chunks, lds, blockIdx.x, c, t)) {
+    float g = dz_core[c];
+    g += t;
+    tail_dlat_store(c, g, dlat_direct, lat, eps_e, eps_c, D, gout, dlat);
+  }
+  if (blockIdx.x == 0) decoder_total_store(rowstat, B, inv_bv, terms, red);
 }
 
 __global__ __launch_bounds__(256) void sample_z_kernel(const float* __restrict__ lat, const float* __restrict__ eps_e,
@@ -572,8 +698,7 @@
   const int e = blockIdx.x * 256 + threadIdx.x;
   if (e >= B * 2 * D) return;
   const int b = e / (2 * D), k = e - b * 2 * D;
-  const float* row = lat + (long)b * 4 * D;
-  z[e] = (k < D) ? row[k] + eps_e[k] * expf(row[D + k]) : row[2 * D + (k - D)] + eps_c[k - D] * expf(row[3 * D + (k - D)]);
+  z[e] = tail_sample_z(lat, eps_e, eps_c, D, b, k);
 }
 
 __global__ __launch_bounds__(256) void pair_prob_kernel(const float* __restrict__ lat, const float* __restrict__ eps_e,
@@ -936,6 +1061,8 @@
   float* dz_core; float* dlat_direct; float* dlat; float* dpooled; float* dpre; float* part; float* rowstat; float* dz_part;
   float* dcls; float* dgpart; float* pair_dead; float* mmd_part; float* dz_mmd;
   float* tt_lg; float* tt_spart; float* tt_hpart;
+  float* part2;
+  float* dgpart2;
   size_t total;
 };
 static TailWork carve(float* base, int B, int D, int V) {
@@ -949,6 +1076,8 @@
   w.pair_dead = take(16);
   w.mmd_part = take(4 * MMD_MAX_BLOCKS); w.dz_mmd = take((size_t)B * 2 * D);
   w.tt_lg = take((size_t)B * 16); w.tt_spart = take((size_t)TT_MAX_SLABS * 8); w.tt_hpart = take((size_t)TT_MAX_SLABS * TT_MAX_NHW);
+  w.part2 = take((size_t)chunks * B * 2);
+  w.dgpart2 = take((size_t)((4 * D + DG_CHUNK - 1) / DG_CHUNK) * B * TH);
   w.total = o;
   return w;
 }
@@ -1018,7 +1147,7 @@
   DecPlan p;
   const size_t lds0 = sizeof(float) * ((size_t)B * 2 * D + 16 + (size_t)DEC_J * (2 * D + 1) + (size_t)B * DEC_J);
   int G = DEC_MAXG;
-  auto lds3_of = [&](int g) { return lds0 + sizeof(float) * (size_t)(g - 1) * DEC_J * (2 * D + 2); };
+  auto lds3_of = [&](int g) { const size_t dwp = (size_t)(g - 1) * DEC_J * (2 * D + 2); return lds0 + sizeof(float) * (dwp > (size_t)4 * B ? dwp : (size_t)4 * B); };
   while (G > 1 && (lds3_of(G) > TAIL_LDS_MAX || (B + G - 1) / G < 4)) G >>= 1;
   p.G = G; p.lds1 = lds0; p.lds2 = lds0 + sizeof(float) * (size_t)B * DEC_J; p.lds3 = lds3_of(G);
   p.ldsmax = p.lds2 > p.lds3 ? p.lds2 : p.lds3;
@@ -1096,9 +1225,14 @@
   if (ldsmax > TAIL_LDS_MAX) return set_error(CAREL_ERR_SHAPE, "carel_tail_losses: batch too large for the decoder kernel (%zu B LDS)", ldsmax);
   if (ldsmax > 64 * 1024) {
     hipError_t e = hipSuccess;
-    const void* fns[6] = {(const void*)decoder_kernel<1, 48>, (const void*)decoder_kernel<2, 48>, (const void*)decoder_kernel<3, 48>,
-                          (const void*)decoder_kernel<1, 0>, (const void*)decoder_kernel<2, 0>, (const void*)decoder_kernel<3, 0>};
-    for (int i = 0; i < 6 && e == hipSuccess; ++i) e = hipFuncSetAttribute(fns[i], hipFuncAttributeMaxDynamicSharedMemorySize, (int)ldsmax);
+    const void* fns[] = {(const void*)decoder_kernel<1, 48, true>, (const void*)decoder_kernel<2, 48, true>, (const void*)decoder_kernel<3, 48, true>,
+                         (const void*)decoder_kernel<1, 0, true>, (const void*)decoder_kernel<2, 0, true>, (const void*)decoder_kernel<3, 0, true>,
+#ifdef CAREL_EXPERIMENTS
+                         (const void*)decoder_kernel<1, 48, false>, (const void*)decoder_kernel<2, 48, false>, (const void*)decoder_kernel<3, 48, false>,
+                         (const void*)decoder_kernel<1, 0, false>, (const void*)decoder_kernel<2, 0, false>, (const void*)decoder_kernel<3, 0, false>,
+#endif
+    };
+    for (size_t i = 0; i < sizeof(fns) / sizeof(fns[0]) && e == hipSuccess; ++i) e = hipFuncSetAttribute(fns[i], hipFuncAttributeMaxDynamicSharedMemorySize, (int)ldsmax);
     if (e != hipSuccess) return set_error(CAREL_ERR_HIP, "carel_tail_losses: hipFuncSetAttribute: %s", hipGetErrorString(e));
   }
   c.mmd_part = nullptr; c.mmd_nblk = 0; c.dz_mmd = nullptr;
@@ -1117,7 +1251,8 @@
     hipStream_t side = (hipStream_t)carel_side_stream(0);
     tev = side ? tail_events() : nullptr;
     if (tev) {
-      hipLaunchKernelGGL(sample_z_kernel, dim3((B * 2 * D + 255) / 256), dim3(256), 0, stream, c.lat, c.eps_e, c.eps_c, B, D, c.z);
+      if (!g_tail_merged)
+        hipLaunchKernelGGL(sample_z_kernel, dim3((B * 2 * D + 255) / 256), dim3(256), 0, stream, c.lat, c.eps_e, c.eps_c, B, D, c.z);
       if (hipEventRecord(tev->fork, stream) != hipSuccess || hipStreamWaitEvent(side, tev->fork, 0) != hipSuccess)
         return set_error(CAREL_ERR_HIP, "carel_tail_losses: event fork failed");
       core_stream = side;
@@ -1143,24 +1278,39 @@
   d.B = B; d.D2 = 2 * D; d.V = V; d.z = (const float*)a->z; d.w = (const float*)a->dec_w; d.b = (const float*)a->dec_b;
   d.bow = (const float*)a->bow; d.ls = a->label_smoothing; d.part = w.part; d.rowstat = w.rowstat; d.dz_part = w.dz_part;
   d.dw = (float*)a->d_dec_w; d.db = (float*)a->d_dec_b; d.gscale = 1.0f / ((float)B * (float)V);
-#define DEC_LAUNCH(PASS, LDS)                                                                              \
+  d.lat = c.lat; d.eps_e = c.eps_e; d.eps_c = c.eps_c; d.z_out = c.z ? nullptr : (float*)a->z;
+  d.part2 = w.part2; d.chunks = chunks;
+#define DEC_LAUNCH(PASS, MG, LDS)                                                                              \
   do {                                                                                                  \
-    if (2 * D == 48) hipLaunchKernelGGL((decoder_kernel<PASS, 48>), dim3(chunks), dim3(DEC_J * G), LDS, stream, d); \
-    else hipLaunchKernelGGL((decoder_kernel<PASS, 0>), dim3(chunks), dim3(DEC_J * G), LDS, stream, d);      \
+    if (2 * D == 48) hipLaunchKernelGGL((decoder_kernel<PASS, 48, MG>), dim3(chunks), dim3(DEC_J * G), LDS, stream, d); \
+    else hipLaunchKernelGGL((decoder_kernel<PASS, 0, MG>), dim3(chunks), dim3(DEC_J * G), LDS, stream, d);      \
   } while (0)
-  DEC_LAUNCH(1, lds1);
-  hipLaunchKernelGGL(decoder_combine_kernel, dim3((B + 3) / 4), dim3(256), 0, stream, (const float*)w.part, chunks, B, 1, w.rowstat);
-  DEC_LAUNCH(2, lds2);
-  hipLaunchKernelGGL(decoder_combine_kernel, dim3((B + 3) / 4), dim3(256), 0, stream, (const float*)w.part, chunks, B, 2, w.rowstat);
-  DEC_LAUNCH(3, lds3);
+#ifdef CAREL_EXPERIMENTS
+  if (!g_tail_merged) {
+    DEC_LAUNCH(1, false, lds1);
+    hipLaunchKernelGGL(decoder_combine_kernel, dim3((B + 3) / 4), dim3(256), 0, stream, (const float*)w.part, chunks, B, 1, w.rowstat);
+    DEC_LAUNCH(2, false, lds2);
+    hipLaunchKernelGGL(decoder_combine_kernel, dim3((B + 3) / 4), dim3(256), 0, stream, (const float*)w.part, chunks, B, 2, w.rowstat);
+    DEC_LAUNCH(3, false, lds3);
+    if ((rc = check_launch("decoder kernels"))) return join_on_error(rc);
+    hipLaunchKernelGGL(reduce_parts16_kernel, dim3((B * 2 * D + 15) / 16), dim3(256), 0, stream, (const float*)w.dz_part, w.dz_part, B * 2 * D, chunks);
+    if (tev && hipStreamWaitEvent(stream, tev->join, 0) != hipSuccess) return join_on_error(set_error(CAREL_ERR_HIP, "carel_tail_losses: event join failed"));
+    hipLaunchKernelGGL(decoder_total_kernel, dim3(1), dim3(256), 0, stream, (const float*)w.rowstat, B, d.gscale, (float*)a->terms);
+    hipLaunchKernelGGL(tail_dlat_kernel, dim3((B * 2 * D + 255) / 256), dim3(256), 0, stream, (const float*)w.dz_core, (const float*)w.dz_part,
+                       1, (const float*)w.dlat_direct, (const float*)a->lat, (const float*)a->eps_e, (const float*)a->eps_c, B, D, 1.0f, w.dlat);
+    return check_launch("tail_dlat_kernel");
+  }
+#endif
+  DEC_LAUNCH(1, true, lds1);
+  DEC_LAUNCH(2, true, lds2);
+  DEC_LAUNCH(3, true, lds3);
 #undef DEC_LAUNCH
   if ((rc = check_launch("decoder kernels"))) return join_on_error(rc);
-  hipLaunchKernelGGL(reduce_parts16_kernel, dim3((B * 2 * D + 15) / 16), dim3(256), 0, stream, (const float*)w.dz_part, w.dz_part, B * 2 * D, chunks);
   if (tev && hipStreamWaitEvent(stream, tev->join, 0) != hipSuccess) return join_on_error(set_error(CAREL_ERR_HIP, "carel_tail_losses: event join failed"));
-  hipLaunchKernelGGL(decoder_total_kernel, dim3(1), dim3(256), 0, stream, (const float*)w.rowstat, B, d.gscale, (float*)a->terms);
-  hipLaunchKernelGGL(tail_dlat_kernel, dim3((B * 2 * D + 255) / 256), dim3(256), 0, stream, (const float*)w.dz_core, (const float*)w.dz_part,
-                     1, (const float*)w.dlat_direct, (const float*)a->lat, (const float*)a->eps_e, (const float*)a->eps_c, B, D, 1.0f, w.dlat);
-  return check_launch("tail_dlat_kernel");
+  hipLaunchKernelGGL(tail_close_kernel, dim3((B * 2 * D + 15) / 16), dim3(256), 0, stream, (const float*)w.dz_core, (const float*)w.dz_part, chunks,
+                     (const float*)w.dlat_direct, (const float*)a->lat, (const float*)a->eps_e, (const float*)a->eps_c, B, D, 1.0f, w.dlat,
+                     (const float*)w.rowstat, d.gscale, (float*)a->terms);
+  return check_launch("tail_close_kernel");
 }
 
 extern "C" int carel_tail_losses_tiled(const carel_tail_args* a, void* stream_) {
@@ -1287,8 +1437,10 @@
   if (!a->work || !a->dx_last_f32 || !a->d_pooler_w || !a->d_pooler_b) return set_error(CAREL_ERR_ARG, "carel_tail_backward: null tensor");
   const int B = a->batch, D = a->ec_dim, N = 4 * D;
   TailWork w = carve((float*)a->work, B, D, a->bow_dim);
+  const float* dlat_scale = nullptr;
   if (grad_out_dev) {
-    hipLaunchKernelGGL(scale_inplace_kernel, dim3((B * N + 255) / 256), dim3(256), 0, stream, w.dlat, (long)B * N, (const float*)grad_out_dev);
+    if (g_tail_merged && !dz_extra && !a->head_in_f32) dlat_scale = (const float*)grad_out_dev;
+    else hipLaunchKernelGGL(scale_inplace_kernel, dim3((B * N + 255) / 256), dim3(256), 0, stream, w.dlat, (long)B * N, (const float*)grad_out_dev);
   }
   if (dz_extra) {
     if (!a->lat || !a->eps_e || !a->eps_c) return set_error(CAREL_ERR_ARG, "carel_tail_backward_dz: lat / eps needed");
@@ -1321,21 +1473,34 @@
   for (int i = 0; i < 4; ++i) { hp.w[i] = (const float*)a->head_w[i]; hp.b[i] = nullptr; ho.w[i] = (float*)a->d_head_w[i]; ho.b[i] = (float*)a->d_head_b[i]; }
   if (ho.w[0] && ho.w[1] && ho.w[2] && ho.w[3])
     hipLaunchKernelGGL(rowvec_wgrad_kernel, dim3((N + 3) / 4), dim3(256), 0, stream, (const float*)w.dlat, (long)N, (const float*)a->pooled,
-                       (long)TH, (const int*)nullptr, B, N, D, ho);
-  hipLaunchKernelGGL(rowvec_dgrad_kernel<0>, dim3((B + 3) / 4, hc), dim3(256), 0, stream, (const float*)w.dlat, (long)N, B, N, D, hp,
-                     (const float*)nullptr, (float*)nullptr, w.dgpart);
-  hipLaunchKernelGGL(sum_parts_kernel, dim3((unsigned)((bt / 4 + 255) / 256)), dim3(256), 0, stream, (const float*)w.dgpart, w.dpooled, bt, hc);
+                       (long)TH, (const int*)nullptr, B, N, D, ho, dlat_scale);
   PtrSet4 pp; OutSet4 po;
   for (int i = 0; i < 4; ++i) { pp.w[i] = nullptr; pp.b[i] = nullptr; po.w[i] = nullptr; po.b[i] = nullptr; }
   pp.w[0] = (const float*)a->pooler_w; po.w[0] = (float*)a->d_pooler_w; po.b[0] = (float*)a->d_pooler_b;
-  hipLaunchKernelGGL(rowvec_dgrad_kernel<1>, dim3((B + 3) / 4, pc), dim3(256), 0, stream, (const float*)w.dpooled, (long)TH, B, TH, TH, pp,
-                     (const float*)a->pooled, w.dpre, w.dgpart);
-  hipLaunchKernelGGL(sum_parts_kernel, dim3((unsigned)((bt / 4 + 255) / 256)), dim3(256), 0, stream, (const float*)w.dgpart, w.dcls, bt, pc);
+  const size_t dx_rows = a->n_rows > 0 ? (size_t)a->n_rows : (size_t)B * a->seq_len;
+#ifdef CAREL_EXPERIMENTS
+  if (!g_tail_merged) {
+    hipLaunchKernelGGL(rowvec_dgrad_kernel<0>, dim3((B + 3) / 4, hc), dim3(256), 0, stream, (const float*)w.dlat, (long)N, B, N, D, hp,
+                       (const float*)nullptr, (float*)nullptr, w.dgpart);
+    hipLaunchKernelGGL(sum_parts_kernel, dim3((unsigned)((bt / 4 + 255) / 256)), dim3(256), 0, stream, (const float*)w.dgpart, w.dpooled, bt, hc);
+    hipLaunchKernelGGL(rowvec_dgrad_kernel<1>, dim3((B + 3) / 4, pc), dim3(256), 0, stream, (const float*)w.dpooled, (long)TH, B, TH, TH, pp,
+                       (const float*)a->pooled, w.dpre, w.dgpart);
+    hipLaunchKernelGGL(sum_parts_kernel, dim3((unsigned)((bt / 4 + 255) / 256)), dim3(256), 0, stream, (const float*)w.dgpart, w.dcls, bt, pc);
+    hipLaunchKernelGGL(rowvec_wgrad_kernel, dim3(TH / 4), dim3(256), 0, stream, (const float*)w.dpre, (long)TH, (const float*)a->x_last_f32,
+                       (long)a->seq_len * TH, (const int*)a->cls_rows, B, TH, TH, po);
+    (void)hipMemsetAsync(a->dx_last_f32, 0, dx_rows * TH * sizeof(float), stream);
+    hipLaunchKernelGGL(scatter_cls_kernel, dim3(B), dim3(256), 0, stream, (const float*)w.dcls, B, a->seq_len, (const int*)a->cls_rows,
+                       (float*)a->dx_last_f32);
+    return check_launch("tail backward");
+  }
+#endif
+  hipLaunchKernelGGL(rowvec_dgrad_kernel<0>, dim3((B + 3) / 4, hc), dim3(256), 0, stream, (const float*)w.dlat, (long)N, B, N, D, hp,
+                     (const float*)nullptr, (float*)nullptr, w.dgpart2, 1, 0L, dlat_scale);
+  hipLaunchKernelGGL(rowvec_dgrad_kernel<1>, dim3((B + 3) / 4, pc), dim3(256), 0, stream, (const float*)w.dgpart2, (long)TH, B, TH, TH, pp,
+                     (const float*)a->pooled, w.dpre, w.dgpart, hc, bt);
   hipLaunchKernelGGL(rowvec_wgrad_kernel, dim3(TH / 4), dim3(256), 0, stream, (const float*)w.dpre, (long)TH, (const float*)a->x_last_f32,
                      (long)a->seq_len * TH, (const int*)a->cls_rows, B, TH, TH, po);
-  const size_t dx_rows = a->n_rows > 0 ? (size_t)a->n_rows : (size_t)B * a->seq_len;
-  (void)hipMemsetAsync(a->dx_last_f32, 0, dx_rows * TH * sizeof(float), stream);
-  hipLaunchKernelGGL(scatter_cls_kernel, dim3(B), dim3(256), 0, stream, (const float*)w.dcls, B, a->seq_len, (const int*)a->cls_rows,
-                     (float*)a->dx_last_f32);
+  hipLaunchKernelGGL(tail_dx_kernel, dim3((unsigned)dx_rows), dim3(256), 0, stream, (const float*)w.dgpart, bt, pc, B, a->seq_len,
+                     (const int*)a->cls_rows, (long)dx_rows, (float*)a->dx_last_f32);
   return check_launch("tail backward");
 }
diff --git a/carel_vae_amd/drl_classifier.py b/carel_vae_amd/drl_classifier.py
--- a/carel_vae_amd/drl_classifier.py
+++ b/carel_vae_amd/drl_classifier.py
@@ -955,7 +955,11 @@
             cls_rows, n_rows = (None, c.Bp * c.S) if c.pack is None else (c.pack.cu, c.pack.n_tokens)
         ta = ops.tail_args(c.buf, xl, W, c.labels, c.eps_e, c.eps_c, self.opt, klw, grads=G, drop=drop, cls_rows=cls_rows, n_rows=n_rows,
                            head_in=head_in, d_head_in=d_head_in)
+        z_ptr = ta.z
+        if self._dp is None:
+            ta.z = None
         ops.tail_latents(ta)
+        ta.z = z_ptr
         if self._dp is not None:
             self._dp.fill_global(ta, c)
         ta.serial = 0 if self.overlap_wgrad else 1
```

New measurement: 8419 (median of 4 runs). No clear change (+0.3%).
